# Bernat-C/MRI-Diffusion-SuperResolution

Measured on AMD Instinct MI355X. Metric: MRI slices/sec (50-step DDIM, 256^2, bs=32), higher is better.
Workload: dtype bf16; 1 GPU; configs[1]: 256x256 1-ch synthetic MRI slices -> 4x32x32 latents, SD-1.5-size UNet (859.5M params, random init) + rank-4 LoRA, 50-step DDIM, bs=32 per GPU; ddim_steps=50, parallelism=slice-sharded x1 (no collective), lora=explicit adapters, down-projection + rank-r update inside the projection GEMMs, tile_table=profiles/r03_tune_cache.tsv, hipgraph=True

## Files before the change

include/mrisr_debug.h:

```cpp
#ifndef MRISR_DEBUG_H
#define MRISR_DEBUG_H
#ifdef __cplusplus
extern "C" {
#endif

void mrisr_debug_force_split(int splitk);
void mrisr_debug_force_tile(int tile);
void mrisr_debug_prefer_tile(int tile);
void mrisr_debug_gemm_flags(int flags);
void mrisr_debug_gemm_stamps(void* dev_buf, int tile);
void mrisr_debug_set_tile_eff(int tile, double eff);
void mrisr_debug_set_tuned(const char* key, int tile, int splitk);
void mrisr_debug_gn_fused(int on);

int mrisr_autotune_stats(int* shapes, double* ms);
void mrisr_autotune_release(void);

int mrisr_bench_gemm(int M, int N, int K, int conv, int B, int H, int W, int stride, int ups, int c1, int tile, int splitk,
                     int iters, float* ms_out);

void mrisr_debug_sk_inkernel(int on);

void mrisr_debug_subpix(int min_rows);

void mrisr_debug_temb_table(int on);

void mrisr_debug_mlp_proj(int on);

void mrisr_debug_gn_slabs(int on);

void mrisr_debug_sc_fused(int on);

void mrisr_debug_ff_proj_fused(int on);

void mrisr_debug_xattn_tail(int on);
void mrisr_debug_xattn_tail_stamps(void* dev_buf);

int mrisr_bench_mlp(int M, int hidden, int iters, float* ms_out);

#ifdef __cplusplus
}
#endif
#endif
```

mri-diffusion-superresolution_amd/csrc/capi_ops.hip:

```cpp
#include <algorithm>
#include <cmath>
#include <cstring>
#include <memory>
#include <vector>

#include "api.h"
#include "model.h"
#include "train_ops.h"

using namespace mrisr;

namespace {
struct OpScratch {
    std::vector<std::unique_ptr<DevBuf>> bufs;
    void* alloc(size_t bytes, bool zero = false) {
        bufs.emplace_back(new DevBuf());
        if (bufs.back()->reserve(bytes ? bytes : 1, zero)) return nullptr;
        return bufs.back()->p;
    }
};
template <typename T>
int op_gemm_run(OpScratch& sc, hipStream_t st, GemmArgs& g) {
    return gemm_run<T>(g, st, false, [&sc](size_t n) { return sc.alloc(n); });
}
template <typename T>
int op_plan(GemmArgs& g, int splitk, bool replan, DevBuf& part) {
    g.splitk = splitk;
    if (splitk <= 0) { g.splitk = 1; TRY(gemm_choose(g, sizeof(T) == 2)); }
    else if (replan) { TRY(gemm_choose(g, sizeof(T) == 2)); g.splitk = splitk; }
    return gemm_alloc_partial(g, devbuf_alloc(part));
}
}
template <typename T>
__global__ void rows_to_heads_kernel(const T* x, T* dst, int B, int N, int H, int hd, int npad, int dpad, int tr) {
    const long long total = (long long)B * N * H * hd;
    for (long long i = blockIdx.x * 256ll + threadIdx.x; i < total; i += (long long)gridDim.x * 256) {
        const int dd = (int)(i % hd);
        const int h = (int)((i / hd) % H);
        const int tok = (int)((i / ((long long)hd * H)) % N);
        const int b = (int)(i / ((long long)hd * H * N));
        const size_t bh = (size_t)b * H + h;
        if (!tr) dst[(bh * npad + tok) * dpad + dd] = x[i];
        else dst[(bh * dpad + dd) * npad + tok] = x[i];
    }
}

template <typename T>
static int op_conv3x3_t(const mrisr_tensor* x, const mrisr_tensor* x2, const float* w, const float* bias, int cout,
                        int stride, int ups, int act, int splitk, mrisr_tensor* y, hipStream_t st) {
    const int B = (int)x->shape[0], C0 = (int)x->shape[1], H = (int)x->shape[2], W = (int)x->shape[3];
    const int C1 = x2 ? (int)x2->shape[1] : 0;
    const int Cin = C0 + C1;
    DevBuf wp, part;
    TRY(wp.reserve((size_t)cout * Cin * 9 * sizeof(T), false));
    TRY(launch_pack_conv3x3<T>(w, wp.p, cout, Cin, 3, st));
    if (!x2 && !ups && Cin % (128 / (int)sizeof(T)) != 0) {
        DirectConvArgs a;
        a.x = x->data; a.w = wp.p; a.bias = bias; a.y = y->data; a.B = B; a.Hin = H; a.Win = W; a.Cin = Cin;
        a.Hout = (H - 1) / stride + 1; a.Wout = (W - 1) / stride + 1; a.Cout = cout; a.ks = 3; a.stride = stride; a.pad = 1; a.act = act;
        MRISR_REQUIRE(y->shape[1] == cout && y->shape[2] == a.Hout && y->shape[3] == a.Wout, "conv output shape");
        TRY(launch_direct_conv<T>(a, st));
        MRISR_CHECK_HIP(hipStreamSynchronize(st));
        return 0;
    }
    if (ups == 2) {
        MRISR_REQUIRE(sizeof(T) == 2 && !x2 && stride == 1 && act == ACT_NONE && (4 * Cin) % 64 == 0 && cout % 8 == 0, "sub-pixel upsample conv: bf16, single source");
        MRISR_REQUIRE(y->shape[1] == cout && y->shape[2] == 2 * H && y->shape[3] == 2 * W, "conv output shape");
        DevBuf sp, planes;
        TRY(sp.reserve((size_t)16 * cout * Cin * sizeof(T), false));
        TRY(planes.reserve((size_t)4 * B * H * W * cout * sizeof(T), false));
        TRY(launch_pack_conv_subpix<T>(w, sp.p, cout, Cin, st));
        GemmArgs g;
        ga_rows(g, x->data, C0, C0); ga_conv3(g, B, H, W); g.kw = 2; g.subpix = 1;
        ga_batch(g, 4, 0, (long long)cout * 4 * Cin, (long long)B * H * W * cout); ga_weight(g, sp.p, B * H * W, cout, 4 * Cin);
        g.bias = bias; ga_out(g, planes.p, cout);
        TRY(gemm_run<T>(g, st, false, devbuf_alloc(part)));
        TRY(launch_subpix_shuffle<T>(planes.p, y->data, B, H, W, cout, st));
        MRISR_CHECK_HIP(hipStreamSynchronize(st));
        return 0;
    }
    GemmArgs g;
    ga_rows(g, x->data, C0, C0);
    if (x2) ga_rows2(g, x2->data, C1, C1);
    ga_conv3(g, B, H, W, stride, ups);
    MRISR_REQUIRE(y->shape[1] == cout && y->shape[2] == g.Hout && y->shape[3] == g.Wout, "conv output shape");
    ga_weight(g, wp.p, B * g.Hout * g.Wout, cout, 9 * Cin); g.bias = bias; g.act = act; ga_out(g, y->data, cout);
    TRY(op_plan<T>(g, splitk, false, part));
    TRY(launch_gemm<T>(g, st));
    MRISR_CHECK_HIP(hipStreamSynchronize(st));
    return 0;
}

extern "C" void mrisr_debug_force_tile(int t);
struct ForcedTile {
    explicit ForcedTile(int t) { mrisr_debug_force_tile(t); }
    ~ForcedTile() { mrisr_debug_force_tile(0); }
    ForcedTile(const ForcedTile&) = delete;
    ForcedTile& operator=(const ForcedTile&) = delete;
};

static int op_conv3x3_sc_t(const mrisr_tensor* x, const mrisr_tensor* x2, const float* w, const float* bias, const mrisr_tensor* xs,
                           const mrisr_tensor* xs2, const float* w_sc, const float* bias_sc, int cout, int splitk, int tile, int fused,
                           mrisr_tensor* y, hipStream_t st) {
    typedef bf16 T;
    const int B = (int)x->shape[0], C0 = (int)x->shape[1], H = (int)x->shape[2], W = (int)x->shape[3];
    const int C1 = x2 ? (int)x2->shape[1] : 0, Cin = C0 + C1;
    const int S0 = (int)xs->shape[1], S1 = xs2 ? (int)xs2->shape[1] : 0, Cs = S0 + S1;
    MRISR_REQUIRE(xs->shape[0] == B && xs->shape[2] == H && xs->shape[3] == W && (!xs2 || (xs2->shape[0] == B && xs2->shape[2] == H && xs2->shape[3] == W)),
                  "shortcut sources: the conv input's batch and image size");
    MRISR_REQUIRE(y->shape[1] == cout && y->shape[2] == H && y->shape[3] == W, "conv output shape");
    MRISR_REQUIRE(Cin % 64 == 0 && S0 % 64 == 0 && S1 % 64 == 0 && cout % 4 == 0, "channel counts: multiples of 64");
    const size_t K9 = (size_t)9 * Cin, Kt = K9 + Cs;
    DevBuf w9, wsc, bank, bsum, part;
    TRY(w9.reserve((size_t)cout * K9 * sizeof(T), false));
    TRY(wsc.reserve((size_t)cout * Cs * sizeof(T), false));
    TRY(launch_pack_conv3x3<T>(w, w9.p, cout, Cin, 3, st));
    TRY(launch_pack_rows<T>(w_sc, cout, Cs, wsc.p, Cs, 0, 0, 0, 0, 1.0f, st));
    GemmArgs g;
    ga_rows(g, x->data, C0, C0);
    if (x2) ga_rows2(g, x2->data, C1, C1);
    ga_conv3(g, B, H, W); ga_out(g, y->data, cout);
    const int M = B * H * W;
    if (fused) {
        TRY(bank.reserve((size_t)cout * Kt * sizeof(T), false));
        TRY(bsum.reserve((size_t)cout * sizeof(float), false));
        MRISR_CHECK_HIP(hipMemcpy2DAsync(bank.p, Kt * sizeof(T), w9.p, K9 * sizeof(T), K9 * sizeof(T), cout, hipMemcpyDeviceToDevice, st));
        MRISR_CHECK_HIP(hipMemcpy2DAsync(static_cast<T*>(bank.p) + K9, Kt * sizeof(T), wsc.p, (size_t)Cs * sizeof(T), (size_t)Cs * sizeof(T), cout,
                                         hipMemcpyDeviceToDevice, st));
        MRISR_CHECK_HIP(hipMemcpyAsync(bsum.p, bias, (size_t)cout * sizeof(float), hipMemcpyDeviceToDevice, st));
        TRY(launch_add_inplace<float>(bsum.p, bias_sc, cout, st));
        ga_tail(g, xs->data, S0, S0);
        if (xs2) ga_tail2(g, xs2->data, S1, S1);
        ga_weight(g, bank.p, M, cout, (int)Kt); g.bias = static_cast<const float*>(bsum.p);
    } else {
        GemmArgs s;
        ga_rows(s, xs->data, S0, S0);
        if (xs2) ga_rows2(s, xs2->data, S1, S1);
        ga_weight(s, wsc.p, M, cout, Cs); s.bias = bias_sc; ga_out(s, y->data, cout);
        DevBuf spart;
        TRY(gemm_run<T>(s, st, false, devbuf_alloc(spart)));
        MRISR_CHECK_HIP(hipStreamSynchronize(st));
        ga_weight(g, w9.p, M, cout, (int)K9); g.bias = bias; ga_resid(g, y->data, cout);
    }
    ForcedTile forced(tile);
    TRY(op_plan<T>(g, splitk, !tile, part));
    TRY(launch_gemm<T>(g, st));
    MRISR_CHECK_HIP(hipStreamSynchronize(st));
    return 0;
}

static int run_planned(GemmArgs& g, DevBuf& part, hipStream_t st) { return gemm_run<bf16>(g, st, false, devbuf_alloc(part)); }
static int op_ff_proj_t(const mrisr_tensor* h, const mrisr_tensor* t, const mrisr_tensor* x, const float* w2, const float* b2, const float* wp,
                        const float* bp, int tile, int fused, mrisr_tensor* y, hipStream_t st) {
    typedef bf16 T;
    const int M = (int)h->shape[0], K4 = (int)h->shape[1], C = (int)t->shape[1];
    MRISR_REQUIRE(t->shape[0] == M && x->shape[0] == M && x->shape[1] == C && y->shape[0] == M && y->shape[1] == C, "ff.net.2 + proj_out: row shapes");
    MRISR_REQUIRE(C % 64 == 0 && K4 % 64 == 0, "ff.net.2 + proj_out: widths that are multiples of 64");
    DevBuf bank, bsum, w2p, wpp, mid, part;
    if (fused) {
        const int Kt = K4 + C;
        TRY(bank.reserve((size_t)C * Kt * sizeof(T), false));
        TRY(bsum.reserve((size_t)C * sizeof(float), false));
        TRY(launch_compose_ff_proj(wp, w2, b2, bp, bank.p, Kt, static_cast<float*>(bsum.p), C, K4, st));
        TRY(launch_pack_rows<T>(wp, C, C, bank.p, Kt, 0, K4, 0, 0, 1.0f, st));
        GemmArgs g;
        ga_rows(g, h->data, K4, K4); ga_rows2(g, t->data, C, C); ga_weight(g, bank.p, M, C, Kt); g.bias = static_cast<const float*>(bsum.p);
        ga_resid(g, x->data, C); ga_out(g, y->data, C); g.no_rp = 1;
        ForcedTile forced(tile);
        TRY(run_planned(g, part, st));
    } else {
        TRY(w2p.reserve((size_t)C * K4 * sizeof(T), false));
        TRY(wpp.reserve((size_t)C * C * sizeof(T), false));
        TRY(mid.reserve((size_t)M * C * sizeof(T), false));
        TRY(launch_pack_rows<T>(w2, C, K4, w2p.p, K4, 0, 0, 0, 0, 1.0f, st));
        TRY(launch_pack_rows<T>(wp, C, C, wpp.p, C, 0, 0, 0, 0, 1.0f, st));
        GemmArgs g1, g2;
        auto linear = [&](GemmArgs& g, const void* a, int k, const void* w, const float* b, const void* resid, void* out) {
            ga_rows(g, a, k, k); ga_weight(g, w, M, C, k); g.bias = b; ga_resid(g, resid, C); ga_out(g, out, C);
        };
        linear(g1, h->data, K4, w2p.p, b2, t->data, mid.p);
        linear(g2, mid.p, C, wpp.p, bp, x->data, y->data);
        ForcedTile forced(tile);
        TRY(run_planned(g1, part, st));
        MRISR_CHECK_HIP(hipStreamSynchronize(st));
        TRY(run_planned(g2, part, st));
    }
    MRISR_CHECK_HIP(hipStreamSynchronize(st));
    return 0;
}

template <typename T>
static int op_attention_t(const mrisr_tensor* q, const mrisr_tensor* k, const mrisr_tensor* v, int H, int flash,
                          mrisr_tensor* out, hipStream_t st) {
    const int B = (int)q->shape[0], N = (int)q->shape[1], C = (int)q->shape[2], Nk = (int)k->shape[1];
    const int hd = C / H;
    constexpr int BK = 128 / (int)sizeof(T);
    const bool use_flash = flash && sizeof(T) == 2;
    const int dpad = round_up(hd, use_flash ? 32 : BK), npad = round_up(N, 64), nkpad = round_up(Nk, 64);
    DevBuf qb, kb, vb;
    TRY(qb.reserve((size_t)B * H * npad * dpad * sizeof(T), true));
    TRY(kb.reserve((size_t)B * H * nkpad * dpad * sizeof(T), true));
    TRY(vb.reserve((size_t)B * H * dpad * nkpad * sizeof(T), true));
    auto conv = [&](const mrisr_tensor* x, void* dst, int n, int np, int tr) {
        hipLaunchKernelGGL(rows_to_heads_kernel<T>, dim3(1024), dim3(256), 0, st, static_cast<const T*>(x->data),
                           static_cast<T*>(dst), B, n, H, hd, np, dpad, tr);
    };
    conv(q, qb.p, N, npad, 0);
    conv(k, kb.p, Nk, nkpad, 0);
    conv(v, vb.p, Nk, nkpad, 1);
    MRISR_CHECK_HIP(hipGetLastError());
    OpScratch sc;
    auto scratch = [&sc](size_t n) { return sc.alloc(n); };
    AttnGeom geo;
    geo.B = B; geo.H = H; geo.N = N; geo.npad = npad; geo.hd = hd; geo.dpad = dpad; geo.nk = Nk; geo.nkpad = nkpad;
    if (use_flash) {
        const bool fp8 = flash == 2;
        AttnArgs a;
        TRY(attn_flash_args(a, geo, qb.p, kb.p, vb.p, out->data, nullptr, fp8, scratch));
        TRY(attn_flash_launch(a, fp8, false, st));
    } else {
        const size_t cnt = (size_t)B * H * N * nkpad;
        float* S = static_cast<float*>(sc.alloc(cnt * sizeof(float)));
        void* P = sizeof(T) == 2 ? sc.alloc(cnt * sizeof(T)) : S;
        if (!S || !P) return 7;
        TRY(attn_materialised<T>(geo, qb.p, kb.p, vb.p, S, P, out->data, false, st, [&](GemmArgs& g) { return op_gemm_run<T>(sc, st, g); }));
    }
    MRISR_CHECK_HIP(hipStreamSynchronize(st));
    return 0;
}


template <typename T>
static int op_conv_lora_down_t(const void* x, int B, int H, int W, int cin, const float* A, int r, float* z, int route, hipStream_t st) {
    DevBuf av, bdummy, scr;
    TRY(av.reserve((size_t)r * 9 * cin * sizeof(T), false));
    TRY(bdummy.reserve((size_t)r * sizeof(float), true));
    TRY(launch_conv_lora_pack<T>(A, static_cast<const float*>(bdummy.p), 1.0f, av.p, nullptr, nullptr, nullptr, cin, 1, r, st));
    const size_t sb = conv_lora_down_scratch_bytes(B * H * W, cin, r, sizeof(T), route);
    if (sb) TRY(scr.reserve(sb, false));
    TRY(launch_conv_lora_down<T>(x, av.p, z, B, H, W, cin, r, static_cast<float*>(scr.p), st, route));
    MRISR_CHECK_HIP(hipStreamSynchronize(st));
    return 0;
}
template <typename T>
static int op_conv_lora_dgrad_t(const float* dz, int B, int H, int W, int r, const float* A, int cin, void* dx, int accumulate, hipStream_t st) {
    DevBuf av, bank, bdummy;
    TRY(av.reserve((size_t)r * 9 * cin * sizeof(T), false));
    if (sizeof(T) == 2) TRY(bank.reserve((size_t)cin * conv_lora_kpad(r) * 2, true));
    TRY(bdummy.reserve((size_t)r * sizeof(float), true));
    TRY(launch_conv_lora_pack<T>(A, static_cast<const float*>(bdummy.p), 1.0f, av.p, bank.p, nullptr, nullptr, cin, 1, r, st));
    TRY(launch_conv_lora_dgrad<T>(dz, av.p, bank.p, dx, B, H, W, cin, r, accumulate, st));
    MRISR_CHECK_HIP(hipStreamSynchronize(st));
    return 0;
}
template <typename T>
static int op_conv3x3_lora_t(const mrisr_tensor* x, const float* w, const float* bias, const float* A, const float* Bm, int r, float scale,
                             const float* rowvec, const mrisr_tensor* resid, int cout, int splitk, int tile, mrisr_tensor* y, hipStream_t st) {
    const int B = (int)x->shape[0], Cin = (int)x->shape[1], H = (int)x->shape[2], W = (int)x->shape[3], M = B * H * W;
    DevBuf wp, av, sb, zb, scr, part;
    TRY(wp.reserve((size_t)cout * Cin * 9 * sizeof(T), false));
    TRY(launch_pack_conv3x3<T>(w, wp.p, cout, Cin, 3, st));
    if (r > 0) {
        TRY(av.reserve((size_t)r * 9 * Cin * sizeof(T), false));
        TRY(sb.reserve((size_t)cout * r * sizeof(float), false));
        TRY(zb.reserve((size_t)M * r * sizeof(float), false));
        TRY(launch_conv_lora_pack<T>(A, Bm, scale, av.p, nullptr, static_cast<float*>(sb.p), nullptr, Cin, cout, r, st));
        const size_t sbytes = conv_lora_down_scratch_bytes(M, Cin, r, sizeof(T));
        if (sbytes) TRY(scr.reserve(sbytes, false));
        TRY(launch_conv_lora_down<T>(x->data, av.p, static_cast<float*>(zb.p), B, H, W, Cin, r, static_cast<float*>(scr.p), st));
    }
    GemmArgs g;
    ga_rows(g, x->data, Cin, Cin); ga_conv3(g, B, H, W); ga_weight(g, wp.p, M, cout, 9 * Cin); g.bias = bias;
    if (rowvec) ga_rowvec(g, rowvec, cout, H * W);
    if (resid) ga_resid(g, resid->data, cout);
    ga_out(g, y->data, cout);
    if (r > 0) ga_lora_epilogue(g, static_cast<const float*>(zb.p), r, static_cast<const float*>(sb.p), r, cout);
    ForcedTile forced(tile);
    TRY(op_plan<T>(g, splitk, !tile, part));
    TRY(launch_gemm<T>(g, st));
    MRISR_CHECK_HIP(hipStreamSynchronize(st));
    return 0;
}

static GemmArgs op_linear_args(const mrisr_tensor* x, const void* w, int n, const float* bias, int act, const mrisr_tensor* y) {
    const int K = (int)x->shape[1];
    GemmArgs g;
    ga_rows(g, x->data, K, K); ga_weight(g, w, (int)x->shape[0], n, K); g.bias = bias; g.act = act; ga_out(g, y->data, (int)y->shape[1]);
    return g;
}

extern "C" {

static int op_dtype_ok(const mrisr_tensor* x) {
    MRISR_REQUIRE(x && (x->dtype == MRISR_F32 || x->dtype == MRISR_BF16), "op tensors: f32 or bf16");
    return 0;
}

int mrisr_op_conv3x3(const mrisr_tensor* x, const mrisr_tensor* x2, const float* w_oihw_dev, const float* bias_dev,
                     int cout, int stride, int upsample, int act, int splitk, int tile, mrisr_tensor* y,
                     void* stream) {
    API_BEGIN
    TRY(op_dtype_ok(x));
    TRY(gemm_prepare());
    MRISR_REQUIRE(x->layout == MRISR_NHWC && y && y->layout == MRISR_NHWC && y->dtype == x->dtype, "NHWC in/out, same dtype");
    ForcedTile forced(tile);
    return x->dtype == MRISR_F32 ? op_conv3x3_t<float>(x, x2, w_oihw_dev, bias_dev, cout, stride, upsample, act, splitk, y, (hipStream_t)stream)
                                 : op_conv3x3_t<bf16>(x, x2, w_oihw_dev, bias_dev, cout, stride, upsample, act, splitk, y, (hipStream_t)stream);
    API_END
}

int mrisr_op_conv3x3_sc(const mrisr_tensor* x, const mrisr_tensor* x2, const float* w_oihw_dev, const float* bias_dev, const mrisr_tensor* xs,
                        const mrisr_tensor* xs2, const float* w_sc_dev, const float* bias_sc_dev, int cout, int splitk, int tile, int fused,
                        mrisr_tensor* y, void* stream) {
    API_BEGIN
    MRISR_REQUIRE(x && xs && y && w_oihw_dev && bias_dev && w_sc_dev && bias_sc_dev, "null argument");
    MRISR_REQUIRE(x->dtype == MRISR_BF16 && xs->dtype == MRISR_BF16 && y->dtype == MRISR_BF16 && (!x2 || x2->dtype == MRISR_BF16) &&
                      (!xs2 || xs2->dtype == MRISR_BF16),
                  "conv3x3 + 1x1 shortcut: bf16 tensors");
    MRISR_REQUIRE(x->layout == MRISR_NHWC && xs->layout == MRISR_NHWC && y->layout == MRISR_NHWC && (!x2 || x2->layout == MRISR_NHWC) &&
                      (!xs2 || xs2->layout == MRISR_NHWC),
                  "NHWC in/out");
    TRY(gemm_prepare());
    return op_conv3x3_sc_t(x, x2, w_oihw_dev, bias_dev, xs, xs2, w_sc_dev, bias_sc_dev, cout, splitk, tile, fused, y, (hipStream_t)stream);
    API_END
}

int mrisr_op_ff_proj(const mrisr_tensor* h, const mrisr_tensor* t, const mrisr_tensor* x, const float* w2_dev, const float* b2_dev,
                     const float* wp_dev, const float* bp_dev, int tile, int fused, mrisr_tensor* y, void* stream) {
    API_BEGIN
    MRISR_REQUIRE(h && t && x && y && w2_dev && wp_dev, "null argument");
    MRISR_REQUIRE(h->dtype == MRISR_BF16 && t->dtype == MRISR_BF16 && x->dtype == MRISR_BF16 && y->dtype == MRISR_BF16, "ff.net.2 + proj_out: bf16 rows");
    MRISR_REQUIRE(h->ndim == 2 && t->ndim == 2 && x->ndim == 2 && y->ndim == 2, "rows in/out");
    TRY(gemm_prepare());
    return op_ff_proj_t(h, t, x, w2_dev, b2_dev, wp_dev, bp_dev, tile, fused, y, (hipStream_t)stream);
    API_END
}

int mrisr_op_linear(const mrisr_tensor* x, const float* w_dev, const float* bias_dev, int n, int act, int splitk,
                    int tile, mrisr_tensor* y, void* stream) {
    API_BEGIN
    TRY(op_dtype_ok(x));
    TRY(gemm_prepare());
    MRISR_REQUIRE(x->ndim == 2 && y && y->ndim == 2 && y->dtype == x->dtype, "rows in/out");
    hipStream_t st = (hipStream_t)stream;
    const int M = (int)x->shape[0], K = (int)x->shape[1];
    const bool f32 = x->dtype == MRISR_F32;
    const int esz = f32 ? 4 : 2;
    DevBuf wp, part, bp;
    TRY(wp.reserve((size_t)n * K * esz, false));
    const bool geglu = act == ACT_GEGLU;
    if (f32) TRY(launch_pack_rows<float>(w_dev, n, K, wp.p, K, 0, 0, geglu ? 1 : 0, n / 2, 1.0f, st));
    else TRY(launch_pack_rows<bf16>(w_dev, n, K, wp.p, K, 0, 0, geglu ? 1 : 0, n / 2, 1.0f, st));
    const float* bias = bias_dev;
    if (geglu && bias_dev) {
        TRY(bp.reserve((size_t)n * sizeof(float), false));
        TRY(launch_pack_bias_geglu(bias_dev, static_cast<float*>(bp.p), n / 2, st));
        bias = static_cast<const float*>(bp.p);
    }
    GemmArgs g = op_linear_args(x, wp.p, n, bias, act, y);
    ForcedTile forced(tile);
    TRY(f32 ? op_plan<float>(g, splitk, false, part) : op_plan<bf16>(g, splitk, false, part));
    TRY(f32 ? launch_gemm<float>(g, st) : launch_gemm<bf16>(g, st));
    MRISR_CHECK_HIP(hipStreamSynchronize(st));
    return 0;
    API_END
}

int mrisr_op_linear_resid(const mrisr_tensor* x, const float* w_dev, const float* bias_dev, int n, const float* rowvec_dev, int rowvec_rows,
                          const float* lora_a_dev, const float* lora_b_dev, int lora_r, float lora_scale, const mrisr_tensor* resid, int splitk,
                          int tile, mrisr_tensor* y, void* stream) {
    API_BEGIN
    typedef bf16 T;
    MRISR_REQUIRE(x && y && w_dev && x->dtype == MRISR_BF16 && y->dtype == MRISR_BF16 && x->ndim == 2 && y->ndim == 2, "linear + residual: bf16 rows in/out");
    MRISR_REQUIRE(!resid || (resid->dtype == MRISR_BF16 && resid->ndim == 2 && resid->shape[0] == x->shape[0] && resid->shape[1] >= n), "residual rows");
    TRY(gemm_prepare());
    hipStream_t st = (hipStream_t)stream;
    const int M = (int)x->shape[0], K = (int)x->shape[1];
    MRISR_REQUIRE(!rowvec_dev || (rowvec_rows >= 1 && M % rowvec_rows == 0), "row vector: rows dividing M");
    MRISR_REQUIRE(lora_r == 0 || (lora_r >= 1 && lora_r <= 16 && lora_a_dev && lora_b_dev && splitk <= 1), "adapter: rank 1 .. 16, A and B, un-split");
    DevBuf wp, part, av, sb, zb;
    TRY(wp.reserve((size_t)n * K * sizeof(T), false));
    TRY(launch_pack_rows<T>(w_dev, n, K, wp.p, K, 0, 0, 0, 0, 1.0f, st));
    GemmArgs g = op_linear_args(x, wp.p, n, bias_dev, ACT_NONE, y);
    if (rowvec_dev) ga_rowvec(g, rowvec_dev, n, M / rowvec_rows);
    if (resid) ga_resid(g, resid->data, (int)resid->shape[1]);
    ForcedTile forced(tile);
    if (!lora_r) {
// ... 877 lines not shown
```

mri-diffusion-superresolution_amd/csrc/gemm.hip:

```cpp
#include "common.h"
#include "prof.h"

#include <cstdio>
#include <cstdlib>
#include <cstring>
#include <map>
#include <mutex>
#include <unordered_map>

namespace mrisr {

static void* g_zero_page = nullptr;
static constexpr size_t kZeroPageBytes = 128 * 1024;
const void* zero_page() { return g_zero_page; }
int init_zero_page() {
    if (g_zero_page) return 0;
    MRISR_CHECK_HIP(hipMalloc(&g_zero_page, kZeroPageBytes));
    MRISR_CHECK_HIP(hipMemset(g_zero_page, 0, kZeroPageBytes));
    return 0;
}

typedef const __attribute__((address_space(1))) void* gptr_t;
typedef __attribute__((address_space(3))) void* lptr_t;

__device__ __forceinline__ void glds16(const void* src, char* lds_wave_base) {
    __builtin_amdgcn_global_load_lds((gptr_t)src, (lptr_t)lds_wave_base, 16, 0, 0);
}

template <typename T>
__device__ __forceinline__ void store4(T* p, const float* v);
template <>
__device__ __forceinline__ void store4<float>(float* p, const float* v) {
    *reinterpret_cast<float4*>(p) = make_float4(v[0], v[1], v[2], v[3]);
}
template <>
__device__ __forceinline__ void store4<bf16>(bf16* p, const float* v) {
    bf16x4 o = {(bf16)v[0], (bf16)v[1], (bf16)v[2], (bf16)v[3]};
    *reinterpret_cast<bf16x4*>(p) = o;
}
template <typename T>
__device__ __forceinline__ void load4(const T* p, float* v);
template <>
__device__ __forceinline__ void load4<float>(const float* p, float* v) {
    float4 t = *reinterpret_cast<const float4*>(p);
    v[0] = t.x; v[1] = t.y; v[2] = t.z; v[3] = t.w;
}
template <>
__device__ __forceinline__ void load4<bf16>(const bf16* p, float* v) {
    bf16x4 t = *reinterpret_cast<const bf16x4*>(p);
    v[0] = (float)t[0]; v[1] = (float)t[1]; v[2] = (float)t[2]; v[3] = (float)t[3];
}

__device__ __forceinline__ int exchange_tokens4(const float* v, unsigned& w0, unsigned& w1) {
    const int fr = threadIdx.x & 15;
    const bool odd = fr & 1;
    const float s0 = __shfl_xor(odd ? v[0] : v[2], 1);
    const float s1 = __shfl_xor(odd ? v[1] : v[3], 1);
    const float a0 = odd ? s0 : v[0], a1 = odd ? v[2] : s0;
    const float c0 = odd ? s1 : v[1], c1 = odd ? v[3] : s1;
    typedef __attribute__((ext_vector_type(2))) __bf16 bf16x2;
    const bf16x2 pa = {(bf16)a0, (bf16)a1}, pc = {(bf16)c0, (bf16)c1};
    const unsigned ua = __builtin_bit_cast(unsigned, pa), uc = __builtin_bit_cast(unsigned, pc);
    const bool hi2 = fr & 2;
    const unsigned recv = __shfl_xor(hi2 ? ua : uc, 2);
    w0 = hi2 ? recv : ua;
    w1 = hi2 ? uc : recv;
    return (odd ? 2 : 0) + (hi2 ? 1 : 0);
}

template <typename T>
__device__ __forceinline__ void epilogue4(const GemmArgs& g, int z, int m, int n0, float* v, const float* vg, const float* zl = nullptr,
                                          T* lds_dst = nullptr, bool resid_later = false, bool mfma_lanes = true, T* lds_t = nullptr,
                                          int ml = 0, int nl = 0, int tpitch = 0, const float* pb = nullptr, const float* pbg = nullptr) {
    const float alpha = g.alpha;
    float b4[4] = {0.f, 0.f, 0.f, 0.f};
    if (g.act == ACT_GEGLU) {
        float bu[4] = {0, 0, 0, 0}, bg[4] = {0, 0, 0, 0};
        if (pb) {
#pragma unroll
            for (int r = 0; r < 4; ++r) { bu[r] = pb[r]; bg[r] = pbg[r]; }
        } else if (g.bias) {
            load4<float>(g.bias + n0, bu);
            load4<float>(g.bias + n0 + 16, bg);
        }
#pragma unroll
        for (int r = 0; r < 4; ++r) v[r] = (v[r] * alpha + bu[r]) * gelu_erf_t<T>(vg[r] * alpha + bg[r]);
        const int nc = (n0 >> 5) * 16 + (n0 & 15);
        T* o = reinterpret_cast<T*>(g.out) + (size_t)m * g.ldo + nc;
        store4<T>(o, v);
        return;
    }
    if (pb) {
#pragma unroll
        for (int r = 0; r < 4; ++r) b4[r] = pb[r];
    } else if (g.bias) {
        load4<float>(g.bias + n0, b4);
    }
#pragma unroll
    for (int r = 0; r < 4; ++r) v[r] = v[r] * alpha + b4[r];
    if (g.lora_z || zl) {
        const float* zr = (zl ? zl : g.lora_z + (size_t)m * g.lora_zld) + (n0 / g.lora_secN) * g.lora_r;
        const float* lb = g.lora_b + (size_t)n0 * g.lora_r;
        if (g.lora_r == 4) {
            float z4[4];
            load4<float>(zr, z4);
#pragma unroll
            for (int r = 0; r < 4; ++r) {
                float l4[4];
                load4<float>(lb + r * 4, l4);
                v[r] += z4[0] * l4[0] + z4[1] * l4[1] + z4[2] * l4[2] + z4[3] * l4[3];
            }
        } else {
            for (int q = 0; q < g.lora_r; ++q) {
                const float zq = zr[q];
#pragma unroll
                for (int r = 0; r < 4; ++r) v[r] += zq * lb[r * g.lora_r + q];
            }
        }
    }
    if (g.rowvec && !(pb && g.rowvec_div >= g.M)) {
        float t4[4];
        load4<float>(g.rowvec + (size_t)(m / g.rowvec_div) * g.rowvec_ld + n0, t4);
#pragma unroll
        for (int r = 0; r < 4; ++r) v[r] += t4[r];
    }
    if (g.act == ACT_RELU) {
#pragma unroll
        for (int r = 0; r < 4; ++r) v[r] = fmaxf(v[r], 0.f);
    } else if (g.act == ACT_SILU) {
#pragma unroll
        for (int r = 0; r < 4; ++r) v[r] = silu_f(v[r]);
    }
    const size_t zoff = (size_t)(z / g.heads) * g.o_bs + (size_t)(z % g.heads) * g.o_hs;
    if (g.resid && !resid_later) {
        float r4[4];
        load4<T>(reinterpret_cast<const T*>(g.resid) + zoff + (size_t)m * g.ldr + n0, r4);
#pragma unroll
        for (int r = 0; r < 4; ++r) v[r] += r4[r];
    }
    if (g.out_mode == OUT_NONE) {
        if (v[0] == 1.2345e30f) store4<T>(reinterpret_cast<T*>(g.out), v);
    } else if (g.out_mode == OUT_ROWS) {
        if (lds_dst) store4<T>(lds_dst, v);
        else store4<T>(reinterpret_cast<T*>(g.out) + zoff + (size_t)m * g.ldo + n0, v);
    } else if (g.out_mode == OUT_F32) {
        store4<float>(reinterpret_cast<float*>(g.out) + zoff + (size_t)m * g.ldo + n0, v);
    } else {
        if (lds_dst) {
            store4<T>(lds_dst, v);
            return;
        }
        if (sizeof(T) == 2 && lds_t) {
            unsigned w0, w1;
            const int drow = exchange_tokens4(v, w0, w1);
            *reinterpret_cast<uint2*>(lds_t + (nl + drow) * tpitch + (ml & ~3)) = make_uint2(w0, w1);
            return;
        }
        const int s = n0 / g.secC;
        const int c = n0 - s * g.secC;
        const int h = c / g.hd;
        const int dd = c - h * g.hd;
        const int b = m / g.ntok;
        const int tok = m - b * g.ntok;
        T* base = reinterpret_cast<T*>(s == 0 ? g.sec_ptr[0] : (s == 1 ? g.sec_ptr[1] : g.sec_ptr[2]));
        const int tr = (s == 0 ? g.sec_tr[0] : (s == 1 ? g.sec_tr[1] : g.sec_tr[2]));
        const size_t bh = (size_t)b * g.nheads + h;
        if (!tr) {
            store4<T>(base + (bh * g.npad + tok) * g.dpad + dd, v);
        } else if (sizeof(T) == 2 && mfma_lanes && (g.ntok & 3) == 0 && (g.M & 3) == 0) {
            unsigned w0, w1;
            const int drow = exchange_tokens4(v, w0, w1);
            T* o = base + (bh * g.dpad + dd + drow) * g.npad + (tok & ~3);
            *reinterpret_cast<uint2*>(o) = make_uint2(w0, w1);
        } else {
            T* o = base + (bh * g.dpad + dd) * g.npad + tok;
#pragma unroll
            for (int r = 0; r < 4; ++r) o[(size_t)r * g.npad] = from_f32<T>(v[r]);
        }
    }
}

template <int NFR>
__device__ __forceinline__ void preload_cols(const GemmArgs& g, int nbase, float (&pb)[NFR][4]) {
    const bool fold = g.rowvec && g.rowvec_div >= g.M;
#pragma unroll
    for (int i = 0; i < NFR; ++i) {
        const int n = min(nbase + i * 16, g.N - 4);
        float b[4] = {0.f, 0.f, 0.f, 0.f}, t[4] = {0.f, 0.f, 0.f, 0.f};
        if (g.bias) load4<float>(g.bias + n, b);
        if (fold) load4<float>(g.rowvec + n, t);
#pragma unroll
        for (int r = 0; r < 4; ++r) pb[i][r] = b[r] + t[r];
    }
}

template <int NFR>
__device__ __forceinline__ void preload_cols(const GemmArgs& g, int nbase, f32x4 (&pb)[NFR]) {
    const bool fold = g.rowvec && g.rowvec_div >= g.M;
#pragma unroll
    for (int i = 0; i < NFR; ++i) pb[i] = f32x4{0.f, 0.f, 0.f, 0.f};
    if (g.bias) {
#pragma unroll
        for (int i = 0; i < NFR; ++i) pb[i] = *reinterpret_cast<const f32x4*>(g.bias + min(nbase + i * 16, g.N - 4));
    }
    if (fold) {
#pragma unroll
        for (int i = 0; i < NFR; ++i) pb[i] += *reinterpret_cast<const f32x4*>(g.rowvec + min(nbase + i * 16, g.N - 4));
    }
}

template <typename T> struct Frag;
template <> struct Frag<bf16> { typedef bf16x8 type; };
template <> struct Frag<float> { typedef f32x4 type; };

__device__ __forceinline__ void mma(f32x4& acc, const bf16x8& w, const bf16x8& a) {
    acc = __builtin_amdgcn_mfma_f32_16x16x32_bf16(w, a, acc, 0, 0, 0);
}
__device__ __forceinline__ void mma(f32x4& acc, const f32x4& w, const f32x4& a) {
#pragma unroll
    for (int j = 0; j < 4; ++j) acc = __builtin_amdgcn_mfma_f32_16x16x4f32(w[j], a[j], acc, 0, 0, 0);
}

__device__ __forceinline__ void lds_poison(char* smem_base, int nthreads) {
    const unsigned bytes = ((const __attribute__((address_space(4))) unsigned*)__builtin_amdgcn_dispatch_ptr())[7];
    for (unsigned o = threadIdx.x * 16u; o + 16u <= bytes; o += (unsigned)nthreads * 16u)
        *reinterpret_cast<uint4*>(smem_base + o) = make_uint4(~0u, ~0u, ~0u, ~0u);
    __syncthreads();
}
static int gemm_flags_now();

static constexpr int kStampHdr = 8, kStampWgs = 1024, kStampSlotWords = kStampHdr + 8 * kStampWgs, kStampSlots = 256;
__device__ __forceinline__ unsigned long long* gemm_stamp_slot(const GemmArgs& g, bool header) {
    if (!g.stamps) return nullptr;
    const unsigned wg = blockIdx.x + gridDim.x * (blockIdx.y + gridDim.y * blockIdx.z);
    if (header && wg == 0 && threadIdx.x == 0) {
        g.stamps[0] = (unsigned long long)g.M; g.stamps[1] = (unsigned long long)g.N; g.stamps[2] = (unsigned long long)g.K;
        g.stamps[3] = (unsigned long long)gridDim.x * gridDim.y * gridDim.z;
        g.stamps[4] = (g.resid ? 1u : 0u) | (g.lora_a ? 2u : 0u) | (g.conv ? 4u : 0u) | (g.cs0 ? 8u : 0u);
        g.stamps[5] = (unsigned long long)g.splitk; g.stamps[6] = (unsigned long long)(unsigned)g.dbg; g.stamps[7] = 1ull;
    }
    return wg < (unsigned)kStampWgs ? g.stamps + kStampHdr + (size_t)wg * 8 : nullptr;
}
__device__ __forceinline__ unsigned long long* gemm_stamp_word(const GemmArgs& g, int k, bool header = false) {
    unsigned long long* const slot = gemm_stamp_slot(g, header);
    return slot ? slot + k : nullptr;
}
static_assert(kStampSlotWords == kStampHdr + 8 * kStampWgs, "a slot: the header, then 8 words for each of the first kStampWgs workgroups");

template <typename T, int BM, int BN, int WGM, int WGN>
__global__ __launch_bounds__(256) void gemm_kernel(const GemmArgs g, const char* __restrict__ zero) {
    constexpr int EB = sizeof(T);
    constexpr int CH = 16 / EB;
    constexpr int BK = 8 * CH;
    constexpr int A_IT = BM / 32, W_IT = BN / 32;
    constexpr int WTM = BM / WGM, WTN = BN / WGN;
    constexpr int MF = WTM / 16, NF = WTN / 16;
    constexpr int STAGE = (BM + BN) * 128;
    static_assert(WGM * WGN == 4, "4 waves");
    extern __shared__ __attribute__((aligned(16))) char smem[];

    const int tid = threadIdx.x;
    const int lane = tid & 63;
    const int wave = __builtin_amdgcn_readfirstlane(tid >> 6);
    const int z = blockIdx.z;
    const int split = blockIdx.y;
    if (g.dbg & 2048) lds_poison(smem, (int)blockDim.x);

    const int ntn = (g.N + BN - 1) / BN;
    const int ntm = (g.M + BM - 1) / BM;
    const int nblk = ntn * ntm;
    int logical;
    {
        const int bid = blockIdx.x;
        const int xcd = bid & 7, q = nblk >> 3, r = nblk & 7;
        logical = (xcd < r ? xcd * (q + 1) : r * (q + 1) + (xcd - r) * q) + (bid >> 3);
    }
    int tn, tm;
    {
        const int GM = g.group_m > 1 ? g.group_m : 1;
        const int per_group = GM * ntn;
        const int grp = logical / per_group;
        const int first_m = grp * GM;
        const int gsz = min(GM, ntm - first_m);
        const int within = logical - grp * per_group;
        tm = first_m + within % gsz;
        tn = within / gsz;
    }
    const int m0 = tm * BM, n0 = tn * BN;

    const T* a0 = reinterpret_cast<const T*>(g.a0) + (size_t)z * g.a_bs;
    const T* a1 = reinterpret_cast<const T*>(g.a1);
    const T* w = reinterpret_cast<const T*>(g.w) + (size_t)z * g.w_bs;

    const int lrow = tid >> 3, pch = tid & 7;
    const T* wsrc[W_IT];
    bool wok[W_IT];
#pragma unroll
    for (int it = 0; it < W_IT; ++it) {
        const int row = it * 32 + lrow;
        const int n = n0 + row;
        const int c = pch ^ (row & 7);
        wok[it] = n < g.N;
        wsrc[it] = w + (size_t)n * g.K + c * CH;
    }
    const T* asrc0[A_IT];
    const T* asrc1[A_IT];
    int ab[A_IT], ay[A_IT], ax[A_IT];
    bool aok[A_IT];
    int acoff[A_IT];
#pragma unroll
    for (int it = 0; it < A_IT; ++it) {
        const int row = it * 32 + lrow;
        const int m = m0 + row;
        const int c = pch ^ (row & 7);
        aok[it] = m < g.M;
        acoff[it] = c * CH;
        if (!g.conv) {
            asrc0[it] = a0 + (size_t)m * g.lda0 + c * CH;
            asrc1[it] = a1 ? a1 + (size_t)m * g.lda1 + c * CH : nullptr;
            ab[it] = ay[it] = ax[it] = 0;
        } else {
            const int hw = g.Hout * g.Wout;
            const int b = m / hw;
            const int rem = m - b * hw;
            const int oy = rem / g.Wout;
            ab[it] = b;
            ay[it] = oy * g.stride - g.pad;
            ax[it] = (rem - oy * g.Wout) * g.stride - g.pad;
            asrc0[it] = asrc1[it] = nullptr;
        }
    }

    const int nkt = g.K / BK;
    const int per = (nkt + g.splitk - 1) / g.splitk;
    const int kt_beg = split * per;
    const int kt_end = min(nkt, kt_beg + per);
    const int Ct = g.c0 + g.c1;
    int tap = 0, cc = 0;
    if (g.conv) {
        const int k0 = kt_beg * BK;
        tap = k0 / Ct;
        cc = k0 - tap * Ct;
    }
    const int Hc = g.Hin << g.ups, Wc = g.Win << g.ups;

    auto stage = [&](int kt, int buf) {
        char* sb = smem + buf * STAGE;
        const int k0 = kt * BK;
#pragma unroll
        for (int it = 0; it < W_IT; ++it) {
            const void* src = wok[it] ? (const void*)(wsrc[it] + k0) : (const void*)zero;
            glds16(src, sb + BM * 128 + (it * 256 + wave * 64) * 16);
        }
        if (!g.conv) {
            const bool second = k0 >= g.c0;
#pragma unroll
            for (int it = 0; it < A_IT; ++it) {
                const void* src = zero;
                if (aok[it]) src = second ? (const void*)(asrc1[it] + (k0 - g.c0)) : (const void*)(asrc0[it] + k0);
                glds16(src, sb + (it * 256 + wave * 64) * 16);
            }
        } else {
            const int ky = tap / 3, kx = tap - ky * 3;
            const bool second = cc >= g.c0;
            const T* base = second ? a1 : a0;
            const int ld = second ? g.lda1 : g.lda0;
            const int ch = second ? cc - g.c0 : cc;
#pragma unroll
            for (int it = 0; it < A_IT; ++it) {
                const int iy = ay[it] + ky, ix = ax[it] + kx;
                const void* src = zero;
                if (aok[it] && iy >= 0 && iy < Hc && ix >= 0 && ix < Wc && (!g.zstuff || ((iy | ix) & 1) == 0)) {
                    const size_t pix = ((size_t)ab[it] * g.Hin + (iy >> g.ups)) * g.Win + (ix >> g.ups);
                    src = base + pix * ld + ch + acoff[it];
                }
                glds16(src, sb + (it * 256 + wave * 64) * 16);
            }
            cc += BK;
            if (cc >= Ct) { cc = 0; ++tap; }
        }
    };

    f32x4 acc[NF][MF];
#pragma unroll
    for (int i = 0; i < NF; ++i)
#pragma unroll
        for (int j = 0; j < MF; ++j) acc[i][j] = f32x4{0.f, 0.f, 0.f, 0.f};

    const int wm0 = (wave / WGN) * WTM, wn0 = (wave % WGN) * WTN;
    const int fr = lane & 15, fg = lane >> 4;

    typedef typename Frag<T>::type frag_t;
    auto compute = [&](int buf) {
        const char* sa = smem + buf * STAGE;
        const char* sw = sa + BM * 128;
#pragma unroll
        for (int kk = 0; kk < 2; ++kk) {
            const int phys = ((kk * 4 + fg) ^ (fr & 7)) * 16;
            frag_t wf[NF], af[MF];
#pragma unroll
            for (int i = 0; i < NF; ++i)
                wf[i] = *reinterpret_cast<const frag_t*>(sw + (wn0 + i * 16 + fr) * 128 + phys);
#pragma unroll
            for (int j = 0; j < MF; ++j)
                af[j] = *reinterpret_cast<const frag_t*>(sa + (wm0 + j * 16 + fr) * 128 + phys);
#pragma unroll
            for (int i = 0; i < NF; ++i)
#pragma unroll
                for (int j = 0; j < MF; ++j) mma(acc[i][j], wf[i], af[j]);
        }
    };

    if (kt_beg < kt_end) {
        stage(kt_beg, 0);
        asm volatile("s_waitcnt vmcnt(0)" ::: "memory");
        __syncthreads();
        int cur = 0;
        for (int kt = kt_beg; kt < kt_end; ++kt) {
            if (kt + 1 < kt_end) stage(kt + 1, cur ^ 1);
            compute(cur);
            asm volatile("s_waitcnt vmcnt(0)" ::: "memory");
            __syncthreads();
            cur ^= 1;
        }
    }

    if (g.splitk > 1) {
        float* part = g.partial + ((size_t)z * g.splitk + split) * (size_t)g.M * g.N;
#pragma unroll
        for (int i = 0; i < NF; ++i)
#pragma unroll
            for (int j = 0; j < MF; ++j) {
                const int m = m0 + wm0 + j * 16 + fr;
                const int n = n0 + wn0 + i * 16 + fg * 4;
                if (m < g.M && n < g.N) {
                    float v[4] = {acc[i][j][0], acc[i][j][1], acc[i][j][2], acc[i][j][3]};
                    store4<float>(part + (size_t)m * g.N + n, v);
                }
            }
        return;
    }
    float pb[NF][4];
    preload_cols<NF>(g, n0 + wn0 + fg * 4, pb);
    if (g.act == ACT_GEGLU) {
#pragma unroll
        for (int i = 0; i < NF; i += 2)
#pragma unroll
            for (int j = 0; j < MF; ++j) {
                const int m = m0 + wm0 + j * 16 + fr;
                const int n = n0 + wn0 + i * 16 + fg * 4;
                if (m < g.M && n < g.N) {
                    float v[4] = {acc[i][j][0], acc[i][j][1], acc[i][j][2], acc[i][j][3]};
                    float vg[4] = {acc[i + 1][j][0], acc[i + 1][j][1], acc[i + 1][j][2], acc[i + 1][j][3]};
                    epilogue4<T>(g, z, m, n, v, vg, nullptr, nullptr, false, true, nullptr, 0, 0, 0, pb[i], pb[i + 1 < NF ? i + 1 : i]);
                }
            }
        return;
    }
#pragma unroll
    for (int i = 0; i < NF; ++i)
#pragma unroll
        for (int j = 0; j < MF; ++j) {
            const int m = m0 + wm0 + j * 16 + fr;
            const int n = n0 + wn0 + i * 16 + fg * 4;
            if (m < g.M && n < g.N) {
                float v[4] = {acc[i][j][0], acc[i][j][1], acc[i][j][2], acc[i][j][3]};
                epilogue4<T>(g, z, m, n, v, nullptr, nullptr, nullptr, false, true, nullptr, 0, 0, 0, pb[i]);
            }
        }
}

template <int BM, int BN, int NT = 256>
__device__ __forceinline__ void copy_out_tile(const GemmArgs& g, const bf16* otile, int pitch, int m0, int n0, int z, bool add_resid,
                                              unsigned long long* stamp_resid = nullptr) {
    __syncthreads();
    constexpr int CPR = BN / 8;
    bf16* out = reinterpret_cast<bf16*>(g.out) + (size_t)z * g.o_bs;
    const bf16* res = add_resid ? reinterpret_cast<const bf16*>(g.resid) + (size_t)z * g.o_bs : nullptr;
    constexpr int TOTAL = BM * CPR, IT = (TOTAL + NT - 1) / NT, BATCH = IT < 5 ? IT : 5;
    for (int it0 = 0; it0 < IT; it0 += BATCH) {
        bf16x8 rv[BATCH];
#pragma unroll
        for (int u = 0; u < BATCH; ++u) {
            const int idx = (int)threadIdx.x + (it0 + u) * NT;
            const int row = idx / CPR, ch = idx - row * CPR;
            const int m = m0 + row, n = n0 + ch * 8;
            if (res && idx < TOTAL && m < g.M && n + 8 <= g.N) rv[u] = *reinterpret_cast<const bf16x8*>(res + (size_t)m * g.ldr + n);
        }
        if (stamp_resid && it0 == 0 && threadIdx.x == 0) {
            if (res) asm volatile("s_waitcnt vmcnt(0)" ::: "memory");
            *stamp_resid = __builtin_readcyclecounter();
        }
#pragma unroll
        for (int u = 0; u < BATCH; ++u) {
            const int idx = (int)threadIdx.x + (it0 + u) * NT;
            const int row = idx / CPR, ch = idx - row * CPR;
            const int m = m0 + row, n = n0 + ch * 8;
            if (idx >= TOTAL || m >= g.M || n >= g.N) continue;
            const bf16* src = otile + row * pitch + ch * 8;
            bf16* dst = out + (size_t)m * g.ldo + n;
            if (n + 8 <= g.N) {
                bf16x8 v = *reinterpret_cast<const bf16x8*>(src);
                if (res) {
#pragma unroll
                    for (int e = 0; e < 8; ++e) v[e] = (bf16)((float)v[e] + (float)rv[u][e]);
                }
                *reinterpret_cast<bf16x8*>(dst) = v;
            } else {
                bf16x4 v = *reinterpret_cast<const bf16x4*>(src);
                if (res) {
                    const bf16x4 r = *reinterpret_cast<const bf16x4*>(res + (size_t)m * g.ldr + n);
#pragma unroll
                    for (int e = 0; e < 4; ++e) v[e] = (bf16)((float)v[e] + (float)r[e]);
                }
                *reinterpret_cast<bf16x4*>(dst) = v;
            }
        }
    }
}

template <int BM, int BN>
__device__ __forceinline__ void copy_out_heads(const GemmArgs& g, const bf16* otile, int m0, int n0, bool tr) {
    __syncthreads();
    const int s = n0 / g.secC;
    bf16* base = reinterpret_cast<bf16*>(s == 0 ? g.sec_ptr[0] : (s == 1 ? g.sec_ptr[1] : g.sec_ptr[2]));
    if (!tr) {
        constexpr int CPR = BN / 8, P = BN + 8;
        for (int idx = threadIdx.x; idx < BM * CPR; idx += 256) {
            const int row = idx / CPR, ch = idx - row * CPR;
            const int m = m0 + row, n = n0 + ch * 8;
            if (m >= g.M || n >= g.N) continue;
            const int c = n - s * g.secC, h = c / g.hd, dd = c - h * g.hd;
            const int b = m / g.ntok, tok = m - b * g.ntok;
            *reinterpret_cast<bf16x8*>(base + (((size_t)b * g.nheads + h) * g.npad + tok) * g.dpad + dd) =
                *reinterpret_cast<const bf16x8*>(otile + row * P + ch * 8);
        }
    } else {
        constexpr int TPC = BM / 8, P = BM + 8;
        for (int idx = threadIdx.x; idx < BN * TPC; idx += 256) {
            const int col = idx / TPC, tc = idx - col * TPC;
            const int n = n0 + col, m = m0 + tc * 8;
            if (m >= g.M || n >= g.N) continue;
            const int c = n - s * g.secC, h = c / g.hd, dd = c - h * g.hd;
            const int b = m / g.ntok, tok = m - b * g.ntok;
            *reinterpret_cast<bf16x8*>(base + (((size_t)b * g.nheads + h) * g.dpad + dd) * g.npad + tok) =
                *reinterpret_cast<const bf16x8*>(otile + col * P + tc * 8);
        }
    }
}

typedef __attribute__((address_space(3))) void* lds_ptr_t;
__device__ __forceinline__ __amdgpu_buffer_rsrc_t make_rsrc(const void* p, unsigned bytes) {
    return __builtin_amdgcn_make_buffer_rsrc(const_cast<void*>(p), 0, bytes, 0x00020000);
}
__device__ __forceinline__ void bl16(__amdgpu_buffer_rsrc_t r, char* lds_wave_base, unsigned voff, unsigned soff) {
    __builtin_amdgcn_raw_ptr_buffer_load_lds(r, (lds_ptr_t)lds_wave_base, 16, voff, soff, 0, 0);
}
#define BL_OOB 0x80000000u


__device__ __forceinline__ void pretouch_weights(const __amdgpu_buffer_rsrc_t& rw, long long w_bytes, char* scratch, int wave, int lane, int cap) {
    const int n_wg = (int)(gridDim.x * gridDim.y);
    const int wg = (int)(blockIdx.x + blockIdx.y * gridDim.x);
    const long long pieces = (w_bytes + 1023) >> 10;
    const int per_wg = (int)((pieces + n_wg - 1) / n_wg);
    const int per_wave = min((per_wg + 3) >> 2, cap);
    const long long first = (long long)wg * per_wg + (long long)wave * per_wave;
    for (int i = 0; i < per_wave; ++i) {
        const long long pc = first + i;
        const unsigned off = pc < pieces ? (unsigned)(pc << 10) + (unsigned)lane * 16u : BL_OOB;
        bl16(rw, scratch + ((wave * 2 + (i & 1)) << 10), off, 0u);
    }
}

template <int NF, int MF>
__device__ __forceinline__ bool splitk_last_arriver(const GemmArgs& g, f32x4 (&acc)[NF][MF], unsigned tile_idx, const float* slab0, int m_base, int n_base,
                                                    int fr, int fg, char* ticket_lds) {
    __builtin_amdgcn_fence(__ATOMIC_RELEASE, "agent");
    __syncthreads();
    if (threadIdx.x == 0)
        *reinterpret_cast<volatile unsigned*>(ticket_lds) = __hip_atomic_fetch_add(g.sk_counters + tile_idx, 1u, __ATOMIC_ACQ_REL, __HIP_MEMORY_SCOPE_AGENT);
    __syncthreads();
    const unsigned ticket = *reinterpret_cast<volatile unsigned*>(ticket_lds);
    if (ticket != (unsigned)g.splitk - 1) return false;
    __syncthreads();
    if (threadIdx.x == 0) __hip_atomic_store(g.sk_counters + tile_idx, 0u, __ATOMIC_RELAXED, __HIP_MEMORY_SCOPE_AGENT);
    __builtin_amdgcn_fence(__ATOMIC_ACQUIRE, "agent");
    const size_t slab = (size_t)g.M * g.N;
#pragma unroll
    for (int i = 0; i < NF; ++i)
#pragma unroll
        for (int j = 0; j < MF; ++j) acc[i][j] = f32x4{0.f, 0.f, 0.f, 0.f};
    for (int s = 0; s < g.splitk; ++s) {
        const float* p = slab0 + (size_t)s * slab;
#pragma unroll
        for (int i = 0; i < NF; ++i)
#pragma unroll
            for (int j = 0; j < MF; ++j) {
                const int m = m_base + j * 16 + fr;
                const int n = n_base + i * 16 + fg * 4;
                if (m < g.M && n < g.N) {
                    const f32x4 t = __builtin_nontemporal_load(reinterpret_cast<const f32x4*>(p + (size_t)m * g.N + n));
                    acc[i][j] += t;
                }
            }
    }
    return true;
}

template <int BM, int BN, int WGM, int WGN, int NSTAGE, bool LORA>
__global__ __launch_bounds__(256, 2) void gemm_bl_kernel(const GemmArgs g) {
    static_assert(NSTAGE >= 2 && NSTAGE <= 4, "2 (drain per tile), 3 or 4 (counted ring)");
    typedef bf16 T;
    constexpr int BK = 64;
    constexpr int A_IT = BM / 32, W_IT = BN / 32;
    constexpr int WTM = BM / WGM, WTN = BN / WGN;
    constexpr int MF = WTM / 16, NF = WTN / 16;
    constexpr int STAGE = (BM + BN) * 128 + (LORA ? 16 * 128 : 0);
    static_assert(WGM * WGN == 4, "4 waves");
    extern __shared__ __attribute__((aligned(16))) char smem[];

    const int tid = threadIdx.x;
    const int lane = tid & 63;
    const int wave = __builtin_amdgcn_readfirstlane(tid >> 6);
    const int z = blockIdx.z;
    const int split = blockIdx.y;
    auto stamp = [&](int k, bool drain = false) {
        if constexpr (NSTAGE == 2) {
            unsigned long long* const stp = gemm_stamp_word(g, k, k == 0);
            if (stp && tid == 0) {
                if (drain) asm volatile("s_waitcnt vmcnt(0) lgkmcnt(0)" ::: "memory");
                *stp = __builtin_readcyclecounter();
            }
        }
    };
    stamp(0);
    if (g.dbg & 2048) lds_poison(smem, (int)blockDim.x);

    const int ntn = (g.N + BN - 1) / BN;
    const int ntm = (g.M + BM - 1) / BM;
    const int nblk = ntn * ntm;
    int logical;
    {
        const int bid = blockIdx.x;
        const int xcd = bid & 7, q = nblk >> 3, r = nblk & 7;
        logical = (xcd < r ? xcd * (q + 1) : r * (q + 1) + (xcd - r) * q) + (bid >> 3);
    }
    int tn, tm;
    {
        const int GM = g.group_m > 1 ? g.group_m : 1;
        const int per_group = GM * ntn;
        const int grp = logical / per_group;
        const int first_m = grp * GM;
        const int gsz = min(GM, ntm - first_m);
        const int within = logical - grp * per_group;
        tm = first_m + within % gsz;
        tn = within / gsz;
    }
    const int m0 = tm * BM, n0 = tn * BN;

    const T* a0p = reinterpret_cast<const T*>(g.a0) + (size_t)z * g.a_bs;
    const T* a1p = reinterpret_cast<const T*>(g.a1);
    const T* wp = reinterpret_cast<const T*>(g.w) + (size_t)z * g.w_bs;
    const long long a_rows = g.conv ? (long long)g.B * g.Hin * g.Win : (long long)g.M;
    const __amdgpu_buffer_rsrc_t rw = make_rsrc(wp, (unsigned)min((long long)g.N * g.K * 2, 0x7FFFFFFFll));
    const __amdgpu_buffer_rsrc_t ra0 = make_rsrc(a0p, (unsigned)min(a_rows * g.lda0 * 2, 0x7FFFFFFFll));
    const __amdgpu_buffer_rsrc_t ra1 = make_rsrc(a1p ? (const void*)a1p : (const void*)a0p,
                                                 a1p ? (unsigned)min(a_rows * g.lda1 * 2, 0x7FFFFFFFll) : 0u);

    const int lrow = tid >> 3, pch = tid & 7;
    unsigned wvo[W_IT];
#pragma unroll
    for (int it = 0; it < W_IT; ++it) {
        const int row = it * 32 + lrow;
        const int n = n0 + row;
        const int c = pch ^ (row & 7);
        wvo[it] = n < g.N ? (unsigned)(((size_t)n * g.K + c * 8) * 2) : BL_OOB;
    }
    unsigned avo[A_IT], avo1[A_IT];
    int ab[A_IT], ay[A_IT], ax[A_IT];
#pragma unroll
    for (int it = 0; it < A_IT; ++it) {
        const int row = it * 32 + lrow;
        const int m = m0 + row;
        const int c = pch ^ (row & 7);
        const bool ok = m < g.M;
        avo[it] = avo1[it] = BL_OOB;
        ab[it] = -1;
        ay[it] = ax[it] = 0;
        if (!g.conv) {
            if (ok) {
                avo[it] = (unsigned)(((size_t)m * g.lda0 + c * 8) * 2);
                avo1[it] = (unsigned)(((size_t)m * g.lda1 + c * 8) * 2);
            }
        } else if (ok) {
            const int hw = g.Hout * g.Wout;
            const int b = m / hw;
            const int rem = m - b * hw;
            const int oy = rem / g.Wout;
            ab[it] = b * g.Hin;
            ay[it] = oy * g.stride - g.pad + (g.subpix ? (z >> 1) : 0);
            ax[it] = (rem - oy * g.Wout) * g.stride - g.pad + (g.subpix ? (z & 1) : 0);
        }
    }
    const int acb = pch * 16;
    const __amdgpu_buffer_rsrc_t rl = make_rsrc(LORA ? g.lora_a : (const void*)wp, LORA ? (unsigned)((long long)g.lora_R * g.K * 2) : 0u);
    unsigned lvo = BL_OOB;
    if (LORA && (wave < 2 || NSTAGE > 2)) {
        const int row = (wave & 1) * 8 + (lane >> 3);
        const int c = (lane & 7) ^ (row & 7);
        if (row < g.lora_R) lvo = (unsigned)(((size_t)row * g.K + c * 8) * 2);
        else if (NSTAGE > 2) lvo = (unsigned)(((size_t)(g.lora_R - 1) * g.K + c * 8) * 2);
    }

    const int nkt = g.K / BK;
    const int per = (nkt + g.splitk - 1) / g.splitk;
    const int kt_beg = split * per;
    const int kt_end = min(nkt, kt_beg + per);
    const int Ct = g.c0 + g.c1;
    const int Hc = g.Hin << g.ups, Wc = g.Win << g.ups;
    int tap = 0, cc = 0, seg_key = -1;
    const int ntaps = g.kw * g.kw;
    if (g.conv) {
        const int k0 = kt_beg * BK;
        tap = min(k0 / Ct, ntaps);
        cc = k0 - tap * Ct;
    }

    auto stage_w = [&](int kt, int buf) {
        char* sb = smem + buf * STAGE;
        const unsigned k0b = (unsigned)kt * BK * 2;
#pragma unroll
        for (int it = 0; it < W_IT; ++it) bl16(rw, sb + BM * 128 + (it * 256 + wave * 64) * 16, wvo[it], k0b);
        if (LORA && (wave < 2 || NSTAGE > 2)) bl16(rl, sb + (BM + BN) * 128 + (wave & 1) * 64 * 16, lvo, k0b);
    };
    auto stage_a = [&](int kt, int buf) {
        char* sb = smem + buf * STAGE;
        const unsigned k0b = (unsigned)kt * BK * 2;
        if (!g.conv) {
            const bool second = kt * BK >= g.c0;
            if (!second) {
#pragma unroll
                for (int it = 0; it < A_IT; ++it) bl16(ra0, sb + (it * 256 + wave * 64) * 16, avo[it], k0b);
            } else {
                const unsigned kb = (unsigned)(kt * BK - g.c0) * 2;
#pragma unroll
                for (int it = 0; it < A_IT; ++it) bl16(ra1, sb + (it * 256 + wave * 64) * 16, avo1[it], kb);
            }
        } else {
            const bool tail = tap >= ntaps;
            const int cfirst = tail ? +g.cs0 : +g.c0;
            const bool second = cc >= cfirst;
            const int key = tap * 2 + (second ? 1 : 0);
            if (key != seg_key) {
                seg_key = key;
                int ky = g.kw == 3 ? tap / 3 : tap / g.kw, kx = tap - ky * g.kw;
                int ld = second ? g.lda1 : g.lda0;
                if (tail) { ky = kx = g.pad; ld = second ? +g.lds1 : +g.lds0; }
#pragma unroll
                for (int it = 0; it < A_IT; ++it) {
                    const int row = it * 32 + lrow;
                    const int c = pch ^ (row & 7);
                    const int iy = ay[it] + ky, ix = ax[it] + kx;
                    const bool ok = ab[it] >= 0 && iy >= 0 && iy < Hc && ix >= 0 && ix < Wc && (!g.zstuff || ((iy | ix) & 1) == 0);
                    const unsigned pix = (unsigned)((ab[it] + (iy >> g.ups)) * g.Win + (ix >> g.ups));
                    avo[it] = ok ? (pix * (unsigned)ld + (unsigned)c * 8u) * 2u : BL_OOB;
                }
            }
            const unsigned chb = (unsigned)(second ? cc - cfirst : cc) * 2;
            if (tail) {
                const long long ld_cur = second ? +g.lds1 : +g.lds0;
                const __amdgpu_buffer_rsrc_t rs = make_rsrc(second ? g.s1 : g.s0, (unsigned)min(a_rows * ld_cur * 2, 0x7FFFFFFFll));
#pragma unroll
                for (int it = 0; it < A_IT; ++it) bl16(rs, sb + (it * 256 + wave * 64) * 16, avo[it], chb);
            } else if (!second) {
#pragma unroll
                for (int it = 0; it < A_IT; ++it) bl16(ra0, sb + (it * 256 + wave * 64) * 16, avo[it], chb);
            } else {
#pragma unroll
                for (int it = 0; it < A_IT; ++it) bl16(ra1, sb + (it * 256 + wave * 64) * 16, avo[it], chb);
            }
            cc += BK;
            if (cc >= Ct && !tail) { cc = 0; ++tap; }
        }
    };
    auto stage = [&](int kt, int buf) { stage_w(kt, buf); stage_a(kt, buf); };
    (void)acb;

    f32x4 acc[NF][MF];
#pragma unroll
    for (int i = 0; i < NF; ++i)
#pragma unroll
        for (int j = 0; j < MF; ++j) acc[i][j] = f32x4{0.f, 0.f, 0.f, 0.f};

    const int wm0 = (wave / WGN) * WTM, wn0 = (wave % WGN) * WTN;
    const int fr = lane & 15, fg = lane >> 4;
    const bool zwave = LORA && (wave % WGN) == 0;
    const bool lora_mma = LORA && g.lora_r == 4 && g.alpha == 1.0f && !(g.dbg & 8);
    bf16x8 lbf[NF];
    if (LORA) {
#pragma unroll
        for (int i = 0; i < NF; ++i) {
            lbf[i] = bf16x8{0, 0, 0, 0, 0, 0, 0, 0};
            const int n = n0 + wn0 + i * 16 + fr;
            if (lora_mma && n < g.N) {
                const int sec = n / g.lora_secN;
                if ((sec >> 1) == fg) {
                    const f32x4 l = *reinterpret_cast<const f32x4*>(g.lora_b + (size_t)n * 4);
                    if (sec & 1) { lbf[i][4] = (bf16)l[0]; lbf[i][5] = (bf16)l[1]; lbf[i][6] = (bf16)l[2]; lbf[i][7] = (bf16)l[3]; }
                    else { lbf[i][0] = (bf16)l[0]; lbf[i][1] = (bf16)l[1]; lbf[i][2] = (bf16)l[2]; lbf[i][3] = (bf16)l[3]; }
                }
            }
        }
    }
    f32x4 zacc[MF];
#pragma unroll
    for (int j = 0; j < MF; ++j) zacc[j] = f32x4{0.f, 0.f, 0.f, 0.f};

    auto compute = [&](int buf, auto&& mid) {
        const char* sa = smem + buf * STAGE;
        const char* sw = sa + BM * 128;
#pragma unroll
        for (int kk = 0; kk < 2; ++kk) {
            if (kk == 1) mid();
            const int phys = ((kk * 4 + fg) ^ (fr & 7)) * 16;
            bf16x8 wf[NF], af[MF];
#pragma unroll
            for (int i = 0; i < NF; ++i) wf[i] = *reinterpret_cast<const bf16x8*>(sw + (wn0 + i * 16 + fr) * 128 + phys);
#pragma unroll
            for (int j = 0; j < MF; ++j) af[j] = *reinterpret_cast<const bf16x8*>(sa + (wm0 + j * 16 + fr) * 128 + phys);
#pragma unroll
            for (int i = 0; i < NF; ++i)
#pragma unroll
                for (int j = 0; j < MF; ++j) acc[i][j] = __builtin_amdgcn_mfma_f32_16x16x32_bf16(wf[i], af[j], acc[i][j], 0, 0, 0);
            if (LORA && zwave) {
                const bf16x8 lf = *reinterpret_cast<const bf16x8*>(sw + (BN + fr) * 128 + phys);
#pragma unroll
                for (int j = 0; j < MF; ++j) zacc[j] = __builtin_amdgcn_mfma_f32_16x16x32_bf16(lf, af[j], zacc[j], 0, 0, 0);
            }
        }
    };

    stamp(1);

    if constexpr (NSTAGE == 2) {
        if (kt_beg < kt_end) {
            if (g.pretouch) pretouch_weights(rw, (long long)g.N * g.K * 2, smem + STAGE, wave, lane, g.pretouch);
            stage(kt_beg, 0);
            asm volatile("s_waitcnt vmcnt(0)" ::: "memory");
            __syncthreads();
            stamp(2);
            int cur = 0;
            const bool halves = (g.dbg & 16384) != 0;
            for (int kt = kt_beg; kt < kt_end; ++kt) {
                const bool more = kt + 1 < kt_end;
                if (more) { if (halves) stage_w(kt + 1, cur ^ 1); else stage(kt + 1, cur ^ 1); }
                compute(cur, [&]() {
                    if (halves) {
                        __builtin_amdgcn_sched_barrier(0);
                        if (more) stage_a(kt + 1, cur ^ 1);
                        __builtin_amdgcn_sched_barrier(0);
                    }
                });
                asm volatile("s_waitcnt vmcnt(0)" ::: "memory");
                __syncthreads();
                cur ^= 1;
            }
        }
    } else {
        constexpr int PER = A_IT + W_IT + (LORA ? 1 : 0);
        static_assert(PER * (NSTAGE - 2) <= 63, "vmcnt range");
#pragma unroll
        for (int s = 0; s < NSTAGE - 1; ++s)
            if (kt_beg + s < kt_end) stage(kt_beg + s, s);
        int slot = 0;
        for (int kt = kt_beg; kt < kt_end; ++kt) {
            const int younger = min(NSTAGE - 2, kt_end - 1 - kt);
            if (younger >= 2) asm volatile("s_waitcnt vmcnt(%0)" ::"n"(PER * 2) : "memory");
            else if (younger == 1) asm volatile("s_waitcnt vmcnt(%0)" ::"n"(PER) : "memory");
            else asm volatile("s_waitcnt vmcnt(0)" ::: "memory");
            asm volatile("s_waitcnt lgkmcnt(0)" ::: "memory");
            __builtin_amdgcn_s_barrier();
            if (kt == kt_beg) stamp(2);
            if (kt + NSTAGE - 1 < kt_end) stage(kt + NSTAGE - 1, (slot + NSTAGE - 1) % NSTAGE);
            compute(slot, []() {});
            slot = slot + 1 == NSTAGE ? 0 : slot + 1;
        }
        __syncthreads();
    }

    stamp(3);
    float* zlds = reinterpret_cast<float*>(smem);
    if (LORA) {
        if (zwave) {
#pragma unroll
            for (int j = 0; j < MF; ++j) {
                const int ml = wm0 + j * 16 + fr;
                *reinterpret_cast<f32x4*>(zlds + ml * 16 + fg * 4) = zacc[j];
                if (g.lora_zout && tn == 0 && m0 + ml < g.M && fg * 4 < g.lora_R)
                    *reinterpret_cast<f32x4*>(g.lora_zout + (size_t)(m0 + ml) * g.lora_R + fg * 4) = zacc[j];
            }
        }
        __syncthreads();
    }
    if (LORA && lora_mma) {
        bf16x8 zf[MF];
#pragma unroll
        for (int j = 0; j < MF; ++j) {
            zf[j] = bf16x8{0, 0, 0, 0, 0, 0, 0, 0};
            if (fg < 2) {
                const float* zp = zlds + (wm0 + j * 16 + fr) * 16 + fg * 8;
                const f32x4 a = *reinterpret_cast<const f32x4*>(zp), b = *reinterpret_cast<const f32x4*>(zp + 4);
                zf[j] = bf16x8{(bf16)a[0], (bf16)a[1], (bf16)a[2], (bf16)a[3], (bf16)b[0], (bf16)b[1], (bf16)b[2], (bf16)b[3]};
            }
        }
#pragma unroll
        for (int i = 0; i < NF; ++i)
#pragma unroll
            for (int j = 0; j < MF; ++j) acc[i][j] = __builtin_amdgcn_mfma_f32_16x16x32_bf16(lbf[i], zf[j], acc[i][j], 0, 0, 0);
    }
    if (g.splitk > 1) {
        float* part = g.partial + ((size_t)z * g.splitk + split) * (size_t)g.M * g.N;
#pragma unroll
        for (int i = 0; i < NF; ++i)
#pragma unroll
            for (int j = 0; j < MF; ++j) {
                const int m = m0 + wm0 + j * 16 + fr;
                const int n = n0 + wn0 + i * 16 + fg * 4;
                if (m < g.M && n < g.N) {
                    float v[4] = {acc[i][j][0], acc[i][j][1], acc[i][j][2], acc[i][j][3]};
                    store4<float>(part + (size_t)m * g.N + n, v);
                }
            }
        if constexpr (NF * MF > 20) return;
        else {
            if (!g.sk_counters) return;
            if (!splitk_last_arriver<NF, MF>(g, acc, (unsigned)(z * gridDim.x + blockIdx.x), g.partial + (size_t)z * g.splitk * (size_t)g.M * g.N,
                                             m0 + wm0, n0 + wn0, fr, fg, smem))
                return;
        }
    }
    constexpr bool kRing = NSTAGE > 2;
    f32x4 pb[kRing ? 1 : NF];
    float pbr[kRing ? NF : 1][4];
    if constexpr (kRing) preload_cols<NF>(g, n0 + wn0 + fg * 4, pbr);
    else preload_cols<NF>(g, n0 + wn0 + fg * 4, pb);
    auto cols = [&](int i, float (&o)[4]) {
#pragma unroll
        for (int r = 0; r < 4; ++r) {
            if constexpr (kRing) o[r] = pbr[i][r];
            else o[r] = pb[i][r];
        }
    };
    stamp(4, true);
    if (g.act == ACT_GEGLU) {
        if constexpr (NF % 2 == 0) {
#pragma unroll
            for (int i = 0; i < NF; i += 2)
#pragma unroll
                for (int j = 0; j < MF; ++j) {
                    const int m = m0 + wm0 + j * 16 + fr;
                    const int n = n0 + wn0 + i * 16 + fg * 4;
                    if (m < g.M && n < g.N) {
                        float v[4] = {acc[i][j][0], acc[i][j][1], acc[i][j][2], acc[i][j][3]};
                        float vg[4] = {acc[i + 1][j][0], acc[i + 1][j][1], acc[i + 1][j][2], acc[i + 1][j][3]};
                        float bu[4], bg[4];
                        cols(i, bu); cols(i + 1, bg);
                        epilogue4<T>(g, z, m, n, v, vg, nullptr, nullptr, false, true, nullptr, 0, 0, 0, bu, bg);
                    }
                }
        }
        stamp(7);
        return;
    }
    constexpr int OPITCH = BN + 8;
    T* otile = reinterpret_cast<T*>(smem + (LORA ? BM * 16 * 4 : 0));
    const bool staged = g.out_mode == OUT_ROWS && (g.ldo & 7) == 0 && g.heads == 1 && g.stage_out;
    const bool resid_later = staged && g.resid != nullptr && (g.ldr & 7) == 0 && g.stage_out < 3;
    bool hstaged = false, htr = false;
    if (g.out_mode == OUT_HEADS && g.stage_out && !(g.dbg & 16)) {
        const int sec = n0 / g.secC;
        hstaged = (min(n0 + BN, g.N) - 1) / g.secC == sec && ((g.N | g.M | g.hd | g.secC | g.dpad | g.npad | g.ntok) & 7) == 0 && g.heads == 1 &&
                  g.batch == 1;
        htr = (sec == 0 ? g.sec_tr[0] : (sec == 1 ? g.sec_tr[1] : g.sec_tr[2])) != 0;
    }
    const bool plain_epi = !kRing && !(g.dbg & 64) && (staged || (hstaged && !htr)) && g.act == ACT_NONE && !g.lora_z && !(LORA && !lora_mma) &&
                           (!g.resid || resid_later);
    if constexpr (!kRing) {
        if (plain_epi) {
            const float alpha = g.alpha;
            const bool rows_rv = g.rowvec && g.rowvec_div < g.M;
#pragma unroll
            for (int i = 0; i < NF; ++i)
#pragma unroll
                for (int j = 0; j < MF; ++j) {
                    const int ml = wm0 + j * 16 + fr, nl = wn0 + i * 16 + fg * 4;
                    if (m0 + ml < g.M && n0 + nl < g.N) {
                        f32x4 a = acc[i][j];
#pragma unroll
                        for (int r = 0; r < 4; ++r) a[r] = a[r] * alpha + pb[i][r];
                        if (rows_rv) a += *reinterpret_cast<const f32x4*>(g.rowvec + (size_t)((m0 + ml) / g.rowvec_div) * g.rowvec_ld + n0 + nl);
                        const bf16x4 o = {(bf16)a[0], (bf16)a[1], (bf16)a[2], (bf16)a[3]};
                        *reinterpret_cast<bf16x4*>(otile + ml * OPITCH + nl) = o;
                    }
                }
        }
    }
    if (!plain_epi) {
#pragma unroll
        for (int i = 0; i < NF; ++i)
#pragma unroll
            for (int j = 0; j < MF; ++j) {
                const int m = m0 + wm0 + j * 16 + fr;
                const int n = n0 + wn0 + i * 16 + fg * 4;
                if (m < g.M && n < g.N) {
                    float v[4] = {acc[i][j][0], acc[i][j][1], acc[i][j][2], acc[i][j][3]};
                    float pbi[4];
                    cols(i, pbi);
                    epilogue4<T>(g, z, m, n, v, nullptr, LORA && !lora_mma ? zlds + (m - m0) * 16 : nullptr,
                                 staged || (hstaged && !htr) ? otile + (m - m0) * OPITCH + (n - n0) : nullptr, resid_later, true,
                                 hstaged && htr ? otile : nullptr, m - m0, n - n0, BM + 8, pbi);
                }
            }
    }
    stamp(5);
    if (staged) copy_out_tile<BM, BN>(g, otile, OPITCH, m0, n0, z, resid_later, NSTAGE == 2 ? gemm_stamp_word(g, 6) : nullptr);
    else if (hstaged) copy_out_heads<BM, BN>(g, otile, m0, n0, htr);
    stamp(7);
}

template <int BM, int BN, int WGM, int WGN>
__global__ __launch_bounds__(256, 2) void gemm_halo_kernel(const GemmArgs g) {
    typedef bf16 T;
    constexpr int BK = 64;
    constexpr int W_IT = BN / 32;
    constexpr int WTM = BM / WGM, WTN = BN / WGN;
    constexpr int MF = WTM / 16, NF = WTN / 16;
    constexpr int WSTAGE = BN * 128;
    constexpr int PIT_MAX = (BM >= 256 ? 13 : (BM >= 128 ? 9 : 6));
    static_assert(WGM * WGN == 4, "4 waves");
    extern __shared__ __attribute__((aligned(16))) char smem[];

    const int tid = threadIdx.x;
    const int lane = tid & 63;
    const int wave = __builtin_amdgcn_readfirstlane(tid >> 6);
    const int split = blockIdx.y;
    auto stamp = [&](int k, bool drain = false) {
        unsigned long long* const stp = gemm_stamp_word(g, k, k == 0);
        if (stp && tid == 0) {
            if (drain) asm volatile("s_waitcnt vmcnt(0) lgkmcnt(0)" ::: "memory");
            *stp = __builtin_readcyclecounter();
        }
    };
    stamp(0);
    if (g.dbg & 2048) lds_poison(smem, (int)blockDim.x);
    const int Wd = g.Win, Hd = g.Hin;
    const int TH = BM / Wd, PW = Wd + 2;
    const int npix = (TH + 2) * PW;
    const int pit = (npix * 8 + 255) / 256;
    char* patch = smem;
    char* wbase = smem + pit * 4096;

    const int ntn = (g.N + BN - 1) / BN;
    const int ntm = g.M / BM;
    const int nblk = ntn * ntm;
    int logical;
    {
        const int bid = blockIdx.x;
        const int xcd = bid & 7, q = nblk >> 3, r = nblk & 7;
        logical = (xcd < r ? xcd * (q + 1) : r * (q + 1) + (xcd - r) * q) + (bid >> 3);
    }
    int tn, tm;
    {
        const int GM = g.group_m > 1 ? g.group_m : 1;
        const int per_group = GM * ntn;
        const int grp = logical / per_group;
        const int first_m = grp * GM;
        const int gsz = min(GM, ntm - first_m);
        const int within = logical - grp * per_group;
        tm = first_m + within % gsz;
        tn = within / gsz;
    }
    const int m0 = tm * BM, n0 = tn * BN;
    const int img = m0 / (Hd * Wd);
    const int y0 = (m0 - img * Hd * Wd) / Wd;

    const T* a0p = reinterpret_cast<const T*>(g.a0);
    const T* a1p = reinterpret_cast<const T*>(g.a1);
    const T* wp = reinterpret_cast<const T*>(g.w);
    const long long a_rows = (long long)g.B * Hd * Wd;
    const __amdgpu_buffer_rsrc_t rw = make_rsrc(wp, (unsigned)min((long long)g.N * g.K * 2, 0x7FFFFFFFll));
    const __amdgpu_buffer_rsrc_t ra0 = make_rsrc(a0p, (unsigned)min(a_rows * g.lda0 * 2, 0x7FFFFFFFll));
    const __amdgpu_buffer_rsrc_t ra1 = make_rsrc(a1p ? (const void*)a1p : (const void*)a0p,
                                                 a1p ? (unsigned)min(a_rows * g.lda1 * 2, 0x7FFFFFFFll) : 0u);

    const int lrow = tid >> 3, pch = tid & 7;
    unsigned wvo[W_IT];
#pragma unroll
    for (int it = 0; it < W_IT; ++it) {
        const int row = it * 32 + lrow;
        const int n = n0 + row;
        const int c = pch ^ (row & 7);
        wvo[it] = n < g.N ? (unsigned)(((size_t)n * g.K + c * 8) * 2) : BL_OOB;
    }
    unsigned pvo0[PIT_MAX], pvo1[PIT_MAX];
#pragma unroll
    for (int it = 0; it < PIT_MAX; ++it) {
        const int t = it * 256 + tid;
        const int pp = t >> 3;
        const int c = (t & 7) ^ (pp & 7);
        const int hy = pp / PW, hx = pp - hy * PW;
        const int iy = y0 - 1 + hy, ix = hx - 1;
        const bool ok = pp < npix && iy >= 0 && iy < Hd && ix >= 0 && ix < Wd;
        const unsigned pix = (unsigned)((img * Hd + iy) * Wd + ix);
        pvo0[it] = ok ? (pix * (unsigned)g.lda0 + (unsigned)c * 8u) * 2u : BL_OOB;
        pvo1[it] = ok ? (pix * (unsigned)g.lda1 + (unsigned)c * 8u) * 2u : BL_OOB;
    }

    const int Ct = g.c0 + g.c1;
    const int nch = Ct / BK;
    const int per = (nch + g.splitk - 1) / g.splitk;
    const int ch_beg = split * per, ch_end = min(nch, ch_beg + per);
    const int nsc = (g.cs0 + g.cs1) / BK;
    const int per_sc = (nsc + g.splitk - 1) / g.splitk;
    const int sc_beg = min(nsc, split * per_sc), sc_end = min(nsc, sc_beg + per_sc);
    const __amdgpu_buffer_rsrc_t rs0 = make_rsrc(g.s0 ? g.s0 : (const void*)a0p, g.s0 ? (unsigned)min(a_rows * g.lds0 * 2, 0x7FFFFFFFll) : 0u);
    const __amdgpu_buffer_rsrc_t rs1 = make_rsrc(g.s1 ? g.s1 : (const void*)a0p, g.s1 ? (unsigned)min(a_rows * g.lds1 * 2, 0x7FFFFFFFll) : 0u);

    auto stage_patch = [&](int ch) {
        const int cc = ch * BK;
        const bool second = cc >= g.c0;
        const unsigned chb = (unsigned)(second ? cc - g.c0 : cc) * 2;
#pragma unroll
        for (int it = 0; it < PIT_MAX; ++it) {
            if (it < pit) {
                if (!second) bl16(ra0, patch + (it * 256 + wave * 64) * 16, pvo0[it], chb);
                else bl16(ra1, patch + (it * 256 + wave * 64) * 16, pvo1[it], chb);
            }
        }
    };
    auto stage_w = [&](int ch, int tap, int buf) {
        char* sb = wbase + buf * WSTAGE;
        const unsigned kb = (unsigned)(tap * Ct + ch * BK) * 2;
#pragma unroll
        for (int it = 0; it < W_IT; ++it) bl16(rw, sb + (it * 256 + wave * 64) * 16, wvo[it], kb);
    };
    auto stage_w_sc = [&](int sc, int buf) {
        char* sb = wbase + buf * WSTAGE;
        const unsigned kb = (unsigned)(9 * Ct + sc * BK) * 2;
#pragma unroll
        for (int it = 0; it < W_IT; ++it) bl16(rw, sb + (it * 256 + wave * 64) * 16, wvo[it], kb);
    };
    unsigned spix[PIT_MAX];
    auto sc_setup = [&]() {
#pragma unroll
        for (int it = 0; it < PIT_MAX; ++it) {
            int t = it * 256 + tid;
            asm volatile("" : "+v"(t));
            const int pp = t >> 3;
            const int hy = pp / PW, hx = pp - hy * PW;
            const bool ok = hy >= 1 && hy <= TH && hx >= 1 && hx <= Wd;
            spix[it] = ok ? (unsigned)((img * Hd + y0 - 1 + hy) * Wd + hx - 1) : ~0u;
        }
    };
    auto stage_patch_sc = [&](int sc) {
        const int cc = sc * BK;
        const bool second = cc >= g.cs0;
        const unsigned chb = (unsigned)(second ? cc - g.cs0 : cc) * 2;
        const unsigned ld2 = (unsigned)(second ? g.lds1 : g.lds0) * 2u;
#pragma unroll
        for (int it = 0; it < PIT_MAX; ++it) {
            if (it < pit) {
                const int t = it * 256 + tid;
                const unsigned c16 = (unsigned)((t & 7) ^ ((t >> 3) & 7)) * 16u;
                const unsigned off = spix[it] != ~0u ? spix[it] * ld2 + c16 : BL_OOB;
                if (!second) bl16(rs0, patch + (it * 256 + wave * 64) * 16, off, chb);
                else bl16(rs1, patch + (it * 256 + wave * 64) * 16, off, chb);
            }
        }
    };

    f32x4 acc[NF][MF];
#pragma unroll
    for (int i = 0; i < NF; ++i)
#pragma unroll
        for (int j = 0; j < MF; ++j) acc[i][j] = f32x4{0.f, 0.f, 0.f, 0.f};

    const int wm0 = (wave / WGN) * WTM, wn0 = (wave % WGN) * WTN;
    const int fr = lane & 15, fg = lane >> 4;
    int prow[MF];
#pragma unroll
    for (int j = 0; j < MF; ++j) {
        const int p = wm0 + j * 16 + fr;
        const int ty = p / Wd, tx = p - ty * Wd;
        prow[j] = ty * PW + tx;
    }

    auto compute = [&](int buf, int tap) {
        const char* sw = wbase + buf * WSTAGE;
        const int ky = tap / 3, kx = tap - ky * 3;
        const int toff = ky * PW + kx;
#pragma unroll
        for (int kk = 0; kk < 2; ++kk) {
            const int physw = ((kk * 4 + fg) ^ (fr & 7)) * 16;
            bf16x8 wf[NF], af[MF];
#pragma unroll
            for (int i = 0; i < NF; ++i) wf[i] = *reinterpret_cast<const bf16x8*>(sw + (wn0 + i * 16 + fr) * 128 + physw);
#pragma unroll
            for (int j = 0; j < MF; ++j) {
                const int pr = prow[j] + toff;
                af[j] = *reinterpret_cast<const bf16x8*>(patch + pr * 128 + (((kk * 4 + fg) ^ (pr & 7)) * 16));
            }
#pragma unroll
            for (int i = 0; i < NF; ++i)
#pragma unroll
                for (int j = 0; j < MF; ++j) acc[i][j] = __builtin_amdgcn_mfma_f32_16x16x32_bf16(wf[i], af[j], acc[i][j], 0, 0, 0);
        }
    };

    stamp(1);

    if (ch_beg < ch_end || sc_beg < sc_end) {
        int cur = 0;
        if (g.pretouch) pretouch_weights(rw, (long long)g.N * g.K * 2, wbase + WSTAGE, wave, lane, g.pretouch);
        if (ch_beg < ch_end) stage_w(ch_beg, 0, 0);
        else stage_w_sc(sc_beg, 0);
        for (int ch = ch_beg; ch < ch_end; ++ch) {
            stage_patch(ch);
            asm volatile("s_waitcnt vmcnt(0)" ::: "memory");
            __syncthreads();
            if (ch == ch_beg) stamp(2);
            if (g.dbg & 1024) {
                for (int t = tid; t < npix * 8; t += 256) {
                    bf16x8 v = *reinterpret_cast<bf16x8*>(patch + t * 16);
#pragma unroll
                    for (int e = 0; e < 8; ++e) {
                        const float f = (float)v[e] * 1.0009765625f + 0.03125f;
                        v[e] = (bf16)(f / (1.0f + __expf(-f)));
                    }
                    *reinterpret_cast<bf16x8*>(patch + t * 16) = v;
                }
                __syncthreads();
            }
            for (int tap = 0; tap < 9; ++tap) {
                if (tap + 1 < 9) stage_w(ch, tap + 1, cur ^ 1);
                else if (ch + 1 < ch_end) stage_w(ch + 1, 0, cur ^ 1);
                else if (sc_beg < sc_end) stage_w_sc(sc_beg, cur ^ 1);
                compute(cur, tap);
                asm volatile("s_waitcnt vmcnt(0)" ::: "memory");
                __syncthreads();
                cur ^= 1;
            }
        }
        if (sc_beg < sc_end) sc_setup();
        for (int sc = sc_beg; sc < sc_end; ++sc) {
            stage_patch_sc(sc);
            asm volatile("s_waitcnt vmcnt(0)" ::: "memory");
            __syncthreads();
            if (sc + 1 < sc_end) stage_w_sc(sc + 1, cur ^ 1);
            compute(cur, 4);
            asm volatile("s_waitcnt vmcnt(0)" ::: "memory");
            __syncthreads();
            cur ^= 1;
        }
    }
    stamp(3);

    if (g.splitk > 1) {
        float* part = g.partial + (size_t)split * (size_t)g.M * g.N;
#pragma unroll
        for (int i = 0; i < NF; ++i)
#pragma unroll
            for (int j = 0; j < MF; ++j) {
                const int m = m0 + wm0 + j * 16 + fr;
                const int n = n0 + wn0 + i * 16 + fg * 4;
                if (m < g.M && n < g.N) {
                    float v[4] = {acc[i][j][0], acc[i][j][1], acc[i][j][2], acc[i][j][3]};
                    store4<float>(part + (size_t)m * g.N + n, v);
                }
            }
        if constexpr (NF * MF > 20) return;
        else {
            if (!g.sk_counters) return;
            if (!splitk_last_arriver<NF, MF>(g, acc, blockIdx.x, g.partial, m0 + wm0, n0 + wn0, fr, fg, smem)) return;
        }
    }
    constexpr int OPITCH = BN + 8;
    T* otile = reinterpret_cast<T*>(smem);
    const bool staged = g.out_mode == OUT_ROWS && (g.ldo & 7) == 0 && (size_t)BM * OPITCH * 2 <= (size_t)pit * 4096 + 2 * WSTAGE && g.stage_out > 1;
    const bool resid_later = staged && g.resid != nullptr && (g.ldr & 7) == 0 && g.stage_out < 3;
    f32x4 pb[NF];
    preload_cols<NF>(g, n0 + wn0 + fg * 4, pb);
    stamp(4, true);
    const bool plain_epi = !(g.dbg & 64) && staged && g.act == ACT_NONE && !g.lora_z && (!g.resid || resid_later);
    if (plain_epi) {
        const float alpha = g.alpha;
        const bool rows_rv = g.rowvec && g.rowvec_div < g.M;
#pragma unroll
        for (int i = 0; i < NF; ++i)
#pragma unroll
            for (int j = 0; j < MF; ++j) {
                const int ml = wm0 + j * 16 + fr, nl = wn0 + i * 16 + fg * 4;
                if (m0 + ml < g.M && n0 + nl < g.N) {
                    f32x4 a = acc[i][j];
#pragma unroll
                    for (int r = 0; r < 4; ++r) a[r] = a[r] * alpha + pb[i][r];
                    if (rows_rv) a += *reinterpret_cast<const f32x4*>(g.rowvec + (size_t)((m0 + ml) / g.rowvec_div) * g.rowvec_ld + n0 + nl);
                    const bf16x4 o = {(bf16)a[0], (bf16)a[1], (bf16)a[2], (bf16)a[3]};
                    *reinterpret_cast<bf16x4*>(otile + ml * OPITCH + nl) = o;
                }
            }
    } else {
#pragma unroll
        for (int i = 0; i < NF; ++i)
#pragma unroll
            for (int j = 0; j < MF; ++j) {
                const int m = m0 + wm0 + j * 16 + fr;
                const int n = n0 + wn0 + i * 16 + fg * 4;
                if (m < g.M && n < g.N) {
                    float v[4] = {acc[i][j][0], acc[i][j][1], acc[i][j][2], acc[i][j][3]};
                    const float pbi[4] = {pb[i][0], pb[i][1], pb[i][2], pb[i][3]};
                    epilogue4<T>(g, 0, m, n, v, nullptr, nullptr, staged ? otile + (m - m0) * OPITCH + (n - n0) : nullptr, resid_later, true, nullptr,
                                 0, 0, 0, pbi);
                }
            }
    }
    stamp(5);
    if (staged) copy_out_tile<BM, BN>(g, otile, OPITCH, m0, n0, 0, resid_later, gemm_stamp_word(g, 6));
    stamp(7);
}

template <int BN, int NSTAGE>
__global__ __launch_bounds__(512, 2) void gemm_halo8_kernel(const GemmArgs g) {
    typedef bf16 T;
    constexpr int BM = 256, NT = 512, BK = 64, WGN = 2;
    constexpr int WTM = 64, WTN = BN / WGN;
    constexpr int MF = WTM / 16, NF = WTN / 16;
    constexpr int W_IT = (BN * 8 + NT - 1) / NT;
    constexpr int WSTAGE = W_IT * NT * 16;
    constexpr int PIT_MAX = 7;
    constexpr int D = NSTAGE - 1;
    static_assert(NSTAGE >= 2 && NSTAGE <= 4, "2..4 weight stages");
    extern __shared__ __attribute__((aligned(16))) char smem[];

    const int tid = threadIdx.x;
    const int lane = tid & 63;
    const int wave = __builtin_amdgcn_readfirstlane(tid >> 6);
    const int split = blockIdx.y;
    if (g.dbg & 2048) lds_poison(smem, (int)blockDim.x);
    const int Wd = g.Win, Hd = g.Hin;
    const int TH = BM / Wd, PW = Wd + 2;
    const int npix = (TH + 2) * PW;
    const int pit = (npix * 8 + NT - 1) / NT;
    char* patch = smem;
    char* wbase = smem + pit * (NT * 16);

    const int ntn = (g.N + BN - 1) / BN;
    const int ntm = g.M / BM;
    const int nblk = ntn * ntm;
    int logical;
    {
        const int bid = blockIdx.x;
        const int xcd = bid & 7, q = nblk >> 3, r = nblk & 7;
        logical = (xcd < r ? xcd * (q + 1) : r * (q + 1) + (xcd - r) * q) + (bid >> 3);
    }
    int tn, tm;
    {
        const int GM = g.group_m > 1 ? g.group_m : 1;
        const int per_group = GM * ntn;
        const int grp = logical / per_group;
        const int first_m = grp * GM;
        const int gsz = min(GM, ntm - first_m);
        const int within = logical - grp * per_group;
        tm = first_m + within % gsz;
        tn = within / gsz;
    }
    const int m0 = tm * BM, n0 = tn * BN;
    const int img = m0 / (Hd * Wd);
    const int y0 = (m0 - img * Hd * Wd) / Wd;

    const T* a0p = reinterpret_cast<const T*>(g.a0);
    const T* a1p = reinterpret_cast<const T*>(g.a1);
    const T* wp = reinterpret_cast<const T*>(g.w);
    const long long a_rows = (long long)g.B * Hd * Wd;
    const __amdgpu_buffer_rsrc_t rw = make_rsrc(wp, (unsigned)min((long long)g.N * g.K * 2, 0x7FFFFFFFll));
    const __amdgpu_buffer_rsrc_t ra0 = make_rsrc(a0p, (unsigned)min(a_rows * g.lda0 * 2, 0x7FFFFFFFll));
    const __amdgpu_buffer_rsrc_t ra1 = make_rsrc(a1p ? (const void*)a1p : (const void*)a0p,
                                                 a1p ? (unsigned)min(a_rows * g.lda1 * 2, 0x7FFFFFFFll) : 0u);

    const int lrow = tid >> 3, pch = tid & 7;
    unsigned wvo[W_IT];
#pragma unroll
    for (int it = 0; it < W_IT; ++it) {
        const int row = it * (NT / 8) + lrow;
        const int n = min(n0 + min(row, BN - 1), g.N - 1);
        const int c = pch ^ (row & 7);
        wvo[it] = (unsigned)(((size_t)n * g.K + c * 8) * 2);
    }
    unsigned pvo0[PIT_MAX], pvo1[PIT_MAX];
#pragma unroll
    for (int it = 0; it < PIT_MAX; ++it) {
        const int t = it * NT + tid;
        const int pp = t >> 3;
        const int c = (t & 7) ^ (pp & 7);
        const int hy = pp / PW, hx = pp - hy * PW;
        const int iy = y0 - 1 + hy, ix = hx - 1;
        const bool ok = pp < npix && iy >= 0 && iy < Hd && ix >= 0 && ix < Wd;
        const unsigned pix = (unsigned)((img * Hd + iy) * Wd + ix);
        pvo0[it] = ok ? (pix * (unsigned)g.lda0 + (unsigned)c * 8u) * 2u : BL_OOB;
        pvo1[it] = ok ? (pix * (unsigned)g.lda1 + (unsigned)c * 8u) * 2u : BL_OOB;
    }

    const int Ct = g.c0 + g.c1;
    const int nch = Ct / BK;
    const int per = (nch + g.splitk - 1) / g.splitk;
    const int ch_beg = split * per, ch_end = min(nch, ch_beg + per);
    const int P = (ch_end - ch_beg) * 9;

    auto stage_patch = [&](int ch) {
        const int cc = ch * BK;
        const bool second = cc >= g.c0;
        const unsigned chb = (unsigned)(second ? cc - g.c0 : cc) * 2;
#pragma unroll
        for (int it = 0; it < PIT_MAX; ++it) {
            if (it < pit) {
                if (!second) bl16(ra0, patch + (it * NT + wave * 64) * 16, pvo0[it], chb);
                else bl16(ra1, patch + (it * NT + wave * 64) * 16, pvo1[it], chb);
            }
        }
    };
    auto stage_w = [&](int p) {
        const int ch = ch_beg + p / 9, tap = p - (p / 9) * 9;
        char* sb = wbase + (p % NSTAGE) * WSTAGE;
        const unsigned kb = (unsigned)(tap * Ct + ch * BK) * 2;
#pragma unroll
        for (int it = 0; it < W_IT; ++it) bl16(rw, sb + (it * NT + wave * 64) * 16, wvo[it], kb);
    };

    f32x4 acc[NF][MF];
#pragma unroll
    for (int i = 0; i < NF; ++i)
#pragma unroll
        for (int j = 0; j < MF; ++j) acc[i][j] = f32x4{0.f, 0.f, 0.f, 0.f};

    const int wm0 = (wave / WGN) * WTM, wn0 = (wave % WGN) * WTN;
    const int fr = lane & 15, fg = lane >> 4;
    int prow[MF];
#pragma unroll
    for (int j = 0; j < MF; ++j) {
        const int p = wm0 + j * 16 + fr;
        const int ty = p / Wd, tx = p - ty * Wd;
        prow[j] = ty * PW + tx;
    }

    auto compute = [&](int p) {
        const char* sw = wbase + (p % NSTAGE) * WSTAGE;
        const int tap = p - (p / 9) * 9;
        const int ky = tap / 3, kx = tap - ky * 3;
        const int toff = ky * PW + kx;
#pragma unroll
        for (int kk = 0; kk < 2; ++kk) {
            const int physw = ((kk * 4 + fg) ^ (fr & 7)) * 16;
            bf16x8 wf[NF], af[MF];
#pragma unroll
            for (int i = 0; i < NF; ++i) wf[i] = *reinterpret_cast<const bf16x8*>(sw + (wn0 + i * 16 + fr) * 128 + physw);
#pragma unroll
            for (int j = 0; j < MF; ++j) {
                const int pr = prow[j] + toff;
                af[j] = *reinterpret_cast<const bf16x8*>(patch + pr * 128 + (((kk * 4 + fg) ^ (pr & 7)) * 16));
            }
#pragma unroll
            for (int i = 0; i < NF; ++i)
#pragma unroll
                for (int j = 0; j < MF; ++j) acc[i][j] = __builtin_amdgcn_mfma_f32_16x16x32_bf16(wf[i], af[j], acc[i][j], 0, 0, 0);
        }
    };

    if (P > 0) {
#pragma unroll
        for (int d = 0; d < D; ++d)
            if (d < P) stage_w(d);
        stage_patch(ch_beg);
        asm volatile("s_waitcnt vmcnt(0)" ::: "memory");
        __syncthreads();
        for (int p = 0; p < P; ++p) {
            if (p + D < P) stage_w(p + D);
            compute(p);
            const int tap = p - (p / 9) * 9;
            if (tap == 8 && p + 1 < P) {
                asm volatile("s_waitcnt lgkmcnt(0)" ::: "memory");
                __builtin_amdgcn_s_barrier();
                stage_patch(ch_beg + (p + 1) / 9);
                asm volatile("s_waitcnt vmcnt(0)" ::: "memory");
            } else {
                const int young = min(D - 1, P - 2 - p);
                if (young >= 2) asm volatile("s_waitcnt vmcnt(%0)" ::"n"(2 * W_IT) : "memory");
                else if (young == 1) asm volatile("s_waitcnt vmcnt(%0)" ::"n"(W_IT) : "memory");
                else asm volatile("s_waitcnt vmcnt(0)" ::: "memory");
            }
            asm volatile("s_waitcnt lgkmcnt(0)" ::: "memory");
            __builtin_amdgcn_s_barrier();
        }
        __syncthreads();
    }

    if (g.splitk > 1) {
        float* part = g.partial + (size_t)split * (size_t)g.M * g.N;
#pragma unroll
        for (int i = 0; i < NF; ++i)
#pragma unroll
            for (int j = 0; j < MF; ++j) {
                const int m = m0 + wm0 + j * 16 + fr;
                const int n = n0 + wn0 + i * 16 + fg * 4;
                if (m < g.M && n < g.N) {
                    float v[4] = {acc[i][j][0], acc[i][j][1], acc[i][j][2], acc[i][j][3]};
                    store4<float>(part + (size_t)m * g.N + n, v);
                }
            }
        return;
    }
    constexpr int OPITCH = BN + 8;
    T* otile = reinterpret_cast<T*>(smem);
    const bool staged = g.out_mode == OUT_ROWS && (g.ldo & 7) == 0 && (size_t)BM * OPITCH * 2 <= (size_t)pit * (NT * 16) + NSTAGE * WSTAGE && g.stage_out > 1;
    const bool resid_later = staged && g.resid != nullptr && (g.ldr & 7) == 0 && g.stage_out < 3;
    float pb[NF][4];
    preload_cols<NF>(g, n0 + wn0 + fg * 4, pb);
#pragma unroll
    for (int i = 0; i < NF; ++i)
#pragma unroll
        for (int j = 0; j < MF; ++j) {
            const int m = m0 + wm0 + j * 16 + fr;
// ... 887 lines not shown
                for (int i = 0; i < NF1; ++i) dst[i] = *reinterpret_cast<const bf16x8*>(s1 + i * 16 * (K * 2) + off);
            };
#pragma unroll
            for (int kk = 0; kk < PF; ++kk) load_w(wf[kk], kk);
#pragma unroll
            for (int kk = 0; kk < KS; ++kk) {
                if (q + 1 < NQ) {
                    stageP(q + 1, buf ^ 1, kk);
                    if (kk == 1) { load_x(q + 1, xvn); load_b(q + 1, pbpn); }
                }
                __builtin_amdgcn_sched_barrier(0);
                if (kk + PF < KS) load_w(wf[(kk + PF) % (PF + 1)], kk + PF);
#pragma unroll
                for (int i = 0; i < NF1; ++i)
#pragma unroll
                    for (int j = 0; j < MF; ++j) {
                        const f32x4 cz = kk == 0 ? f32x4{pbp[i][0], pbp[i][1], pbp[i][2], pbp[i][3]} : acc3[i][j];
                        acc3[i][j] = __builtin_amdgcn_mfma_f32_16x16x32_bf16(wf[kk % (PF + 1)][i], t2[j][kk], cz, 0, 0, 0);
                    }
                if (kk + PF < KS) {
#pragma unroll
                    for (int u = 0; u < NF1; ++u) {
                        __builtin_amdgcn_sched_group_barrier(0x008, 2, 0);
                        __builtin_amdgcn_sched_group_barrier(0x100, 1, 0);
                    }
                }
                __builtin_amdgcn_sched_barrier(0);
            }
#pragma unroll
            for (int i = 0; i < NF1; ++i)
#pragma unroll
                for (int j = 0; j < MF; ++j) {
                    const int m = m0 + wave * 32 + j * 16 + fr;
                    bf16x4 o;
#pragma unroll
                    for (int r = 0; r < 4; ++r) {
                        const bf16 v = (bf16)acc3[i][j][r];
                        o[r] = (bf16)((float)v + (float)xv[i][j][r]);
                    }
                    if (m < a.M) *reinterpret_cast<bf16x4*>(ob2 + (size_t)m * a.ldo2 + q * 64 + i * 16 + fg * 4) = o;
                }
        }
        return;
    }
    asm volatile("s_waitcnt vmcnt(0)" ::: "memory");
    __syncthreads();
    constexpr int OP = N2 + 8;
    T* wt = reinterpret_cast<T*>(smem + wave * (32 * OP * 2));
#pragma unroll
    for (int i = 0; i < NF2; ++i)
#pragma unroll
        for (int j = 0; j < MF; ++j) {
            const bf16x4 o = {(bf16)acc2[i][j][0], (bf16)acc2[i][j][1], (bf16)acc2[i][j][2], (bf16)acc2[i][j][3]};
            *reinterpret_cast<bf16x4*>(wt + (j * 16 + fr) * OP + i * 16 + fg * 4) = o;
        }
    asm volatile("s_waitcnt lgkmcnt(0)" ::: "memory");
    constexpr int CPRO = N2 / 8;
    T* ob = reinterpret_cast<T*>(a.out);
    const T* rb = reinterpret_cast<const T*>(a.resid);
    constexpr int ITO = 32 * CPRO / 64, OB = 5;
    static_assert(32 * CPRO % 64 == 0 && ITO % OB == 0, "whole batches");
    for (int it0 = 0; it0 < ITO; it0 += OB) {
        bf16x8 rv[OB];
#pragma unroll
        for (int u = 0; u < OB; ++u) {
            const int idx = (it0 + u) * 64 + lane;
            const int row = idx / CPRO, ch = idx - row * CPRO;
            const int m = m0 + wave * 32 + row;
            if (rb && m < a.M) rv[u] = *reinterpret_cast<const bf16x8*>(rb + (size_t)m * a.ldr + ch * 8);
        }
#pragma unroll
        for (int u = 0; u < OB; ++u) {
            const int idx = (it0 + u) * 64 + lane;
            const int row = idx / CPRO, ch = idx - row * CPRO;
            const int m = m0 + wave * 32 + row;
            if (m >= a.M) continue;
            bf16x8 v = *reinterpret_cast<const bf16x8*>(wt + row * OP + ch * 8);
            if (rb) {
#pragma unroll
                for (int e = 0; e < 8; ++e) v[e] = (bf16)((float)v[e] + (float)rv[u][e]);
            }
            *reinterpret_cast<bf16x8*>(ob + (size_t)m * a.ldo + ch * 8) = v;
        }
    }
}

__global__ void pack_mlp_w2_kernel(const bf16* __restrict__ src, bf16* __restrict__ dst, int N2, int H) {
    const long long total = (long long)N2 * H;
    for (long long i = blockIdx.x * 256ll + threadIdx.x; i < total; i += (long long)gridDim.x * 256) {
        const int n = (int)(i / H), k = (int)(i - (long long)n * H);
        const int blk = k & ~31, pos = k & 31, fgp = pos >> 3, e = pos & 7;
        const int srck = blk + (e < 4 ? 4 * fgp + e : 16 + 4 * fgp + (e - 4));
        dst[i] = src[(size_t)n * H + srck];
    }
}
int launch_pack_mlp_w2(const void* w2_bf16, void* dst, int N2, int H, hipStream_t st) {
    MRISR_REQUIRE(H % 32 == 0, "fused feed-forward: hidden width a multiple of 32");
    hipLaunchKernelGGL(pack_mlp_w2_kernel, dim3(1024), dim3(256), 0, st, reinterpret_cast<const bf16*>(w2_bf16), reinterpret_cast<bf16*>(dst), N2, H);
    MRISR_CHECK_HIP(hipGetLastError());
    return 0;
}
#define MLP_PROBES(X) X(0) X(1) X(2) X(4) X(8) X(12) X(14) X(15)
static int g_mlp_proj = -1;
extern "C" void mrisr_debug_mlp_proj(int on) { g_mlp_proj = on; }
bool mlp_proj_enabled() {
    static const int env = [] { const char* e = getenv("MRISR_MLP_PROJ"); return e ? atoi(e) : 1; }();
    return g_mlp_proj < 0 ? env != 0 : g_mlp_proj != 0;
}
bool mlp_fused_ok(int C, int H, int N2) {
    static const int env = [] { const char* e = getenv("MRISR_MLP_FUSED"); return e ? atoi(e) : 1; }();
    return env && C == 320 && N2 == 320 && H % 32 == 0 && H >= 64;
}
constexpr int kMlpSmem = 2 * (64 * 320 * 2) + 2 * (320 * 64);
static int mlp_fused_prepare() {
    static bool attr = false;
    if (!attr) {
#define MLP_ATTR(D) MRISR_CHECK_HIP(hipFuncSetAttribute((const void*)mlp_fused_kernel<10, D>, hipFuncAttributeMaxDynamicSharedMemorySize, kMlpSmem));
        MLP_PROBES(MLP_ATTR)
#undef MLP_ATTR
        MRISR_CHECK_HIP(hipFuncSetAttribute((const void*)mlp_fused_kernel<10, 0, true>, hipFuncAttributeMaxDynamicSharedMemorySize, kMlpSmem));
        attr = true;
    }
    return 0;
}
int launch_mlp_fused(const MlpArgs& m, hipStream_t st) {
    MRISR_REQUIRE(mlp_fused_ok(m.C, m.H, m.N2), "fused feed-forward: C = N2 = 320");
    MRISR_REQUIRE(m.x && m.w1 && m.w2p && m.out && m.ln_gamma && m.ln_beta && m.ldx % 8 == 0 && m.ldo % 8 == 0 && (!m.resid || m.ldr % 8 == 0),
                  "fused feed-forward: operands");
    MRISR_REQUIRE((size_t)std::max(2 * m.H, m.N2) * sizeof(float) <= kZeroPageBytes, "fused feed-forward: bias-free form beyond the zero page");
    constexpr int smem = kMlpSmem;
    static const int dbg = [] { const char* e = getenv("MRISR_MLP_DBG"); return e ? atoi(e) : 0; }();
    if (mlp_fused_prepare()) return 1;
    MlpDev d;
    d.x = m.x; d.ldx = m.ldx; d.M = m.M; d.ln_gamma = m.ln_gamma; d.ln_beta = m.ln_beta; d.ln_eps = m.ln_eps;
    d.w1 = m.w1; d.b1 = m.b1 ? m.b1 : static_cast<const float*>(zero_page());
    d.w2p = m.w2p; d.b2 = m.b2 ? m.b2 : static_cast<const float*>(zero_page());
    d.resid = m.resid; d.ldr = m.ldr; d.out = m.out; d.ldo = m.ldo; d.H = m.H;
    d.wp = m.wp; d.bp = m.wp ? (m.bp ? m.bp : static_cast<const float*>(zero_page())) : nullptr;
    d.xres = m.xres; d.ldxr = m.ldxr; d.out2 = m.out2; d.ldo2 = m.ldo2;
    MRISR_REQUIRE(!m.wp || (m.xres && m.out2 && m.ldxr % 4 == 0 && m.ldo2 % 4 == 0 && m.M % 128 == 0), "fused feed-forward + proj_out: operands (whole 128-row panels)");
    d.poison = (gemm_flags_now() & 2048) ? 1 : 0;
    static const int rot = [] { const char* e = getenv("MRISR_MLP_ROT"); return e ? atoi(e) : 1; }();
    static const int spread = [] { const char* e = getenv("MRISR_MLP_SPREAD"); return e ? atoi(e) : 1; }();
    d.rot = rot; d.spread = spread;
    const double fl = 2.0 * m.M * ((double)2 * m.H * m.C + (double)m.H * m.N2);
    const double by = 2.0 * ((double)m.M * m.C * (m.resid ? 3 : 2) + 3.0 * m.H * m.C);
    ProfScope ps("mlp_fused_c320", fl, by, st);
    bool launched = false;
#define MLP_GO(D) if (dbg == D && !(D == 0 && d.wp)) { hipLaunchKernelGGL((mlp_fused_kernel<10, D>), dim3((m.M + 127) / 128), dim3(256), smem, st, d); launched = true; }
    MLP_PROBES(MLP_GO)
#undef MLP_GO
    if (dbg == 0 && d.wp) { hipLaunchKernelGGL((mlp_fused_kernel<10, 0, true>), dim3((m.M + 127) / 128), dim3(256), smem, st, d); launched = true; }
    MRISR_REQUIRE(dbg == 0 || !d.wp, "MRISR_MLP_DBG probes: without the proj_out continuation (MRISR_MLP_PROJ=0)");
    MRISR_REQUIRE(launched, "MRISR_MLP_DBG: no such probe build");
    MRISR_CHECK_HIP(hipGetLastError());
    return 0;
}

template <typename T>
__global__ __launch_bounds__(256) void splitk_reduce_kernel(const GemmArgs g) {
    const int nq = g.N >> 2;
    const long long total = (long long)g.M * nq;
    const int z = blockIdx.z;
    for (long long i = blockIdx.x * 256ll + threadIdx.x; i < total; i += (long long)gridDim.x * 256) {
        const int m = (int)(i / nq);
        const int n = (int)(i - (long long)m * nq) * 4;
        float v[4] = {0.f, 0.f, 0.f, 0.f};
        const float* p = g.partial + (size_t)z * g.splitk * (size_t)g.M * g.N + (size_t)m * g.N + n;
        const bool fast = g.out_mode == OUT_ROWS && !g.lora_z && g.heads == 1 && g.batch == 1;
        float b4[4] = {0.f, 0.f, 0.f, 0.f}, t4[4] = {0.f, 0.f, 0.f, 0.f}, r4[4] = {0.f, 0.f, 0.f, 0.f};
        if (fast) {
            if (g.bias) load4<float>(g.bias + n, b4);
            if (g.rowvec) load4<float>(g.rowvec + (size_t)(m / g.rowvec_div) * g.rowvec_ld + n, t4);
            if (g.resid) load4<T>(reinterpret_cast<const T*>(g.resid) + (size_t)m * g.ldr + n, r4);
        }
        for (int s = 0; s < g.splitk; ++s) {
            float t[4];
            load4<float>(p + (size_t)s * g.M * g.N, t);
#pragma unroll
            for (int r = 0; r < 4; ++r) v[r] += t[r];
        }
        if (fast) {
#pragma unroll
            for (int r = 0; r < 4; ++r) v[r] = v[r] * g.alpha + b4[r];
            if (g.rowvec) {
#pragma unroll
                for (int r = 0; r < 4; ++r) v[r] += t4[r];
            }
            if (g.act == ACT_RELU) {
#pragma unroll
                for (int r = 0; r < 4; ++r) v[r] = fmaxf(v[r], 0.f);
            } else if (g.act == ACT_SILU) {
#pragma unroll
                for (int r = 0; r < 4; ++r) v[r] = silu_f(v[r]);
            }
            if (g.resid) {
#pragma unroll
                for (int r = 0; r < 4; ++r) v[r] += r4[r];
            }
            store4<T>(reinterpret_cast<T*>(g.out) + (size_t)m * g.ldo + n, v);
            continue;
        }
        epilogue4<T>(g, z, m, n, v, nullptr, nullptr, nullptr, false, false);
    }
}

enum class Fam { F32, BL, HALO, HALO8, WS, RP };
#define TILES(X)                                   \
    X(1, F32, 128, 128, 2, 2, 2, 0.75, false)      \
    X(2, F32, 256, 64, 4, 1, 2, 0.65, false)       \
    X(3, F32, 128, 64, 2, 2, 2, 0.60, false)       \
    X(4, F32, 64, 64, 2, 2, 2, 0.45, false)        \
    X(14, BL, 128, 128, 2, 2, 2, 1.00, true)       \
    X(15, BL, 256, 64, 4, 1, 2, 0.90, true)        \
    X(16, BL, 128, 64, 2, 2, 2, 0.88, true)        \
    X(17, BL, 64, 64, 2, 2, 2, 0.60, true)         \
    X(18, BL, 64, 128, 2, 2, 2, 0.86, true)        \
    X(25, BL, 128, 160, 2, 2, 2, 0, true)          \
    X(26, BL, 64, 160, 2, 2, 2, 0, true)           \
    X(27, BL, 160, 160, 2, 2, 2, 0, false)         \
    X(28, BL, 128, 192, 2, 2, 2, 0, true)          \
    X(29, BL, 192, 128, 2, 2, 2, 0, false)         \
    X(30, BL, 160, 128, 2, 2, 2, 0, false)         \
    X(31, BL, 96, 160, 2, 2, 2, 0, false)          \
    X(32, BL, 64, 64, 2, 2, 4, 0, false)           \
    X(33, BL, 64, 64, 2, 2, 3, 0, false)           \
    X(34, BL, 64, 128, 2, 2, 3, 0, false)          \
    X(35, BL, 128, 64, 2, 2, 3, 0, false)          \
    X(36, BL, 128, 128, 2, 2, 3, 0, false)         \
    X(37, BL, 128, 160, 2, 2, 4, 0, false)         \
    X(38, BL, 128, 128, 2, 2, 4, 0, false)         \
    X(39, BL, 64, 160, 2, 2, 3, 0, false)          \
    X(41, HALO, 128, 160, 2, 2, 2, 0, true)        \
    X(42, HALO, 128, 128, 2, 2, 2, 0, true)        \
    X(43, HALO, 64, 160, 2, 2, 2, 0, true)         \
    X(44, HALO, 128, 192, 2, 2, 2, 0, true)        \
    X(45, HALO, 256, 64, 4, 1, 2, 0, true)         \
    X(46, HALO8, 256, 160, 4, 2, 2, 0, false)      \
    X(47, HALO8, 256, 160, 4, 2, 3, 0, false)      \
    X(48, HALO8, 256, 160, 4, 2, 4, 0, false)      \
    X(50, WS, 10, 10, 0, 0, 0, 0, false)           \
    X(51, WS, 10, 8, 0, 0, 0, 0, false)            \
    X(52, WS, 20, 4, 0, 0, 0, 0, false)            \
    X(60, RP, 10, 4, 0, 4, 0, 0, true)             \
    X(61, RP, 20, 2, 0, 4, 0, 0, true)             \
    X(62, RP, 10, 4, 1, 4, 0, 0, false)            \
    X(63, RP, 20, 4, 1, 2, 0, 0, false)            \
    X(64, RP, 20, 2, 0, 2, 0, 0, true)             \
    X(65, RP, 10, 4, 0, 2, 0, 0, true)
#define TILE_LAUNCH_F32(a, b, c, d, e) launch_cfg<T, a, b, c, d>
#define TILE_LAUNCH_BL(a, b, c, d, e) launch_bl<a, b, c, d, e>
#define TILE_LAUNCH_HALO(a, b, c, d, e) launch_halo<a, b, c, d>
#define TILE_LAUNCH_HALO8(a, b, c, d, e) launch_halo8<b, e>
#define TILE_LAUNCH_WS(a, b, c, d, e) launch_ws<a, b>
#define TILE_LAUNCH_RP(a, b, c, d, e) launch_rp<a, b, (c) != 0, d>

struct Tile {
    int id;
    Fam fam;
    int p[5];
    double eff;
    bool cand;
    constexpr bool tiled() const { return fam == Fam::F32 || fam == Fam::BL || fam == Fam::HALO || fam == Fam::HALO8; }
    constexpr int bm() const { return tiled() ? p[0] : (fam == Fam::WS ? 64 : 32 * p[3]); }
    constexpr int bn() const { return tiled() ? p[1] : 16 * p[1]; }
    constexpr int nstage() const { return tiled() ? p[4] : 1; }
    constexpr int ks() const { return tiled() ? 0 : p[0]; }
    constexpr bool fp8() const { return fam == Fam::RP && p[2] != 0; }
    constexpr int nw() const { return fam == Fam::RP ? p[3] : 0; }
    constexpr int mfrag() const { return tiled() ? p[0] / p[2] / 16 : 0; }
    constexpr int nfrag() const { return tiled() ? p[1] / p[3] / 16 : p[1]; }
    constexpr bool pairs_geglu() const { return nfrag() % 2 == 0; }
    constexpr bool ring() const { return fam == Fam::BL && nstage() > 2; }
    constexpr bool knows_gather2x2() const { return fam == Fam::BL && nstage() == 2; }
    constexpr bool carries_tail() const { return knows_gather2x2() || fam == Fam::HALO; }
    constexpr bool splits() const { return tiled(); }
    constexpr bool reduces_in_kernel() const { return (fam == Fam::BL || fam == Fam::HALO) && mfrag() * nfrag() <= 20; }
    constexpr int lora_max_rank() const { return fam == Fam::BL || fam == Fam::WS || fam == Fam::RP ? 16 : 0; }
    constexpr bool lora_rank4_only() const { return fam == Fam::RP; }
};
#define X(id, fam, a, b, c, d, e, eff, cand) {id, Fam::fam, {a, b, c, d, e}, eff, cand},
static constexpr Tile kTiles[] = {TILES(X)};
#undef X
static constexpr const Tile* find_tile(int id) {
    for (const Tile& t : kTiles)
        if (t.id == id) return &t;
    return nullptr;
}
static constexpr int kTileF32 = 1, kTileBL = 14, kTileGather2x2 = 25;
static constexpr bool registry_ok() {
    for (const Tile& a : kTiles) {
        if (a.id <= 0 || find_tile(a.id) != &a) return false;
        if (a.cand && a.fam == Fam::F32) return false;
    }
    return find_tile(kTileF32)->fam == Fam::F32 && find_tile(kTileBL)->knows_gather2x2() && find_tile(kTileGather2x2)->knows_gather2x2();
}
static_assert(registry_ok(), "tile registry: unique ids, bf16 candidates, default tiles of the right family");

bool gemm_tile_lora_in_kernel(int tile, int r, int R) {
    const Tile* t = find_tile(tile);
    return t && R >= 1 && R <= t->lora_max_rank() && (!t->lora_rank4_only() || r == 4);
}

static int auto_group_m(int ntm) {
    static const int env = [] { const char* e = getenv("MRISR_GROUP_M"); return e ? atoi(e) : 8; }();
    return std::max(1, std::min(env, ntm));
}
static dim3 tile_grid(GemmArgs& g, int BM, int BN) {
    const int ntn = (g.N + BN - 1) / BN, ntm = (g.M + BM - 1) / BM;
    g.group_m = auto_group_m(ntm);
    return dim3(ntn * ntm, g.splitk, g.batch);
}
static ProfScope gemm_scope(const GemmArgs& g, const std::string& base, const char* tag, double a_el, int elt, int w_elt, hipStream_t st) {
    if (!prof_enabled()) return ProfScope(base.c_str(), 0.0, 0.0, st);
    const char* name = base.c_str();
    if (tag && prof_shapes()) {
        char buf[160];
        snprintf(buf, sizeof(buf), "%s %s M=%d N=%d K=%d s=%d b=%d", name, tag, g.M, g.N, g.K, g.splitk, g.batch);
        name = prof_intern(buf);
    }
    const double fl = g.alg_flops != 0.0 ? g.alg_flops : 2.0 * g.M * (double)g.N * g.K * g.batch;
    const double by = g.alg_bytes != 0.0 ? g.alg_bytes : g.batch * (elt * (a_el + (double)g.M * g.N) + w_elt * ((double)g.N * g.K));
    return ProfScope(name, fl, by, st);
}
static double conv_a_elements(const GemmArgs& g, bool with_tail) { return (double)g.B * g.Hin * g.Win * (g.c0 + g.c1 + (with_tail ? g.cs0 + g.cs1 : 0)); }

template <typename T, int BM, int BN, int WGM, int WGN>
static int prepare_cfg() {
    constexpr int smem = 2 * (BM + BN) * 128;
    static bool attr_set = false;
    if (!attr_set) {
        auto kern = gemm_kernel<T, BM, BN, WGM, WGN>;
        MRISR_CHECK_HIP(hipFuncSetAttribute((const void*)kern, hipFuncAttributeMaxDynamicSharedMemorySize, smem));
        attr_set = true;
    }
    return 0;
}
template <typename T, int BM, int BN, int WGM, int WGN>
static int launch_cfg(GemmArgs& g, hipStream_t st) {
    constexpr int smem = 2 * (BM + BN) * 128;
    auto kern = gemm_kernel<T, BM, BN, WGM, WGN>;
    if (prepare_cfg<T, BM, BN, WGM, WGN>()) return 1;
    const dim3 grid = tile_grid(g, BM, BN);
    static const std::string base = std::string("gemm_") + (sizeof(T) == 2 ? "bf16_" : "f32_") + std::to_string(BM) + "x" + std::to_string(BN);
    ProfScope ps = gemm_scope(g, base, nullptr, g.conv ? conv_a_elements(g, false) : (double)g.M * g.K, sizeof(T), sizeof(T), st);
    hipLaunchKernelGGL(kern, grid, dim3(256), smem, st, g, (const char*)zero_page());
    MRISR_CHECK_HIP(hipGetLastError());
    return 0;
}

static int g_force_tile = 0;
extern "C" void mrisr_debug_force_tile(int t) { g_force_tile = t; }

template <int BM, int BN, int WGM, int WGN, int NSTAGE>
static int prepare_bl() {
    constexpr int smem = NSTAGE * (BM + BN) * 128;
    constexpr int smem_l = NSTAGE * ((BM + BN) * 128 + 16 * 128);
    static bool done = false;
    if (!done) {
        MRISR_CHECK_HIP(hipFuncSetAttribute((const void*)gemm_bl_kernel<BM, BN, WGM, WGN, NSTAGE, false>, hipFuncAttributeMaxDynamicSharedMemorySize, smem));
        MRISR_CHECK_HIP(hipFuncSetAttribute((const void*)gemm_bl_kernel<BM, BN, WGM, WGN, NSTAGE, true>, hipFuncAttributeMaxDynamicSharedMemorySize, smem_l));
        done = true;
    }
    return 0;
}
template <int BM, int BN, int WGM, int WGN, int NSTAGE>
static int launch_bl(GemmArgs& g, hipStream_t st) {
    constexpr int smem = NSTAGE * (BM + BN) * 128;
    constexpr int smem_l = NSTAGE * ((BM + BN) * 128 + 16 * 128);
    if (prepare_bl<BM, BN, WGM, WGN, NSTAGE>()) return 1;
    const dim3 grid = tile_grid(g, BM, BN);
    static const std::string base = std::string("gemm_bf16_bl") + std::to_string(BM) + "x" + std::to_string(BN) + (NSTAGE > 2 ? "d" + std::to_string(NSTAGE) : std::string());
    ProfScope ps = gemm_scope(g, base, g.conv ? (g.cs0 ? "convsc" : (g.ups ? "convup" : (g.stride == 2 ? "convs2" : "conv"))) : "lin",
                              g.conv ? conv_a_elements(g, true) : (double)g.M * g.K, 2, 2, st);
    if (g.lora_a) hipLaunchKernelGGL((gemm_bl_kernel<BM, BN, WGM, WGN, NSTAGE, true>), grid, dim3(256), smem_l, st, g);
    else hipLaunchKernelGGL((gemm_bl_kernel<BM, BN, WGM, WGN, NSTAGE, false>), grid, dim3(256), smem, st, g);
    MRISR_CHECK_HIP(hipGetLastError());
    return 0;
}

static size_t halo_smem(const GemmArgs& g, int BM, int BN) {
    const int TH = BM / g.Win;
    const size_t npix = (size_t)(TH + 2) * (g.Win + 2);
    const size_t patch = (npix * 8 + 255) / 256 * 4096;
    return patch + 2 * (size_t)BN * 128;
}
template <int BM, int BN, int WGM, int WGN>
static int launch_halo(GemmArgs& g, hipStream_t st) {
    const size_t smem = halo_smem(g, BM, BN);
    MRISR_REQUIRE(smem <= 160 * 1024, "halo conv kernel: LDS");
    static size_t attr = 0;
    if (smem > attr) {
        MRISR_CHECK_HIP(hipFuncSetAttribute((const void*)gemm_halo_kernel<BM, BN, WGM, WGN>, hipFuncAttributeMaxDynamicSharedMemorySize, (int)(96 * 1024)));
        attr = 96 * 1024;
    }
    const dim3 grid = tile_grid(g, BM, BN);
    static const std::string base = std::string("gemm_bf16_halo") + std::to_string(BM) + "x" + std::to_string(BN);
    ProfScope ps = gemm_scope(g, base, g.cs0 ? "convsc" : "conv", conv_a_elements(g, true), 2, 2, st);
    hipLaunchKernelGGL((gemm_halo_kernel<BM, BN, WGM, WGN>), grid, dim3(256), smem, st, g);
    MRISR_CHECK_HIP(hipGetLastError());
    return 0;
}
template <int BN, int NSTAGE>
static int launch_halo8(GemmArgs& g, hipStream_t st) {
    const int npix = (256 / g.Win + 2) * (g.Win + 2);
    const size_t smem = (size_t)((npix * 8 + 511) / 512) * 8192 + (size_t)NSTAGE * ((BN * 8 + 511) / 512) * 8192;
    MRISR_REQUIRE(smem <= 160 * 1024, "256-row halo conv kernel: LDS");
    static bool attr = false;
    if (!attr) {
        MRISR_CHECK_HIP(hipFuncSetAttribute((const void*)gemm_halo8_kernel<BN, NSTAGE>, hipFuncAttributeMaxDynamicSharedMemorySize, 160 * 1024));
        attr = true;
    }
    const dim3 grid = tile_grid(g, 256, BN);
    static const std::string base = std::string("gemm_bf16_halo256x") + std::to_string(BN) + "r" + std::to_string(NSTAGE);
    ProfScope ps = gemm_scope(g, base, "conv", conv_a_elements(g, false), 2, 2, st);
    hipLaunchKernelGGL((gemm_halo8_kernel<BN, NSTAGE>), grid, dim3(512), smem, st, g);
    MRISR_CHECK_HIP(hipGetLastError());
    return 0;
}

template <int KS, int NB>
static int launch_ws(GemmArgs& g, hipStream_t st) {
    constexpr int K = KS * 32, BN = NB * 16, WP = K * 2 + 16;
    const bool lora = g.lora_a != nullptr;
    const size_t smem = (size_t)(BN + (lora ? 16 : 0)) * WP + (lora ? 4 * 16 * 16 * sizeof(float) : 0);
    static bool attr = false;
    if (!attr) {
        MRISR_CHECK_HIP(hipFuncSetAttribute((const void*)gemm_ws_kernel<KS, NB, false>, hipFuncAttributeMaxDynamicSharedMemorySize, 150 * 1024));
        MRISR_CHECK_HIP(hipFuncSetAttribute((const void*)gemm_ws_kernel<KS, NB, true>, hipFuncAttributeMaxDynamicSharedMemorySize, 150 * 1024));
        attr = true;
    }
    MRISR_REQUIRE(smem <= 150 * 1024, "weight-stationary kernel: LDS");
    const int slabs = g.N / BN, nblk = g.M / 64;
    int rgroups = 256 / slabs;
    if (rgroups < 1) rgroups = 1;
    if (rgroups > nblk) rgroups = nblk;
    static const std::string base = std::string("gemm_bf16_ws") + std::to_string(K) + "x" + std::to_string(BN);
    ProfScope ps = gemm_scope(g, base, "lin", (double)g.M * g.K, 2, 2, st);
    if (lora) hipLaunchKernelGGL((gemm_ws_kernel<KS, NB, true>), dim3(slabs * rgroups), dim3(256), smem, st, g, rgroups);
    else hipLaunchKernelGGL((gemm_ws_kernel<KS, NB, false>), dim3(slabs * rgroups), dim3(256), smem, st, g, rgroups);
    MRISR_CHECK_HIP(hipGetLastError());
    return 0;
}

template <int KS, int NF, bool FP8, int NW>
static int launch_rp(GemmArgs& g, hipStream_t st) {
    constexpr int K = KS * 32, BN = NF * 16, BM = 32 * NW;
    constexpr int smem = (FP8 && KS == 10) ? 81920 : 2 * BN * K * (FP8 ? 1 : 2);
    static bool attr = false;
    if (!attr) {
        MRISR_CHECK_HIP(hipFuncSetAttribute((const void*)gemm_rp_kernel<KS, NF, false, 0, FP8, NW>, hipFuncAttributeMaxDynamicSharedMemorySize, smem));
        MRISR_CHECK_HIP(hipFuncSetAttribute((const void*)gemm_rp_kernel<KS, NF, false, 1, FP8, NW>, hipFuncAttributeMaxDynamicSharedMemorySize, smem));
        MRISR_CHECK_HIP(hipFuncSetAttribute((const void*)gemm_rp_kernel<KS, NF, true, 0, FP8, NW>, hipFuncAttributeMaxDynamicSharedMemorySize, smem));
        MRISR_CHECK_HIP(hipFuncSetAttribute((const void*)gemm_rp_kernel<KS, NF, true, 1, FP8, NW>, hipFuncAttributeMaxDynamicSharedMemorySize, smem));
        attr = true;
    }
    const int panels = (g.M + BM - 1) / BM, nchunks = (g.N + BN - 1) / BN;
    static const int ys_env = [] { const char* e = getenv("MRISR_RP_YSPLIT"); return e ? atoi(e) : 0; }();
    int ysplit = ys_env > 0 ? ys_env : (512 + panels / 2) / panels;
    ysplit = std::max(1, std::min(ysplit, nchunks));
    static const std::string base = std::string(FP8 ? "gemm_fp8_rp" : "gemm_bf16_rp") + std::to_string(K) + "x" + std::to_string(BN) + (NW == 2 ? "w2" : "");
    ProfScope ps = gemm_scope(g, base, g.ln_gamma ? "lin+ln" : "lin", (double)g.M * g.K, 2, FP8 ? 1 : 2, st);
    const dim3 grid(panels, ysplit);
    static const int pt_rp = [] { const char* e = getenv("MRISR_PRETOUCH_RP"); return e ? atoi(e) : 1; }();
    if (!pt_rp) g.pretouch = 0;
    const bool lora = g.lora_a != nullptr;
    if (!g.bias) g.bias = static_cast<const float*>(zero_page());
    if (g.ln_gamma) {
        MRISR_REQUIRE(g.ln_beta, "LayerNorm prologue: gamma and beta");
        if (lora) hipLaunchKernelGGL((gemm_rp_kernel<KS, NF, true, 1, FP8, NW>), grid, dim3(64 * NW), smem, st, g);
        else hipLaunchKernelGGL((gemm_rp_kernel<KS, NF, false, 1, FP8, NW>), grid, dim3(64 * NW), smem, st, g);
    } else {
        if (lora) hipLaunchKernelGGL((gemm_rp_kernel<KS, NF, true, 0, FP8, NW>), grid, dim3(64 * NW), smem, st, g);
        else hipLaunchKernelGGL((gemm_rp_kernel<KS, NF, false, 0, FP8, NW>), grid, dim3(64 * NW), smem, st, g);
    }
    MRISR_CHECK_HIP(hipGetLastError());
    return 0;
}

static bool bl_ok(const GemmArgs& g) {
    const long long a_rows = g.conv ? (long long)g.B * g.Hin * g.Win : (long long)g.M;
    const long long lim = 0x7FFFFFFFll;
    return a_rows * g.lda0 * 2 < lim && a_rows * (long long)g.lda1 * 2 < lim && (long long)g.N * g.K * 2 < lim;
}
bool gemm_sc_tail_ok(const GemmArgs& g) {
    if (!g.conv || g.kw != 3 || g.subpix || g.stride != 1 || g.ups || g.zstuff || g.pad != 1 || g.batch != 1) return false;
    if (g.Hout != g.Hin || g.Wout != g.Win || g.act == ACT_GEGLU || g.lora_a) return false;
    if (!g.s0 || g.cs0 <= 0 || g.cs0 % 64 || g.cs1 % 64 || (g.cs1 > 0) != (g.s1 != nullptr) || g.c0 % 64 || g.c1 % 64) return false;
    if (g.lds0 < g.cs0 || (g.s1 && g.lds1 < g.cs1) || (g.lds0 & 7) || (g.lds1 & 7)) return false;
    const long long a_rows = (long long)g.B * g.Hin * g.Win, lim = 0x7FFFFFFFll;
    return bl_ok(g) && a_rows * g.lds0 * 2 < lim && a_rows * (long long)g.lds1 * 2 < lim;
}
static bool halo_geometry_ok(const GemmArgs& g, int BM, int nt, int pit_max) {
    if (!g.conv || g.stride != 1 || g.ups != 0 || g.zstuff || g.batch != 1 || g.pad != 1) return false;
    if (g.Win % 8 != 0 || g.Win > 64 || BM % g.Win != 0) return false;
    if ((g.Hin * g.Win) % BM != 0 || g.M % BM != 0 || g.Hout != g.Hin || g.Wout != g.Win) return false;
    const int npix = (BM / g.Win + 2) * (g.Win + 2);
    return (npix * 8 + nt - 1) / nt <= pit_max && g.N % 4 == 0;
}
static bool rp_form_ok(const GemmArgs& g, const Tile& t) {
    if (g.no_rp || g.heads != 1 || g.lda0 % 8 != 0 || g.N % 16 != 0 || g.M < 1) return false;
    if (g.alpha != 1.0f || g.rowvec || g.lora_z || (!g.bias && (size_t)g.N * sizeof(float) > kZeroPageBytes)) return false;
    if (t.fp8() != (g.w8 != nullptr)) return false;
    if (t.fp8() && (!g.w_scale || (g.lora_a && (!g.lora_a8 || !g.lora_a_scale)))) return false;
    if (g.act == ACT_GEGLU) {
        if (g.N % 32 != 0 || g.out_mode != OUT_ROWS || g.ldo % 8 != 0 || g.resid) return false;
    } else if (g.act != ACT_NONE) {
        return false;
    } else if (g.out_mode == OUT_ROWS) {
        if (g.ldo % 8 != 0 || (g.resid && g.ldr % 8 != 0)) return false;
    } else if (g.out_mode == OUT_HEADS) {
        if (g.secC <= 0 || g.secC % t.bn() != 0 || ((g.N | g.M | g.hd | g.secC | g.dpad | g.npad | g.ntok) & 7) != 0 || g.resid) return false;
    } else {
        return false;
    }
    return true;
}
static bool tile_admits(const GemmArgs& g, bool is_bf16, int tile, const char** why) {
    auto no = [why](const char* reason) { if (why) *why = reason; return false; };
    const Tile* t = find_tile(tile);
    if (!t) return no("no such tile id");
    if (t->fam != Fam::F32 && !(is_bf16 && bl_ok(g))) return no("f32, or an operand of 2 GiB and more: the f32-capable tiled kernels only");
    if ((g.kw != 3 || g.subpix) && !t->knows_gather2x2()) return no("2 x 2 / sub-pixel conv: only the 2-stage buffer-addressed kernel's gather knows these forms");
    if (g.cs0 || g.cs1 || g.s0 || g.s1) {
        if (!t->carries_tail()) return no("1x1 tail: only the 2-stage buffer-addressed kernels and the 4-wave halo kernels carry it");
        if (!is_bf16 || !gemm_sc_tail_ok(g)) return no("1x1 tail: bf16 stride-1 3x3 conv, channel counts multiples of 64, operands below 2 GiB");
    }
    if (g.act == ACT_GEGLU && !t->pairs_geglu())
        return no("GEGLU epilogue: this tile has an odd number of fragments per wave along N, so no (u, gate) fragment pairing");
    if (g.splitk > 1 && !t->splits()) return no("the weight-stationary and row-panel kernels have no split-K");
    if (g.lora_a && !(g.splitk <= 1 && !g.conv && g.c1 == 0 && g.lora_b && g.act != ACT_GEGLU && gemm_tile_lora_in_kernel(tile, g.lora_r, g.lora_R)))
        return no("in-kernel LoRA down-projection: plain un-split GEMM on a buffer-addressed, weight-stationary or row-panel tile, R <= 16 (row-panel: rank 4 per module)");
    const bool plain = !g.conv && !g.c1 && !g.a1 && g.batch == 1;
    switch (t->fam) {
        case Fam::F32: break;
        case Fam::BL:
            if (t->ring() && !(plain && g.M % t->bm() == 0 && g.N % t->bn() == 0 && (g.splitk == 1 || (g.K / 64) / g.splitk >= t->nstage())))
                return no("counted-ring GEMM: plain single-source GEMM that tiles exactly; split: at least NSTAGE K tiles per split");
            break;
        case Fam::HALO:
            if (!halo_geometry_ok(g, t->bm(), 256, t->bm() >= 256 ? 13 : (t->bm() >= 128 ? 9 : 6))) return no("halo conv kernel: unsupported geometry");
            break;
        case Fam::HALO8:
            if (!halo_geometry_ok(g, t->bm(), 512, 7)) return no("256-row halo conv kernel: unsupported geometry");
            break;
        case Fam::WS:
            if (!(plain && g.K == 32 * t->ks() && g.N % t->bn() == 0 && g.M % 64 == 0 && g.lda0 % 8 == 0 && g.out_mode != OUT_NONE))
                return no("weight-stationary kernel: plain rows, K = 32*KS, N a multiple of the slab, M a multiple of 64");
            break;
        case Fam::RP:
            if (!(plain && g.K == 32 * t->ks() && rp_form_ok(g, *t)))
                return no("row-panel kernel: plain un-split bf16 row GEMM with K = 32*KS (fp8: packed weights + scales)");
            break;
    }
    return true;
}
static int tile_for_launch(const GemmArgs& g, bool is_bf16, int tile) {
    const bool bl = is_bf16 && bl_ok(g);
    const Tile* t = find_tile(tile);
    if (!t || (t->fam != Fam::F32 && !bl)) t = find_tile(kTileF32);
    if ((g.kw != 3 || g.subpix) && !t->knows_gather2x2()) t = find_tile(kTileGather2x2);
    if (g.splitk > 1 && !t->splits()) t = find_tile(bl ? kTileBL : kTileF32);
    return t->id;
}
int gemm_rp_tile(const GemmArgs& g) {
    static const int env = [] { const char* e = getenv("MRISR_RP"); return e ? atoi(e) : 1; }();
    if (!env) return 0;
    const int want_nw = (!g.w8 && g.K == 640 && g.N <= 640) ? 2 : 4;
    int best = 0;
    for (const Tile& t : kTiles)
        if (t.fam == Fam::RP && (!best || t.nw() == want_nw) && tile_admits(g, true, t.id, nullptr)) best = t.id;
    return best;
}
static int g_sc_fused = -1;
extern "C" void mrisr_debug_sc_fused(int on) { g_sc_fused = on; ++g_plan_salt; }
bool sc_fused_enabled() {
    static const int env = [] { const char* e = getenv("MRISR_SC_FUSED"); return e ? atoi(e) : 1; }();
    return g_sc_fused < 0 ? env != 0 : g_sc_fused != 0;
}
static int g_ff_proj_fused = -1;
extern "C" void mrisr_debug_ff_proj_fused(int on) { g_ff_proj_fused = on; ++g_plan_salt; }
bool ff_proj_fused_enabled() {
    static const int env = [] { const char* e = getenv("MRISR_FF_PROJ_FUSED"); return e ? atoi(e) : 1; }();
    return g_ff_proj_fused < 0 ? env != 0 : g_ff_proj_fused != 0;
}

static double g_tile_eff[32] = {0};
extern "C" void mrisr_debug_set_tile_eff(int id, double eff) { if (id >= 0 && id < 32) g_tile_eff[id] = eff; }

static bool plan_admits_split(const GemmArgs& g, int s, int nkt) { return g.act != ACT_GEGLU && nkt / s >= 6; }
static bool tune_admits_split(const GemmArgs& g, const Tile& t, int s, int nkt, long long t128) {
    return g.act != ACT_GEGLU && nkt / s >= 4 && t128 * s <= 4096 && t.splits() && !t.ring() && g.kw == 3 && !g.subpix;
}

static void plan(const GemmArgs& g, bool is_bf16, int fixed_split, int* tile_out, int* split_out) {
    const double cu_flops = 1.0e15 / 256.0 * 1e-6;
    double best = 1e300;
    int bt = is_bf16 ? kTileBL : kTileF32, bs = 1;
    const int nkt = g.K / (is_bf16 ? 64 : 32);
    const Fam fam = is_bf16 && bl_ok(g) ? Fam::BL : Fam::F32;
    for (const Tile& t : kTiles) {
        if (t.fam != fam || t.eff <= 0) continue;
        const double eff = g_tile_eff[t.id] > 0 ? g_tile_eff[t.id] : t.eff;
        const long long tiles = (long long)((g.M + t.bm() - 1) / t.bm()) * ((g.N + t.bn() - 1) / t.bn()) * g.batch;
        for (int s = 1; s <= 32; s *= 2) {
            if (fixed_split > 0 && s != fixed_split) continue;
            if (s > 1 && !plan_admits_split(g, s, nkt)) break;
            const long long blocks = tiles * s;
            const long long rounds = (blocks + 511) / 512;
            const double wg_us = 2.0 * t.bm() * t.bn() * ((double)g.K / s) / (cu_flops * eff) * 2.0 + 4.0;
            double cost = rounds * wg_us;
            if (s > 1) cost += 2.0 + (double)g.M * g.N * g.batch * (4.0 * s * 2 + 2) / 3.0e6;
            if (cost < best) { best = cost; bt = t.id; bs = s; }
        }
    }
    if (fixed_split > 0 && best >= 1e300) bs = fixed_split;
    *tile_out = bt;
    *split_out = bs;
}

__global__ void tune_fill_kernel(bf16* p, long long n, unsigned seed) {
    for (long long i = blockIdx.x * 256ll + threadIdx.x; i < n; i += (long long)gridDim.x * 256) {
        unsigned x = (unsigned)i * 2654435761u + seed;
        x ^= x >> 15; x *= 2246822519u; x ^= x >> 13;
        p[i] = (bf16)(((float)(x & 0xFFFF) / 32768.0f - 1.0f) * 0.5f);
    }
}
struct TuneScratch {
    void* p[6] = {nullptr, nullptr, nullptr, nullptr, nullptr, nullptr};
    size_t cap[6] = {0, 0, 0, 0, 0, 0};
    int reserve(int i, size_t bytes, bool randomize) {
        if (bytes <= cap[i]) return 0;
        if (p[i]) (void)hipFree(p[i]);
        p[i] = nullptr; cap[i] = 0;
        bytes = (bytes + (1 << 20)) & ~(size_t)((1 << 20) - 1);
        MRISR_CHECK_HIP(hipMalloc(&p[i], bytes));
        cap[i] = bytes;
        if (randomize) hipLaunchKernelGGL(tune_fill_kernel, dim3(2048), dim3(256), 0, nullptr, (bf16*)p[i], (long long)(bytes / 2), 17u + i);
        else MRISR_CHECK_HIP(hipMemset(p[i], 0, bytes));
        return 0;
    }
    void release() {
        for (int i = 0; i < 6; ++i) { if (p[i]) (void)hipFree(p[i]); p[i] = nullptr; cap[i] = 0; }
    }
};
static TuneScratch g_ts;
static std::map<std::string, std::pair<int, int>> g_tuned;
static int g_tune_count = 0;
static double g_tune_ms = 0.0;
extern "C" int mrisr_autotune_stats(int* shapes, double* ms) { if (shapes) *shapes = g_tune_count; if (ms) *ms = g_tune_ms; return 0; }
extern "C" void mrisr_autotune_release(void) { g_ts.release(); }

static bool autotune_enabled() {
    static int v = -1;
    if (v < 0) { const char* e = getenv("MRISR_AUTOTUNE"); v = (e && e[0] == '0') ? 0 : 1; }
    return v == 1;
}
int mrisr_prof_enable_internal(int on);

template <typename T> int launch_gemm(const GemmArgs& g, hipStream_t st);

static int tune(const GemmArgs& g0, int* tile_out, int* split_out) {
    char key[200];
    snprintf(key, sizeof(key), "%d,%d,%d,c%d,s%d,u%d,%d,%d,a%d,o%d,b%d,r%d,v%d,h%d,w%d", g0.M, g0.N, g0.K, g0.conv, g0.stride + 8 * (1 - g0.pad), g0.ups, g0.c0,
             g0.c1, g0.act, g0.out_mode, g0.batch, g0.resid ? 1 : 0, g0.rowvec ? 1 : 0, g0.Hin, g0.Win);
    if (g0.kw != 3 || g0.subpix) snprintf(key + strlen(key), sizeof(key) - strlen(key), ",q%d", g0.kw * 2 + g0.subpix);
    if (g0.cs0) snprintf(key + strlen(key), sizeof(key) - strlen(key), ",t%d,%d", g0.cs0, g0.cs1);
    static bool cache_loaded = false;
    const char* cache_path = getenv("MRISR_TUNE_CACHE");
    if (!cache_loaded) {
        cache_loaded = true;
        if (cache_path) {
            if (FILE* f = fopen(cache_path, "r")) {
                char k[256];
                int t, sp;
                while (fscanf(f, "%255[^\t]\t%d\t%d\n", k, &t, &sp) == 3) g_tuned[k] = {t, sp};
                fclose(f);
            }
        }
    }
    auto it = g_tuned.find(key);
    if (it != g_tuned.end()) { *tile_out = it->second.first; *split_out = it->second.second; return 0; }
    GemmArgs g = g0;
    const long long a_rows = g.conv ? (long long)g.B * g.Hin * g.Win : (long long)g.M;
    const size_t zb = (size_t)(g.batch > 1 ? g.batch : 1);
    if (g_ts.reserve(0, (size_t)a_rows * std::max(g.lda0, g.lds0) * 2 * zb + 4096, true)) return 1;
    if ((g.c1 || g.cs1) && g_ts.reserve(1, (size_t)a_rows * std::max(g.lda1, g.lds1) * 2 + 4096, true)) return 1;
    if (g_ts.reserve(2, (size_t)g.N * g.K * 2 * zb + 4096, true)) return 1;
    if (g_ts.reserve(3, (size_t)g.M * g.N * 4 * zb + 4096, false)) return 1;
    if (g_ts.reserve(5, (size_t)(g.N + 64) * 4 + ((size_t)(g.rowvec ? g.M / (g.rowvec_div > 0 ? g.rowvec_div : 1) + 1 : 1)) * (g.N + 64) * 4, false)) return 1;
    g.a0 = g_ts.p[0]; g.a_bs = g.batch > 1 ? (long long)a_rows * g.lda0 : 0;
    g.a1 = g.c1 ? g_ts.p[1] : nullptr;
    if (g.cs0) { g.s0 = g_ts.p[0]; g.s1 = g.cs1 ? g_ts.p[1] : nullptr; }
    g.w = g_ts.p[2]; g.w_bs = g.batch > 1 ? (long long)g.N * g.K : 0;
    g.bias = g.bias ? (const float*)g_ts.p[5] : nullptr;
    if (g.rowvec) { g.rowvec = (const float*)g_ts.p[5] + g.N + 64; g.rowvec_ld = g.N + 64; }
    g.heads = 1; g.o_hs = 0; g.o_bs = g.batch > 1 ? (long long)g.M * g.N : 0;
    if (g.out_mode == OUT_HEADS) g.out_mode = OUT_ROWS;
    g.out = g_ts.p[3]; g.ldo = g.act == ACT_GEGLU ? g.N / 2 : g.N;
    if (g.resid) { g.resid = g_ts.p[3]; g.ldr = g.ldo; }
    g.lora_z = nullptr;
    g.lora_a = nullptr;
// ... 224 lines not shown
```

Measured before the change: 69.15 slices/s.

## Precompute GEMM kernel prologue into a compact head with magic-number divisions

Adds a 128-byte GemmHead computed on the host that holds tile counts, extents, flags and magic-multiplier constants, and passes it to the bl and halo GEMM kernels. The kernels pin the head in scalar registers and use multiply-shift division in place of integer division for tile coordinates and pixel decomposition. The weight stage (and pretouch) is also issued before the A-operand address setup, so the first weight loads overlap with that setup. This shortens the per-workgroup prologue, which matters for the many small GEMMs in the UNet, at the cost of an extra kernel argument and some added complexity. A debug pad-0 stride-2 conv option is added but is off by default.

```diff
diff --git a/include/mrisr_debug.h b/include/mrisr_debug.h
--- a/include/mrisr_debug.h
+++ b/include/mrisr_debug.h
@@ -9,6 +9,8 @@
 void mrisr_debug_prefer_tile(int tile);
 void mrisr_debug_gemm_flags(int flags);
 void mrisr_debug_gemm_stamps(void* dev_buf, int tile);
+void mrisr_debug_group_m(int group_m);
+void mrisr_debug_op_conv_pad0(int on);
 void mrisr_debug_set_tile_eff(int tile, double eff);
 void mrisr_debug_set_tuned(const char* key, int tile, int splitk);
 void mrisr_debug_gn_fused(int on);
diff --git a/mri-diffusion-superresolution_amd/csrc/capi_ops.hip b/mri-diffusion-superresolution_amd/csrc/capi_ops.hip
--- a/mri-diffusion-superresolution_amd/csrc/capi_ops.hip
+++ b/mri-diffusion-superresolution_amd/csrc/capi_ops.hip
@@ -44,6 +44,9 @@
         else dst[(bh * dpad + dd) * npad + tok] = x[i];
     }
 }
+
+static int g_op_conv_pad0 = 0;
+extern "C" void mrisr_debug_op_conv_pad0(int on) { g_op_conv_pad0 = on; }
 
 template <typename T>
 static int op_conv3x3_t(const mrisr_tensor* x, const mrisr_tensor* x2, const float* w, const float* bias, int cout,
@@ -82,7 +85,9 @@
     GemmArgs g;
     ga_rows(g, x->data, C0, C0);
     if (x2) ga_rows2(g, x2->data, C1, C1);
-    ga_conv3(g, B, H, W, stride, ups);
+    const bool pad0 = g_op_conv_pad0 && stride == 2 && !ups;
+    if (pad0) MRISR_REQUIRE(H % 2 == 0 && W % 2 == 0, "stride-2 conv with pad 0: even H and W");
+    ga_conv3(g, B, H, W, stride, ups, pad0 ? 0 : 1);
     MRISR_REQUIRE(y->shape[1] == cout && y->shape[2] == g.Hout && y->shape[3] == g.Wout, "conv output shape");
     ga_weight(g, wp.p, B * g.Hout * g.Wout, cout, 9 * Cin); g.bias = bias; g.act = act; ga_out(g, y->data, cout);
     TRY(op_plan<T>(g, splitk, false, part));
diff --git a/mri-diffusion-superresolution_amd/csrc/gemm.hip b/mri-diffusion-superresolution_amd/csrc/gemm.hip
--- a/mri-diffusion-superresolution_amd/csrc/gemm.hip
+++ b/mri-diffusion-superresolution_amd/csrc/gemm.hip
@@ -1,4 +1,5 @@
 #include "common.h"
+#include "gemm_head.h"
 #include "prof.h"
 
 #include <cstdio>
@@ -573,6 +574,17 @@
     }
 }
 
+__device__ __forceinline__ void pretouch_weights_head(const __amdgpu_buffer_rsrc_t& rw, const GemmHead& h, char* scratch, int wave, int lane) {
+    const unsigned wg = blockIdx.x + blockIdx.y * (h.ntn * h.ntm);
+    const unsigned pieces = (h.ext_w + 1023u) >> 10;
+    const unsigned first = wg * h.pt_per_wg + (unsigned)wave * h.pt_per_wave;
+    for (unsigned i = 0; i < h.pt_per_wave; ++i) {
+        const unsigned pc = first + i;
+        const unsigned off = pc < pieces ? (pc << 10) + (unsigned)lane * 16u : BL_OOB;
+        bl16(rw, scratch + ((wave * 2 + (i & 1)) << 10), off, 0u);
+    }
+}
+
 template <int NF, int MF>
 __device__ __forceinline__ bool splitk_last_arriver(const GemmArgs& g, f32x4 (&acc)[NF][MF], unsigned tile_idx, const float* slab0, int m_base, int n_base,
                                                     int fr, int fg, char* ticket_lds) {
@@ -609,7 +621,7 @@
 }
 
 template <int BM, int BN, int WGM, int WGN, int NSTAGE, bool LORA>
-__global__ __launch_bounds__(256, 2) void gemm_bl_kernel(const GemmArgs g) {
+__global__ __launch_bounds__(256, 2) void gemm_bl_kernel(const GemmHead hd, const GemmArgs g) {
     static_assert(NSTAGE >= 2 && NSTAGE <= 4, "2 (drain per tile), 3 or 4 (counted ring)");
     typedef bf16 T;
     constexpr int BK = 64;
@@ -625,49 +637,47 @@
     const int wave = __builtin_amdgcn_readfirstlane(tid >> 6);
     const int z = blockIdx.z;
     const int split = blockIdx.y;
+    GemmHead h = hd;
+    asm volatile("" : "+s"(h.w), "+s"(h.a0), "+s"(h.a1), "+s"(h.ext_w), "+s"(h.ext_a0), "+s"(h.ext_a1), "+s"(h.flags), "+s"(h.rows), "+s"(h.N),
+                 "+s"(h.wpitch), "+s"(h.lda0), "+s"(h.lda1), "+s"(h.c0));
+    asm volatile("" : "+s"(h.ntn), "+s"(h.ntm), "+s"(h.group_m), "+s"(h.mul_pg), "+s"(h.mul_gm), "+s"(h.mul_last), "+s"(h.shifts), "+s"(h.per),
+                 "+s"(h.Ct), "+s"(h.pt_per_wg), "+s"(h.pt_per_wave), "+s"(h.mul_hw), "+s"(h.mul_wd));
+    const void* lora_a = nullptr;
+    int lora_R = 0;
+    if constexpr (LORA) {
+        lora_a = g.lora_a;
+        lora_R = g.lora_R;
+        asm volatile("" : "+s"(lora_a), "+s"(lora_R));
+    }
+    const bool conv = (h.flags & GH_CONV) != 0;
     auto stamp = [&](int k, bool drain = false) {
         if constexpr (NSTAGE == 2) {
-            unsigned long long* const stp = gemm_stamp_word(g, k, k == 0);
-            if (stp && tid == 0) {
-                if (drain) asm volatile("s_waitcnt vmcnt(0) lgkmcnt(0)" ::: "memory");
-                *stp = __builtin_readcyclecounter();
+            if (k <= 1 ? (h.flags & GH_STAMPED) != 0 : g.stamps != nullptr) {
+                unsigned long long* const stp = gemm_stamp_word(g, k, k == 0);
+                if (stp && tid == 0) {
+                    if (drain) asm volatile("s_waitcnt vmcnt(0) lgkmcnt(0)" ::: "memory");
+                    *stp = __builtin_readcyclecounter();
+                }
             }
         }
     };
     stamp(0);
-    if (g.dbg & 2048) lds_poison(smem, (int)blockDim.x);
-
-    const int ntn = (g.N + BN - 1) / BN;
-    const int ntm = (g.M + BM - 1) / BM;
-    const int nblk = ntn * ntm;
-    int logical;
-    {
-        const int bid = blockIdx.x;
-        const int xcd = bid & 7, q = nblk >> 3, r = nblk & 7;
-        logical = (xcd < r ? xcd * (q + 1) : r * (q + 1) + (xcd - r) * q) + (bid >> 3);
-    }
-    int tn, tm;
-    {
-        const int GM = g.group_m > 1 ? g.group_m : 1;
-        const int per_group = GM * ntn;
-        const int grp = logical / per_group;
-        const int first_m = grp * GM;
-        const int gsz = min(GM, ntm - first_m);
-        const int within = logical - grp * per_group;
-        tm = first_m + within % gsz;
-        tn = within / gsz;
-    }
+    if (h.flags & 2048u) lds_poison(smem, (int)blockDim.x);
+
+    uint32_t tm_u, tn_u;
+    gh_tile_coords(h, blockIdx.x, tm_u, tn_u);
+    const int tm = (int)tm_u, tn = (int)tn_u;
     const int m0 = tm * BM, n0 = tn * BN;
-
-    const T* a0p = reinterpret_cast<const T*>(g.a0) + (size_t)z * g.a_bs;
-    const T* a1p = reinterpret_cast<const T*>(g.a1);
-    const T* wp = reinterpret_cast<const T*>(g.w) + (size_t)z * g.w_bs;
-    const long long a_rows = g.conv ? (long long)g.B * g.Hin * g.Win : (long long)g.M;
-    const __amdgpu_buffer_rsrc_t rw = make_rsrc(wp, (unsigned)min((long long)g.N * g.K * 2, 0x7FFFFFFFll));
-    const __amdgpu_buffer_rsrc_t ra0 = make_rsrc(a0p, (unsigned)min(a_rows * g.lda0 * 2, 0x7FFFFFFFll));
-    const __amdgpu_buffer_rsrc_t ra1 = make_rsrc(a1p ? (const void*)a1p : (const void*)a0p,
-                                                 a1p ? (unsigned)min(a_rows * g.lda1 * 2, 0x7FFFFFFFll) : 0u);
-
+    int kt_beg, kt_end;
+    gh_split_range(h.per, h.wpitch >> 7, (uint32_t)split, kt_beg, kt_end);
+
+    const T* wp = reinterpret_cast<const T*>(h.w);
+    const T* a0p = reinterpret_cast<const T*>(h.a0);
+    if (h.flags & GH_BATCHED) {
+        wp += (size_t)z * g.w_bs;
+        a0p += (size_t)z * g.a_bs;
+    }
+    const __amdgpu_buffer_rsrc_t rw = make_rsrc(wp, h.ext_w);
     const int lrow = tid >> 3, pch = tid & 7;
     unsigned wvo[W_IT];
 #pragma unroll
@@ -675,8 +685,33 @@
         const int row = it * 32 + lrow;
         const int n = n0 + row;
         const int c = pch ^ (row & 7);
-        wvo[it] = n < g.N ? (unsigned)(((size_t)n * g.K + c * 8) * 2) : BL_OOB;
-    }
+        wvo[it] = (unsigned)n < h.N ? (unsigned)n * h.wpitch + (unsigned)c * 16u : BL_OOB;
+    }
+    const __amdgpu_buffer_rsrc_t rl = make_rsrc(LORA ? lora_a : (const void*)wp, LORA ? (unsigned)lora_R * h.wpitch : 0u);
+    unsigned lvo = BL_OOB;
+    if (LORA && (wave < 2 || NSTAGE > 2)) {
+        const int row = (wave & 1) * 8 + (lane >> 3);
+        const int c = (lane & 7) ^ (row & 7);
+        if (row < lora_R) lvo = (unsigned)row * h.wpitch + (unsigned)c * 16u;
+        else if (NSTAGE > 2) lvo = (unsigned)(lora_R - 1) * h.wpitch + (unsigned)c * 16u;
+    }
+    auto stage_w = [&](int kt, int buf) {
+        char* sb = smem + buf * STAGE;
+        const unsigned k0b = (unsigned)kt * BK * 2;
+#pragma unroll
+        for (int it = 0; it < W_IT; ++it) bl16(rw, sb + BM * 128 + (it * 256 + wave * 64) * 16, wvo[it], k0b);
+        if (LORA && (wave < 2 || NSTAGE > 2)) bl16(rl, sb + (BM + BN) * 128 + (wave & 1) * 64 * 16, lvo, k0b);
+    };
+    if (kt_beg < kt_end) {
+        if constexpr (NSTAGE == 2) {
+            if (h.pt_per_wave) pretouch_weights_head(rw, h, smem + STAGE, wave, lane);
+        }
+        stage_w(kt_beg, 0);
+    }
+
+    const T* a1p = reinterpret_cast<const T*>(h.a1);
+    const __amdgpu_buffer_rsrc_t ra0 = make_rsrc(a0p, h.ext_a0);
+    const __amdgpu_buffer_rsrc_t ra1 = make_rsrc(a1p ? (const void*)a1p : (const void*)a0p, h.ext_a1);
     unsigned avo[A_IT], avo1[A_IT];
     int ab[A_IT], ay[A_IT], ax[A_IT];
 #pragma unroll
@@ -684,72 +719,56 @@
         const int row = it * 32 + lrow;
         const int m = m0 + row;
         const int c = pch ^ (row & 7);
-        const bool ok = m < g.M;
+        const bool ok = (unsigned)m < h.rows;
         avo[it] = avo1[it] = BL_OOB;
         ab[it] = -1;
         ay[it] = ax[it] = 0;
-        if (!g.conv) {
+        if (!conv) {
             if (ok) {
-                avo[it] = (unsigned)(((size_t)m * g.lda0 + c * 8) * 2);
-                avo1[it] = (unsigned)(((size_t)m * g.lda1 + c * 8) * 2);
+                avo[it] = ((unsigned)m * h.lda0 + (unsigned)c * 8u) * 2u;
+                avo1[it] = ((unsigned)m * h.lda1 + (unsigned)c * 8u) * 2u;
             }
         } else if (ok) {
-            const int hw = g.Hout * g.Wout;
-            const int b = m / hw;
-            const int rem = m - b * hw;
-            const int oy = rem / g.Wout;
-            ab[it] = b * g.Hin;
-            ay[it] = oy * g.stride - g.pad + (g.subpix ? (z >> 1) : 0);
-            ax[it] = (rem - oy * g.Wout) * g.stride - g.pad + (g.subpix ? (z & 1) : 0);
+            uint32_t b, oy, ox;
+            gh_row_pixel(h, (uint32_t)m, (uint32_t)(g.Hout * g.Wout), (uint32_t)g.Wout, b, oy, ox);
+            const bool subpix = (h.flags & GH_SUBPIX) != 0;
+            ab[it] = (int)b * g.Hin;
+            ay[it] = (int)oy * g.stride - g.pad + (subpix ? (z >> 1) : 0);
+            ax[it] = (int)ox * g.stride - g.pad + (subpix ? (z & 1) : 0);
         }
     }
     const int acb = pch * 16;
-    const __amdgpu_buffer_rsrc_t rl = make_rsrc(LORA ? g.lora_a : (const void*)wp, LORA ? (unsigned)((long long)g.lora_R * g.K * 2) : 0u);
-    unsigned lvo = BL_OOB;
-    if (LORA && (wave < 2 || NSTAGE > 2)) {
-        const int row = (wave & 1) * 8 + (lane >> 3);
-        const int c = (lane & 7) ^ (row & 7);
-        if (row < g.lora_R) lvo = (unsigned)(((size_t)row * g.K + c * 8) * 2);
-        else if (NSTAGE > 2) lvo = (unsigned)(((size_t)(g.lora_R - 1) * g.K + c * 8) * 2);
-    }
-
-    const int nkt = g.K / BK;
-    const int per = (nkt + g.splitk - 1) / g.splitk;
-    const int kt_beg = split * per;
-    const int kt_end = min(nkt, kt_beg + per);
-    const int Ct = g.c0 + g.c1;
-    const int Hc = g.Hin << g.ups, Wc = g.Win << g.ups;
+    const long long a_rows = conv ? (long long)g.B * g.Hin * g.Win : (long long)h.rows;
+    const int Ct = (int)h.Ct;
+    const int ups = (h.flags & GH_UPS) ? g.ups : 0;
+    const bool zstuff = (h.flags & GH_ZSTUFF) != 0;
     int tap = 0, cc = 0, seg_key = -1;
-    const int ntaps = g.kw * g.kw;
-    if (g.conv) {
+    int Hc = 0, Wc = 0, ntaps = 0;
+    if (conv) {
+        Hc = g.Hin << ups;
+        Wc = g.Win << ups;
+        ntaps = g.kw * g.kw;
         const int k0 = kt_beg * BK;
         tap = min(k0 / Ct, ntaps);
         cc = k0 - tap * Ct;
     }
 
-    auto stage_w = [&](int kt, int buf) {
-        char* sb = smem + buf * STAGE;
-        const unsigned k0b = (unsigned)kt * BK * 2;
-#pragma unroll
-        for (int it = 0; it < W_IT; ++it) bl16(rw, sb + BM * 128 + (it * 256 + wave * 64) * 16, wvo[it], k0b);
-        if (LORA && (wave < 2 || NSTAGE > 2)) bl16(rl, sb + (BM + BN) * 128 + (wave & 1) * 64 * 16, lvo, k0b);
-    };
     auto stage_a = [&](int kt, int buf) {
         char* sb = smem + buf * STAGE;
         const unsigned k0b = (unsigned)kt * BK * 2;
-        if (!g.conv) {
-            const bool second = kt * BK >= g.c0;
+        if (!conv) {
+            const bool second = kt * BK >= (int)h.c0;
             if (!second) {
 #pragma unroll
                 for (int it = 0; it < A_IT; ++it) bl16(ra0, sb + (it * 256 + wave * 64) * 16, avo[it], k0b);
             } else {
-                const unsigned kb = (unsigned)(kt * BK - g.c0) * 2;
+                const unsigned kb = (unsigned)(kt * BK - (int)h.c0) * 2;
 #pragma unroll
                 for (int it = 0; it < A_IT; ++it) bl16(ra1, sb + (it * 256 + wave * 64) * 16, avo1[it], kb);
             }
         } else {
             const bool tail = tap >= ntaps;
-            const int cfirst = tail ? +g.cs0 : +g.c0;
+            const int cfirst = tail ? +g.cs0 : (int)h.c0;
             const bool second = cc >= cfirst;
             const int key = tap * 2 + (second ? 1 : 0);
             if (key != seg_key) {
@@ -762,8 +781,8 @@
                     const int row = it * 32 + lrow;
                     const int c = pch ^ (row & 7);
                     const int iy = ay[it] + ky, ix = ax[it] + kx;
-                    const bool ok = ab[it] >= 0 && iy >= 0 && iy < Hc && ix >= 0 && ix < Wc && (!g.zstuff || ((iy | ix) & 1) == 0);
-                    const unsigned pix = (unsigned)((ab[it] + (iy >> g.ups)) * g.Win + (ix >> g.ups));
+                    const bool ok = ab[it] >= 0 && iy >= 0 && iy < Hc && ix >= 0 && ix < Wc && (!zstuff || ((iy | ix) & 1) == 0);
+                    const unsigned pix = (unsigned)((ab[it] + (iy >> ups)) * g.Win + (ix >> ups));
                     avo[it] = ok ? (pix * (unsigned)ld + (unsigned)c * 8u) * 2u : BL_OOB;
                 }
             }
@@ -786,6 +805,8 @@
     };
     auto stage = [&](int kt, int buf) { stage_w(kt, buf); stage_a(kt, buf); };
     (void)acb;
+    if (kt_beg < kt_end) stage_a(kt_beg, 0);
+    stamp(1);
 
     f32x4 acc[NF][MF];
 #pragma unroll
@@ -841,12 +862,8 @@
         }
     };
 
-    stamp(1);
-
     if constexpr (NSTAGE == 2) {
         if (kt_beg < kt_end) {
-            if (g.pretouch) pretouch_weights(rw, (long long)g.N * g.K * 2, smem + STAGE, wave, lane, g.pretouch);
-            stage(kt_beg, 0);
             asm volatile("s_waitcnt vmcnt(0)" ::: "memory");
             __syncthreads();
             stamp(2);
@@ -871,7 +888,7 @@
         constexpr int PER = A_IT + W_IT + (LORA ? 1 : 0);
         static_assert(PER * (NSTAGE - 2) <= 63, "vmcnt range");
 #pragma unroll
-        for (int s = 0; s < NSTAGE - 1; ++s)
+        for (int s = 1; s < NSTAGE - 1; ++s)
             if (kt_beg + s < kt_end) stage(kt_beg + s, s);
         int slot = 0;
         for (int kt = kt_beg; kt < kt_end; ++kt) {
@@ -1030,7 +1047,7 @@
 }
 
 template <int BM, int BN, int WGM, int WGN>
-__global__ __launch_bounds__(256, 2) void gemm_halo_kernel(const GemmArgs g) {
+__global__ __launch_bounds__(256, 2) void gemm_halo_kernel(const GemmHead hd, const GemmArgs g) {
     typedef bf16 T;
     constexpr int BK = 64;
     constexpr int W_IT = BN / 32;
@@ -1045,55 +1062,49 @@
     const int lane = tid & 63;
     const int wave = __builtin_amdgcn_readfirstlane(tid >> 6);
     const int split = blockIdx.y;
+    GemmHead h = hd;
+    asm volatile("" : "+s"(h.w), "+s"(h.a0), "+s"(h.a1), "+s"(h.ext_w), "+s"(h.ext_a0), "+s"(h.ext_a1), "+s"(h.flags), "+s"(h.rows), "+s"(h.N),
+                 "+s"(h.wpitch), "+s"(h.lda0), "+s"(h.lda1), "+s"(h.c0));
+    asm volatile("" : "+s"(h.ntn), "+s"(h.ntm), "+s"(h.group_m), "+s"(h.mul_pg), "+s"(h.mul_gm), "+s"(h.mul_last), "+s"(h.shifts), "+s"(h.per),
+                 "+s"(h.Ct), "+s"(h.pt_per_wg), "+s"(h.pt_per_wave), "+s"(h.mul_hw), "+s"(h.mul_wd));
+    asm volatile("" : "+s"(h.mul_pw), "+s"(h.geom), "+s"(h.per_sc));
     auto stamp = [&](int k, bool drain = false) {
-        unsigned long long* const stp = gemm_stamp_word(g, k, k == 0);
-        if (stp && tid == 0) {
-            if (drain) asm volatile("s_waitcnt vmcnt(0) lgkmcnt(0)" ::: "memory");
-            *stp = __builtin_readcyclecounter();
+        if (k <= 1 ? (h.flags & GH_STAMPED) != 0 : g.stamps != nullptr) {
+            unsigned long long* const stp = gemm_stamp_word(g, k, k == 0);
+            if (stp && tid == 0) {
+                if (drain) asm volatile("s_waitcnt vmcnt(0) lgkmcnt(0)" ::: "memory");
+                *stp = __builtin_readcyclecounter();
+            }
         }
     };
     stamp(0);
-    if (g.dbg & 2048) lds_poison(smem, (int)blockDim.x);
-    const int Wd = g.Win, Hd = g.Hin;
-    const int TH = BM / Wd, PW = Wd + 2;
+    if (h.flags & 2048u) lds_poison(smem, (int)blockDim.x);
+    const int Wd = (int)(h.geom & 255u), Hd = (int)h.rows;
+    const int TH = (int)(h.geom >> 8 & 255u), PW = (int)(h.geom >> 16 & 255u);
     const int npix = (TH + 2) * PW;
-    const int pit = (npix * 8 + 255) / 256;
+    const int pit = (int)(h.geom >> 24);
     char* patch = smem;
     char* wbase = smem + pit * 4096;
 
-    const int ntn = (g.N + BN - 1) / BN;
-    const int ntm = g.M / BM;
-    const int nblk = ntn * ntm;
-    int logical;
-    {
-        const int bid = blockIdx.x;
-        const int xcd = bid & 7, q = nblk >> 3, r = nblk & 7;
-        logical = (xcd < r ? xcd * (q + 1) : r * (q + 1) + (xcd - r) * q) + (bid >> 3);
-    }
-    int tn, tm;
-    {
-        const int GM = g.group_m > 1 ? g.group_m : 1;
-        const int per_group = GM * ntn;
-        const int grp = logical / per_group;
-        const int first_m = grp * GM;
-        const int gsz = min(GM, ntm - first_m);
-        const int within = logical - grp * per_group;
-        tm = first_m + within % gsz;
-        tn = within / gsz;
-    }
+    uint32_t tm_u, tn_u;
+    gh_tile_coords(h, blockIdx.x, tm_u, tn_u);
+    const int tm = (int)tm_u, tn = (int)tn_u;
     const int m0 = tm * BM, n0 = tn * BN;
-    const int img = m0 / (Hd * Wd);
-    const int y0 = (m0 - img * Hd * Wd) / Wd;
-
-    const T* a0p = reinterpret_cast<const T*>(g.a0);
-    const T* a1p = reinterpret_cast<const T*>(g.a1);
-    const T* wp = reinterpret_cast<const T*>(g.w);
-    const long long a_rows = (long long)g.B * Hd * Wd;
-    const __amdgpu_buffer_rsrc_t rw = make_rsrc(wp, (unsigned)min((long long)g.N * g.K * 2, 0x7FFFFFFFll));
-    const __amdgpu_buffer_rsrc_t ra0 = make_rsrc(a0p, (unsigned)min(a_rows * g.lda0 * 2, 0x7FFFFFFFll));
-    const __amdgpu_buffer_rsrc_t ra1 = make_rsrc(a1p ? (const void*)a1p : (const void*)a0p,
-                                                 a1p ? (unsigned)min(a_rows * g.lda1 * 2, 0x7FFFFFFFll) : 0u);
-
+    const int Ct = (int)h.Ct;
+    const int nch = Ct / BK;
+    int ch_beg, ch_end;
+    gh_split_range(h.per, (uint32_t)nch, (uint32_t)split, ch_beg, ch_end);
+    int sc_beg = 0, sc_end = 0;
+    if (h.flags & GH_TAIL) {
+        const int nsc = (int)(h.wpitch >> 7) - 9 * nch;
+        sc_beg = min(nsc, split * (int)h.per_sc);
+        sc_end = min(nsc, sc_beg + (int)h.per_sc);
+    }
+
+    const T* a0p = reinterpret_cast<const T*>(h.a0);
+    const T* a1p = reinterpret_cast<const T*>(h.a1);
+    const T* wp = reinterpret_cast<const T*>(h.w);
+    const __amdgpu_buffer_rsrc_t rw = make_rsrc(wp, h.ext_w);
     const int lrow = tid >> 3, pch = tid & 7;
     unsigned wvo[W_IT];
 #pragma unroll
@@ -1101,44 +1112,8 @@
         const int row = it * 32 + lrow;
         const int n = n0 + row;
         const int c = pch ^ (row & 7);
-        wvo[it] = n < g.N ? (unsigned)(((size_t)n * g.K + c * 8) * 2) : BL_OOB;
-    }
-    unsigned pvo0[PIT_MAX], pvo1[PIT_MAX];
-#pragma unroll
-    for (int it = 0; it < PIT_MAX; ++it) {
-        const int t = it * 256 + tid;
-        const int pp = t >> 3;
-        const int c = (t & 7) ^ (pp & 7);
-        const int hy = pp / PW, hx = pp - hy * PW;
-        const int iy = y0 - 1 + hy, ix = hx - 1;
-        const bool ok = pp < npix && iy >= 0 && iy < Hd && ix >= 0 && ix < Wd;
-        const unsigned pix = (unsigned)((img * Hd + iy) * Wd + ix);
-        pvo0[it] = ok ? (pix * (unsigned)g.lda0 + (unsigned)c * 8u) * 2u : BL_OOB;
-        pvo1[it] = ok ? (pix * (unsigned)g.lda1 + (unsigned)c * 8u) * 2u : BL_OOB;
-    }
-
-    const int Ct = g.c0 + g.c1;
-    const int nch = Ct / BK;
-    const int per = (nch + g.splitk - 1) / g.splitk;
-    const int ch_beg = split * per, ch_end = min(nch, ch_beg + per);
-    const int nsc = (g.cs0 + g.cs1) / BK;
-    const int per_sc = (nsc + g.splitk - 1) / g.splitk;
-    const int sc_beg = min(nsc, split * per_sc), sc_end = min(nsc, sc_beg + per_sc);
-    const __amdgpu_buffer_rsrc_t rs0 = make_rsrc(g.s0 ? g.s0 : (const void*)a0p, g.s0 ? (unsigned)min(a_rows * g.lds0 * 2, 0x7FFFFFFFll) : 0u);
-    const __amdgpu_buffer_rsrc_t rs1 = make_rsrc(g.s1 ? g.s1 : (const void*)a0p, g.s1 ? (unsigned)min(a_rows * g.lds1 * 2, 0x7FFFFFFFll) : 0u);
-
-    auto stage_patch = [&](int ch) {
-        const int cc = ch * BK;
-        const bool second = cc >= g.c0;
-        const unsigned chb = (unsigned)(second ? cc - g.c0 : cc) * 2;
-#pragma unroll
-        for (int it = 0; it < PIT_MAX; ++it) {
-            if (it < pit) {
-                if (!second) bl16(ra0, patch + (it * 256 + wave * 64) * 16, pvo0[it], chb);
-                else bl16(ra1, patch + (it * 256 + wave * 64) * 16, pvo1[it], chb);
-            }
-        }
-    };
+        wvo[it] = (unsigned)n < h.N ? (unsigned)n * h.wpitch + (unsigned)c * 16u : BL_OOB;
+    }
     auto stage_w = [&](int ch, int tap, int buf) {
         char* sb = wbase + buf * WSTAGE;
         const unsigned kb = (unsigned)(tap * Ct + ch * BK) * 2;
@@ -1151,6 +1126,53 @@
 #pragma unroll
         for (int it = 0; it < W_IT; ++it) bl16(rw, sb + (it * 256 + wave * 64) * 16, wvo[it], kb);
     };
+    const bool any_work = ch_beg < ch_end || sc_beg < sc_end;
+    if (any_work) {
+        if (h.pt_per_wave) pretouch_weights_head(rw, h, wbase + WSTAGE, wave, lane);
+        if (ch_beg < ch_end) stage_w(ch_beg, 0, 0);
+        else stage_w_sc(sc_beg, 0);
+    }
+
+    const int hw = Hd * Wd;
+    const int img = (int)magic_div((uint32_t)m0, h.mul_hw, gh_shift(h, GH_SH_HW));
+    const int y0 = (int)gh_div_wd(h, (uint32_t)(m0 - img * hw));
+    const __amdgpu_buffer_rsrc_t ra0 = make_rsrc(a0p, h.ext_a0);
+    const __amdgpu_buffer_rsrc_t ra1 = make_rsrc(a1p ? (const void*)a1p : (const void*)a0p, h.ext_a1);
+    unsigned pvo0[PIT_MAX], pvo1[PIT_MAX];
+#pragma unroll
+    for (int it = 0; it < PIT_MAX; ++it) {
+        const int t = it * 256 + tid;
+        const int pp = t >> 3;
+        const int c = (t & 7) ^ (pp & 7);
+        const int hy = (int)gh_div_pw(h, (uint32_t)pp), hx = pp - hy * PW;
+        const int iy = y0 - 1 + hy, ix = hx - 1;
+        const bool ok = pp < npix && iy >= 0 && iy < Hd && ix >= 0 && ix < Wd;
+        const unsigned pix = (unsigned)((img * Hd + iy) * Wd + ix);
+        pvo0[it] = ok ? (pix * h.lda0 + (unsigned)c * 8u) * 2u : BL_OOB;
+        pvo1[it] = ok ? (pix * h.lda1 + (unsigned)c * 8u) * 2u : BL_OOB;
+    }
+
+    auto stage_patch = [&](int ch) {
+        const int cc = ch * BK;
+        const bool second = cc >= (int)h.c0;
+        const unsigned chb = (unsigned)(second ? cc - (int)h.c0 : cc) * 2;
+#pragma unroll
+        for (int it = 0; it < PIT_MAX; ++it) {
+            if (it < pit) {
+                if (!second) bl16(ra0, patch + (it * 256 + wave * 64) * 16, pvo0[it], chb);
+                else bl16(ra1, patch + (it * 256 + wave * 64) * 16, pvo1[it], chb);
+            }
+        }
+    };
+    if (ch_beg < ch_end) stage_patch(ch_beg);
+    stamp(1);
+
+    const bool has_tail = (h.flags & GH_TAIL) != 0;
+    const long long a_rows = has_tail ? (long long)g.B * Hd * Wd : 0ll;
+    const void* const s0p = has_tail ? g.s0 : nullptr;
+    const void* const s1p = has_tail ? g.s1 : nullptr;
+    const __amdgpu_buffer_rsrc_t rs0 = make_rsrc(s0p ? s0p : (const void*)a0p, s0p ? (unsigned)min(a_rows * g.lds0 * 2, 0x7FFFFFFFll) : 0u);
+    const __amdgpu_buffer_rsrc_t rs1 = make_rsrc(s1p ? s1p : (const void*)a0p, s1p ? (unsigned)min(a_rows * g.lds1 * 2, 0x7FFFFFFFll) : 0u);
     unsigned spix[PIT_MAX];
     auto sc_setup = [&]() {
 #pragma unroll
@@ -1158,7 +1180,7 @@
             int t = it * 256 + tid;
             asm volatile("" : "+v"(t));
             const int pp = t >> 3;
-            const int hy = pp / PW, hx = pp - hy * PW;
+            const int hy = (int)gh_div_pw(h, (uint32_t)pp), hx = pp - hy * PW;
             const bool ok = hy >= 1 && hy <= TH && hx >= 1 && hx <= Wd;
             spix[it] = ok ? (unsigned)((img * Hd + y0 - 1 + hy) * Wd + hx - 1) : ~0u;
         }
@@ -1192,7 +1214,7 @@
 #pragma unroll
     for (int j = 0; j < MF; ++j) {
         const int p = wm0 + j * 16 + fr;
-        const int ty = p / Wd, tx = p - ty * Wd;
+        const int ty = (int)gh_div_wd(h, (uint32_t)p), tx = p - ty * Wd;
         prow[j] = ty * PW + tx;
     }
 
@@ -1218,15 +1240,10 @@
         }
     };
 
-    stamp(1);
-
-    if (ch_beg < ch_end || sc_beg < sc_end) {
+    if (any_work) {
         int cur = 0;
-        if (g.pretouch) pretouch_weights(rw, (long long)g.N * g.K * 2, wbase + WSTAGE, wave, lane, g.pretouch);
-        if (ch_beg < ch_end) stage_w(ch_beg, 0, 0);
-        else stage_w_sc(sc_beg, 0);
         for (int ch = ch_beg; ch < ch_end; ++ch) {
-            stage_patch(ch);
+            if (ch != ch_beg) stage_patch(ch);
             asm volatile("s_waitcnt vmcnt(0)" ::: "memory");
             __syncthreads();
             if (ch == ch_beg) stamp(2);
@@ -2720,8 +2737,11 @@
     return t && R >= 1 && R <= t->lora_max_rank() && (!t->lora_rank4_only() || r == 4);
 }
 
+static int g_group_m = 0;
+extern "C" void mrisr_debug_group_m(int gm) { g_group_m = gm; }
 static int auto_group_m(int ntm) {
     static const int env = [] { const char* e = getenv("MRISR_GROUP_M"); return e ? atoi(e) : 8; }();
+    if (g_group_m > 0) return g_group_m;
     return std::max(1, std::min(env, ntm));
 }
 static dim3 tile_grid(GemmArgs& g, int BM, int BN) {
@@ -2767,6 +2787,18 @@
     return 0;
 }
 
+static GemmHead gemm_head_for(const GemmArgs& g, int BM, int BN, bool halo) {
+    GemmHeadIn in;
+    in.w = g.w; in.a0 = g.a0; in.a1 = g.a1;
+    in.M = g.M; in.N = g.N; in.K = g.K; in.c0 = g.c0; in.c1 = g.c1; in.lda0 = g.lda0; in.lda1 = g.lda1;
+    in.conv = g.conv; in.B = g.B; in.Hin = g.Hin; in.Win = g.Win; in.Hout = g.Hout; in.Wout = g.Wout;
+    in.ups = g.ups; in.zstuff = g.zstuff; in.subpix = g.subpix;
+    in.cs0 = g.cs0; in.cs1 = g.cs1; in.splitk = g.splitk; in.batch = g.batch; in.group_m = g.group_m;
+    in.pretouch = g.pretouch; in.dbg = g.dbg; in.stamped = g.stamps != nullptr;
+    in.BM = BM; in.BN = BN; in.halo = halo;
+    return make_gemm_head(in);
+}
+
 static int g_force_tile = 0;
 extern "C" void mrisr_debug_force_tile(int t) { g_force_tile = t; }
 
@@ -2791,8 +2823,9 @@
     static const std::string base = std::string("gemm_bf16_bl") + std::to_string(BM) + "x" + std::to_string(BN) + (NSTAGE > 2 ? "d" + std::to_string(NSTAGE) : std::string());
     ProfScope ps = gemm_scope(g, base, g.conv ? (g.cs0 ? "convsc" : (g.ups ? "convup" : (g.stride == 2 ? "convs2" : "conv"))) : "lin",
                               g.conv ? conv_a_elements(g, true) : (double)g.M * g.K, 2, 2, st);
-    if (g.lora_a) hipLaunchKernelGGL((gemm_bl_kernel<BM, BN, WGM, WGN, NSTAGE, true>), grid, dim3(256), smem_l, st, g);
-    else hipLaunchKernelGGL((gemm_bl_kernel<BM, BN, WGM, WGN, NSTAGE, false>), grid, dim3(256), smem, st, g);
+    const GemmHead hd = gemm_head_for(g, BM, BN, false);
+    if (g.lora_a) hipLaunchKernelGGL((gemm_bl_kernel<BM, BN, WGM, WGN, NSTAGE, true>), grid, dim3(256), smem_l, st, hd, g);
+    else hipLaunchKernelGGL((gemm_bl_kernel<BM, BN, WGM, WGN, NSTAGE, false>), grid, dim3(256), smem, st, hd, g);
     MRISR_CHECK_HIP(hipGetLastError());
     return 0;
 }
@@ -2815,7 +2848,7 @@
     const dim3 grid = tile_grid(g, BM, BN);
     static const std::string base = std::string("gemm_bf16_halo") + std::to_string(BM) + "x" + std::to_string(BN);
     ProfScope ps = gemm_scope(g, base, g.cs0 ? "convsc" : "conv", conv_a_elements(g, true), 2, 2, st);
-    hipLaunchKernelGGL((gemm_halo_kernel<BM, BN, WGM, WGN>), grid, dim3(256), smem, st, g);
+    hipLaunchKernelGGL((gemm_halo_kernel<BM, BN, WGM, WGN>), grid, dim3(256), smem, st, gemm_head_for(g, BM, BN, true), g);
     MRISR_CHECK_HIP(hipGetLastError());
     return 0;
 }
diff --git a/mri-diffusion-superresolution_amd/csrc/gemm_head.h b/mri-diffusion-superresolution_amd/csrc/gemm_head.h
--- /dev/null
+++ b/mri-diffusion-superresolution_amd/csrc/gemm_head.h
@@ -0,0 +1,151 @@
+#pragma once
+#include <cstdint>
+
+#if defined(__HIPCC__) || defined(__CUDACC__)
+#define MRISR_GH_HD __host__ __device__ __forceinline__
+#else
+#define MRISR_GH_HD inline
+#endif
+
+namespace mrisr {
+
+struct MagicDiv {
+    uint32_t mul;
+    uint32_t l;
+};
+inline MagicDiv magic_for(uint32_t d) {
+    MagicDiv m{0x80000000u, 0u};
+    if (d <= 1) return m;
+    uint32_t l = 0;
+    while ((1ull << l) < d) ++l;
+    m.l = l;
+    m.mul = (uint32_t)(((1ull << (31 + l)) + d - 1) / d);
+    return m;
+}
+MRISR_GH_HD uint32_t magic_div(uint32_t x, uint32_t mul, uint32_t l) { return (uint32_t)(((uint64_t)x * mul) >> (31u + l)); }
+
+enum : uint32_t {
+    GH_DBG_MASK = 0xFFFFu,
+    GH_CONV = 1u << 16,
+    GH_SUBPIX = 1u << 17,
+    GH_ZSTUFF = 1u << 18,
+    GH_UPS = 1u << 19,
+    GH_A1 = 1u << 20,
+    GH_TAIL = 1u << 21,
+    GH_STAMPED = 1u << 22,
+    GH_BATCHED = 1u << 23,
+};
+enum { GH_SH_PG = 0, GH_SH_GM = 5, GH_SH_LAST = 10, GH_SH_HW = 15, GH_SH_WD = 20, GH_SH_PW = 25 };
+
+struct GemmHead {
+    const void* w;
+    const void* a0;
+    const void* a1;
+    uint32_t ext_w, ext_a0, ext_a1;
+    uint32_t flags;
+    uint32_t rows;
+    uint32_t N;
+    uint32_t wpitch;
+    uint32_t lda0, lda1;
+    uint32_t c0;
+    uint32_t ntn, ntm;
+    uint32_t group_m;
+    uint32_t mul_pg, mul_gm, mul_last;
+    uint32_t shifts;
+    uint32_t per;
+    uint32_t Ct;
+    uint32_t pt_per_wg, pt_per_wave;
+    uint32_t mul_hw, mul_wd, mul_pw;
+    uint32_t geom;
+    uint32_t per_sc;
+};
+static_assert(sizeof(GemmHead) == 128, "the head is two 64-byte lines");
+
+MRISR_GH_HD uint32_t gh_shift(const GemmHead& h, int field) { return (h.shifts >> field) & 31u; }
+
+struct GemmHeadIn {
+    const void *w = nullptr, *a0 = nullptr, *a1 = nullptr;
+    int M = 0, N = 0, K = 0, c0 = 0, c1 = 0, lda0 = 0, lda1 = 0;
+    int conv = 0, B = 0, Hin = 0, Win = 0, Hout = 0, Wout = 0, ups = 0, zstuff = 0, subpix = 0;
+    int cs0 = 0, cs1 = 0, splitk = 1, batch = 1, group_m = 1, pretouch = 0, dbg = 0, stamped = 0;
+    int BM = 64, BN = 64, halo = 0;
+};
+
+static inline uint32_t gh_clamp_extent(long long bytes) { return (uint32_t)(bytes < 0x7FFFFFFFll ? bytes : 0x7FFFFFFFll); }
+
+inline GemmHead make_gemm_head(const GemmHeadIn& in) {
+    GemmHead h{};
+    h.w = in.w; h.a0 = in.a0; h.a1 = in.a1;
+    const long long a_rows = in.conv ? (long long)in.B * in.Hin * in.Win : (long long)in.M;
+    h.ext_w = gh_clamp_extent((long long)in.N * in.K * 2);
+    h.ext_a0 = gh_clamp_extent(a_rows * in.lda0 * 2);
+    h.ext_a1 = in.a1 ? gh_clamp_extent(a_rows * in.lda1 * 2) : 0u;
+    h.flags = ((uint32_t)in.dbg & GH_DBG_MASK) | (in.conv ? GH_CONV : 0u) | (in.subpix ? GH_SUBPIX : 0u) | (in.zstuff ? GH_ZSTUFF : 0u) |
+              (in.ups ? GH_UPS : 0u) | (in.a1 ? GH_A1 : 0u) | (in.cs0 ? GH_TAIL : 0u) | (in.stamped ? GH_STAMPED : 0u) |
+              (in.batch > 1 ? GH_BATCHED : 0u);
+    h.rows = (uint32_t)(in.halo ? in.Hin : in.M);
+    h.N = (uint32_t)in.N;
+    h.wpitch = (uint32_t)in.K * 2u;
+    h.lda0 = (uint32_t)in.lda0; h.lda1 = (uint32_t)in.lda1; h.c0 = (uint32_t)in.c0;
+    h.ntn = (uint32_t)((in.N + in.BN - 1) / in.BN);
+    h.ntm = (uint32_t)(in.halo ? in.M / in.BM : (in.M + in.BM - 1) / in.BM);
+    const uint32_t GM = (uint32_t)(in.group_m > 1 ? in.group_m : 1);
+    h.group_m = GM;
+    const uint32_t last = h.ntm % GM ? h.ntm % GM : GM;
+    const MagicDiv pg = magic_for(GM * h.ntn), gm = magic_for(GM), ls = magic_for(last);
+    h.mul_pg = pg.mul; h.mul_gm = gm.mul; h.mul_last = ls.mul;
+    const int Ct = in.c0 + in.c1;
+    h.Ct = (uint32_t)Ct;
+    const int units = in.halo ? Ct / 64 : in.K / 64;
+    h.per = (uint32_t)((units + in.splitk - 1) / in.splitk);
+    h.per_sc = (uint32_t)(((in.cs0 + in.cs1) / 64 + in.splitk - 1) / in.splitk);
+    if (in.pretouch > 0) {
+        const long long pieces = ((long long)in.N * in.K * 2 + 1023) >> 10;
+        const long long n_wg = (long long)h.ntn * h.ntm * in.splitk;
+        const int per_wg = (int)((pieces + n_wg - 1) / n_wg);
+        const int per_wave = (per_wg + 3) >> 2;
+        h.pt_per_wg = (uint32_t)per_wg;
+        h.pt_per_wave = (uint32_t)(per_wave < in.pretouch ? per_wave : in.pretouch);
+    }
+    MagicDiv hw = magic_for(1), wd = magic_for(1), pw = magic_for(1);
+    if (in.halo) {
+        const int TH = in.BM / in.Win, PW = in.Win + 2, npix = (TH + 2) * PW, pit = (npix * 8 + 255) / 256;
+        hw = magic_for((uint32_t)(in.Hin * in.Win)); wd = magic_for((uint32_t)in.Win); pw = magic_for((uint32_t)PW);
+        h.geom = (uint32_t)in.Win | (uint32_t)TH << 8 | (uint32_t)PW << 16 | (uint32_t)pit << 24;
+    } else if (in.conv) {
+        hw = magic_for((uint32_t)(in.Hout * in.Wout)); wd = magic_for((uint32_t)in.Wout);
+    }
+    h.mul_hw = hw.mul; h.mul_wd = wd.mul; h.mul_pw = pw.mul;
+    h.shifts = pg.l << GH_SH_PG | gm.l << GH_SH_GM | ls.l << GH_SH_LAST | hw.l << GH_SH_HW | wd.l << GH_SH_WD | pw.l << GH_SH_PW;
+    return h;
+}
+
+MRISR_GH_HD void gh_tile_coords(const GemmHead& h, uint32_t bid, uint32_t& tm, uint32_t& tn) {
+    const uint32_t nblk = h.ntn * h.ntm;
+    const uint32_t xcd = bid & 7u, q = nblk >> 3, r = nblk & 7u;
+    const uint32_t logical = (xcd < r ? xcd * (q + 1u) : r * (q + 1u) + (xcd - r) * q) + (bid >> 3);
+    const uint32_t per_group = h.group_m * h.ntn;
+    const uint32_t grp = magic_div(logical, h.mul_pg, gh_shift(h, GH_SH_PG));
+    const uint32_t first_m = grp * h.group_m;
+    const uint32_t left = h.ntm - first_m;
+    const bool full = h.group_m <= left;
+    const uint32_t gsz = full ? h.group_m : left;
+    const uint32_t within = logical - grp * per_group;
+    tn = magic_div(within, full ? h.mul_gm : h.mul_last, gh_shift(h, full ? GH_SH_GM : GH_SH_LAST));
+    tm = first_m + (within - tn * gsz);
+}
+MRISR_GH_HD void gh_split_range(uint32_t per, uint32_t total, uint32_t split, int& beg, int& end) {
+    const uint32_t b = split * per, e = b + per;
+    beg = (int)b;
+    end = (int)(e < total ? e : total);
+}
+MRISR_GH_HD void gh_row_pixel(const GemmHead& h, uint32_t m, uint32_t hw, uint32_t wout, uint32_t& b, uint32_t& oy, uint32_t& ox) {
+    b = magic_div(m, h.mul_hw, gh_shift(h, GH_SH_HW));
+    const uint32_t rem = m - b * hw;
+    oy = magic_div(rem, h.mul_wd, gh_shift(h, GH_SH_WD));
+    ox = rem - oy * wout;
+}
+MRISR_GH_HD uint32_t gh_div_pw(const GemmHead& h, uint32_t x) { return magic_div(x, h.mul_pw, gh_shift(h, GH_SH_PW)); }
+MRISR_GH_HD uint32_t gh_div_wd(const GemmHead& h, uint32_t x) { return magic_div(x, h.mul_wd, gh_shift(h, GH_SH_WD)); }
+
+}
```

New measurement: 71.30 slices/s, median of 6. 3.1% higher.
